# facebookresearch/dmc-net

Hardware: AMD Instinct MI355X
Metric: clips/sec (3-seg 224x224) DMC-gen+ResNet-18 train step (higher is better)
Workload: dtype f32

## Files before the change

dmc-net_amd/_lib.py:

```python
import ctypes
import os

PKG = os.path.dirname(os.path.abspath(__file__))
LIB_PATH = os.environ.get("DMC_HIP_LIB", os.path.join(PKG, "libdmcnet_hip.so"))

_P = ctypes.c_void_p
_I = ctypes.c_int
_F = ctypes.c_float
_Z = ctypes.c_size_t
_L = ctypes.c_long

SIGNATURES = {
    "dmc_version": (_I, []),
    "dmc_last_error": (ctypes.c_char_p, []),
    "dmc_profile_mark": (_I, [_P]),
    "dmc_set_option": (_I, [ctypes.c_char_p, _I]),
    "dmc_get_option": (_I, [ctypes.c_char_p]),
    "dmc_gen_tiny_workspace_bytes": (_Z, []),
    "dmc_gen_tiny_saved_bytes": (_Z, [_I, _I, _I]),
    "dmc_gen_tiny_gbuf_bytes": (_Z, [_I, _I, _I]),
    "dmc_gen_tiny_partials_bytes": (_Z, [_I, _I, _I]),
    "dmc_gen_tiny_fwd": (_I, [_P, _P, _P, _P, _P, _P, _P, _I, _I, _I, _I, _P]),
    "dmc_gen_tiny_mse_partials_bytes": (_Z, []),
    "dmc_gen_tiny_fwd_mse": (_I, [_P] * 10 + [_I, _I, _I, _I, _P]),
    "dmc_gen_tiny_bwd": (_I, [_P, _P, _P, _P, _P, _P, _P, _P, _P, _P, _I, _I, _I, _P]),
    "dmc_flow_mse_partials_bytes": (_Z, []),
    "dmc_flow_mse_fwd": (_I, [_P, _P, _P, _P, _Z, _P]),
    "dmc_flow_mse_bwd": (_I, [_P, _P, _P, _P, _Z, _P]),
    "dmc_consensus_ce_fwd_bwd": (_I, [_P, _P, _P, _P, _P, _I, _I, _I, _P]),
    "dmc_disc_tail_stats_bytes": (_Z, [_I]),
    "dmc_disc_tail_fwd": (_I, [_P, _P, _P, _P, _P, _P, _P, _P, _I, _I, _I, _I, _I, _I, _F, _F, _P]),
    "dmc_disc_tail_bwd": (_I, [_P, _P, _P, _P, _P, _P, _P, _P, _I, _I, _I, _I, _I, _P]),
    "dmc_prepare_inputs_workspace_bytes": (_Z, [_I, _I, _I, _I]),
    "dmc_prepare_inputs": (_I, [_P, _P, _P, _P, _P, _P, _I, _I, _I, _I, _P, _P]),
    "dmc_prepare_crop_workspace_bytes": (_Z, [_I, _I, _I, _I]),
    "dmc_prepare_inputs_crop": (_I, [_P, _P, _P, _P, _P, _P, _P, _I, _I, _I, _I, _I, _I, _P, _P]),
    "dmc_prepare_views_workspace_bytes": (_Z, [_I, _I, _I, _I, _I]),
    "dmc_prepare_inputs_views": (_I, [_P, _P, _P, _P, _P, _P, _P, _P, _I, _I, _I, _I, _I, _I, _I, _I, _P, _P]),
    "dmc_prepare_interp_taps": (_I, [_I, _I, _P, _P, _P]),
    "dmc_prepare_clip_workspace_bytes": (_Z, [_I, _I, _I, _I, _I]),
    "dmc_prepare_clip": (_I, [_P, _P, _P, _P] + [_I] * 8 + [_P, _P, _P]),
    "dmc_bn_act_supported": (_I, [_I, _I]),
    "dmc_bn_act_stats_bytes": (_Z, [_I]),
    "dmc_bn_act_scratch_bytes": (_Z, [_I]),
    "dmc_bn_act_fwd": (_I, [_P, _P, _P, _P, _P, _P, _P, _P, _P, _P, _I, _I, _I, _I, _F, _F, _P]),
    "dmc_bn_act_bwd": (_I, [_P, _P, _P, _P, _P, _P, _P, _P, _P, _P, _P, _P, _I, _I, _I, _P]),
    "dmc_bn_apply_nhwc": (_I, [_P, _P, _P, _P, _P, _I, _I, _P]),
    "dmc_bn_apply_act_nhwc": (_I, [_P, _P, _P, _P, _P, _P, _P, _I, _I, _I, _P]),
    "dmc_bn_bwd_act_nhwc": (_I, [_P] * 10 + [_I, _F, _I, _I, _P]),
    "dmc_channel_sum_nhwc": (_I, [_P, _P, _P, _I, _I, _P]),
    "dmc_bn_relu_pool_supported": (_I, [_I, _I, _I, _I]),
    "dmc_bn_relu_pool_fwd": (_I, [_P, _P, _P, _P, _P, _P, _P, _P, _I, _I, _I, _I, _I, _F, _F, _P]),
    "dmc_bn_relu_pool_codes_bytes": (_Z, [_I, _I, _I, _I]),
    "dmc_bn_relu_pool_bwd": (_I, [_P, _P, _P, _P, _P, _P, _P, _P, _P, _P, _I, _I, _I, _I, _P]),
    "dmc_conv_nhwc_supported": (_I, [_I] * 9),
    "dmc_conv_nhwc_stat_blocks": (_I, [_I] * 8),
    "dmc_conv_nhwc_fwd": (_I, [_P] * 7 + [_I] * 11 + [_P]),
    "dmc_conv_nhwc_stats_final": (_I, [_P, _I, _I, ctypes.c_long, _P, _P, _P, _F, _F, _P]),
    "dmc_conv_nhwc_wt_bytes": (_Z, [_I] * 4),
    "dmc_conv_nhwc_presplit_supported": (_I, [_I, _I]),
    "dmc_conv_nhwc_split": (_I, [_P, _P, _P, _I, _I, _I, _I, _P]),
    "dmc_conv_nhwc_dgrad": (_I, [_P] * 4 + [_I] * 9 + [_P]),
    "dmc_conv_nhwc_dgrad_add": (_I, [_P] * 5 + [_I] * 9 + [_P]),
    "dmc_conv_nhwc_wgrad_bytes": (_Z, [_I] * 9),
    "dmc_conv_nhwc_wgrad": (_I, [_P] * 4 + [_I] * 9 + [_P]),
    "dmc_x3s_slices_bytes": (_Z, [_L, _I]),
    "dmc_x3s_split": (_I, [_P, _P, _L, _I, _P]),
    "dmc_x3s_merge": (_I, [_P, _P, _L, _I, _P]),
    "dmc_x3s_wpack_bytes": (_Z, [_I, _I]),
    "dmc_x3s_pack_weights": (_I, [_P, _P, _P, _I, _I, _P]),
    "dmc_x3s_conv_supported": (_I, [_I] * 5),
    "dmc_x3s_conv_stat_blocks": (_I, [_I] * 4),
    "dmc_x3s_conv_fwd": (_I, [_P] * 4 + [_I] * 6 + [_P]),
    "dmc_x3s_conv_dgrad": (_I, [_P] * 4 + [_I] * 5 + [_P]),
    "dmc_x3s_conv_wgrad_supported": (_I, [_I] * 5),
    "dmc_x3s_conv_wgrad_bytes": (_Z, [_I] * 5),
    "dmc_x3s_conv_wgrad": (_I, [_P] * 4 + [_I] * 5 + [_P]),
    "dmc_x3s_conv_dgrad_s2_supported": (_I, [_I] * 5),
    "dmc_x3s_pack_weights_s2": (_I, [_P, _P, _I, _I, _P]),
    "dmc_x3s_conv_dgrad_s2": (_I, [_P] * 3 + [_I] * 5 + [_P]),
    "dmc_x3q_wpack_bytes": (_Z, [_I, _I]),
    "dmc_x3q_supported": (_I, [_I] * 5),
    "dmc_x3q_stat_blocks": (_I, [_I] * 4),
    "dmc_x3q_split": (_I, [_P, _P, _I, _I, _I, _I, _P]),
    "dmc_x3q_merge": (_I, [_P, _P, _I, _I, _I, _I, _P]),
    "dmc_x3q_pack_weights": (_I, [_P, _P, _P, _P, _I, _I, _P]),
    "dmc_x3q_conv_fwd": (_I, [_P] * 6 + [_I] * 6 + [_P]),
    "dmc_x3q_conv_dgrad": (_I, [_P] * 4 + [_I] * 5 + [_P]),
    "dmc_bn_apply_act_x3q": (_I, [_P] * 8 + [_I] * 5 + [_P]),
    "dmc_x3q_conv_wgrad_supported": (_I, [_I] * 5),
    "dmc_x3q_conv_wgrad_bytes": (_Z, [_I] * 5),
    "dmc_x3q_conv_wgrad": (_I, [_P] * 6 + [_I] * 5 + [_P]),
    "dmc_bn_apply_act_x3s": (_I, [_P] * 8 + [_I, _I, _I, _P]),
    "dmc_bn_act_bwd_x3s": (_I, [_P] * 13 + [_I, _I, _I, _P]),
    "dmc_x3s_conv_dgrad_bnb": (_I, [_P] * 9 + [_I] + [_P] + [_I] + [_P] * 2 + [_I] * 5 + [_P]),
    "dmc_bn_act_bwd_x3s_apply": (_I, [_P] * 12 + [_I, _I, _I, _P]),
    "dmc_bn_relu_pool_fwd_x3s": (_I, [_P] * 9 + [_I, _I, _I, _I, _I, _F, _F, _P]),
    "dmc_bn_relu_pool_fwd_arg": (_I, [_P] * 11 + [_I, _I, _I, _I, _I, _I, _F, _F, _P]),
    "dmc_bn_relu_pool_bwd_arg": (_I, [_P] * 11 + [_I, _I, _I, _I, _P]),
    "dmc_disc_first_supported": (_I, [_I]),
    "dmc_disc_first_fwd": (_I, [_P] * 5 + [_I] * 5 + [_P]),
    "dmc_disc_first_dgrad": (_I, [_P] * 3 + [_I] * 4 + [_P]),
    "dmc_disc_first_wgrad_bytes": (_Z, [_I]),
    "dmc_disc_first_wgrad": (_I, [_P] * 5 + [_I] * 4 + [_P]),
    "dmc_stem_wgrad_supported": (_I, [_I, _I]),
    "dmc_stem_wgrad_partials_bytes": (_Z, [_I, _I, _I]),
    "dmc_stem_wgrad": (_I, [_P, _P, _P, _P, _I, _I, _I, _P]),
    "dmc_stem_fwd": (_I, [_P, _P, _L, _L, _L, _L, _P, _I, _I, _I, _P]),
    "dmc_stem_fwd_x3_workspace_bytes": (_Z, [_I, _I, _I]),
    "dmc_stem_fwd_x3": (_I, [_P, _P, _L, _L, _L, _L, _P, _P, _I, _I, _I, _P]),
    "dmc_stem_fwd_x3_stat_blocks": (_I, [_I, _I, _I]),
    "dmc_stem_dgrad_workspace_bytes": (_Z, []),
    "dmc_stem_dgrad_supported": (_I, [_I, _I]),
    "dmc_stem_dgrad": (_I, [_P, _P, _L, _L, _L, _L, _P, _P, _I, _I, _I, _P]),
    "dmc_stem_fwd_x3_stats": (_I, [_P, _P, _L, _L, _L, _L, _P, _P, _P, _I, _I, _I, _P]),
    "dmc_conv3d_bf16_supported": (_I, [_I] * 9),
    "dmc_conv3d_bf16_wpack_bytes": (_Z, [_I] * 5),
    "dmc_conv3d_bf16_pack": (_I, [_P, _L, _L, _L, _P, _P] + [_I] * 5 + [_P]),
    "dmc_conv3d_bf16_stat_blocks": (_I, [_I] * 5),
    "dmc_conv3d_bf16_stat_blocks_k": (_I, [_I] * 9),
    "dmc_conv3d_bf16_fwd": (_I, [_P, _P, _L, _L, _L, _P, _P, _P] + [_I] * 9 + [_P]),
    "dmc_conv3d_bf16_dgrad": (_I, [_P, _P, _L, _L, _L, _P, _P] + [_I] * 9 + [_P]),
    "dmc_conv3d_bf16_wgrad_bytes": (_Z, [_I] * 9),
    "dmc_conv3d_bf16_wgrad": (_I, [_P] * 4 + [_I] * 9 + [_P]),
    "dmc_stem3d_bf16_workspace_bytes": (_Z, [_I] * 4),
    "dmc_stem3d_bf16_stat_blocks": (_I, [_I] * 4),
    "dmc_stem3d_bf16_fwd": (_I, [_P] * 5 + [_I] * 4 + [_P]),
    "dmc_stem3d_bf16_wgrad_workspace_bytes": (_Z, [_I] * 4),
    "dmc_stem3d_bf16_wgrad": (_I, [_P] * 4 + [_I] * 4 + [_P]),
    "dmc_stem3d_bf16_dgrad_workspace_bytes": (_Z, []),
    "dmc_stem3d_bf16_dgrad": (_I, [_P] * 4 + [_I] * 4 + [_P]),
    "dmc_bn3d_bf16_supported": (_I, [_L, _I]),
    "dmc_bn3d_bf16_scratch_bytes": (_Z, [_I]),
    "dmc_bn3d_bf16_fwd": (_I, [_P, _P, _I, _P, _P, _P, _P, _P, _P, _L, _I, _I, _F, _F, _P]),
    "dmc_add4_bf16": (_I, [_P] * 5 + [_L, _P]),
    "dmc_bn3d_bf16_fwd_ld": (_I, [_P, _P, _I, _P, _P, _P, _P, _P, _P, _L, _L, _I, _I, _F, _F, _P]),
    "dmc_bn3d_bf16_bwd": (_I, [_P, _L] + [_P] * 8 + [_L, _I, _I, _P]),
    "dmc_unit3d_bf16_fwd_workspace_bytes": (_Z, [_I] * 9),
    "dmc_unit3d_bf16_bwd_workspace_bytes": (_Z, [_I] * 9),
    "dmc_unit3d_bf16_fwd": (_I, [_P] * 9 + [_I] * 10 + [_F, _F, _P]),
    "dmc_unit3d_bf16_fwd_into": (_I, [_P] * 9 + [_L] + [_I] * 10 + [_F, _F, _P]),
    "dmc_unit3d_bf16_bwd": (_I, [_P, _L] + [_P] * 11 + [_I] * 10 + [_P]),
    "dmc_unit3d_bf16_eval_workspace_bytes": (_Z, [_I] * 9),
    "dmc_unit3d_bf16_fwd_eval": (_I, [_P] * 6 + [_F, _P, _P, _L] + [_I] * 10 + [_P]),
    "dmc_stem3d_bf16_eval_workspace_bytes": (_Z, [_I] * 4),
    "dmc_stem3d_bf16_fwd_eval": (_I, [_P] * 6 + [_F, _P, _P] + [_I] * 5 + [_P]),
    "dmc_maxpool3d_tf_out_shape": (_I, [_I] * 10 + [_P] * 3),
    "dmc_maxpool3d_tf_bf16_fwd": (_I, [_P] * 3 + [_I] * 11 + [_P]),
    "dmc_maxpool3d_tf_bf16_bwd": (_I, [_P] * 3 + [_I] * 11 + [_P]),
    "dmc_mv_owner_bytes": (_Z, [_I, _I, _I]),
    "dmc_mv_accu_init": (_I, [_P, _I, _I, _P]),
    "dmc_mv_rasterise": (_I, [_P, _I, _I, _P, _P, _P, _I, _I, _P]),
    "dmc_mv_accumulate": (_I, [_P, _I, _I, _P, _P, _P, _P, _I, _I, _P]),
    "dmc_mv_from_accu": (_I, [_P, _P, _I, _I, _P]),
    "dmc_residual": (_I, [_P, _P, _P, _P, _P, _I, _I, _P]),
    "dmc_mv_gop_batch": (_I, [_P, _I, _I, _P, _I, _P, _I, _P, _P, _P, _P, _P, _P, _P, _P, _I, _I, _P]),
}

_lib = None


class DmcHipError(RuntimeError):
    pass


def load():
    global _lib
    if _lib is None:
        if not os.path.exists(LIB_PATH):
            raise DmcHipError(
                "%s is missing: the DMC-Net hot path has no CPU fallback. Build it with "
                "`python -c 'import __graft_entry__ as g; g.build()'`." % LIB_PATH)
        lib = ctypes.CDLL(LIB_PATH)
        for name, (res, args) in SIGNATURES.items():
            fn = getattr(lib, name)
            fn.restype, fn.argtypes = res, args
        _lib = lib
    return _lib


def check(rc, what):
    if rc != 0:
        raise DmcHipError("%s failed (%d): %s" % (what, rc, load().dmc_last_error().decode()))


def ptr(t):
    return _P(t.data_ptr()) if t is not None else _P(0)


def ptr_array(tensors):
    return (_P * len(tensors))(*[t.data_ptr() for t in tensors])
```

dmc-net_amd/build.py:

```python
import os
import subprocess
import sys

PKG = os.path.dirname(os.path.abspath(__file__))
ROOT = os.path.dirname(PKG)
CSRC = os.path.join(PKG, "csrc")
LIB = os.path.join(PKG, "libdmcnet_hip.so")
MEASURE_ONLY = ["gen_fused_bwd.hip"]
SOURCES = ["gen_tiny.hip", "gen_x3.hip", "gen_fused.hip", "gen_wgrad.hip", "losses.hip", "disc_tail.hip", "bn_act.hip", "prepare.hip", "clip_prep.hip", "stem.hip", "conv_nhwc.hip", "conv_small.hip", "conv_x3s.hip", "conv_x3q.hip", "disc_first.hip", "conv3d_bf16.hip", "pool3d_bf16.hip", "bn3d_bf16.hip", "stem3d_bf16.hip", "unit3d.hip", "coviar_post.hip"]
HIPCC = os.environ.get("HIPCC", "/opt/rocm/bin/hipcc")
FLAGS = ["--offload-arch=gfx950", "-O3", "-std=c++17", "-fPIC", "-ffp-contract=off",
         "-Wall", "-Wno-unused-function"]


MANIFEST = os.path.join(PKG, "libdmcnet_hip.manifest.json")


def _sha(path):
    import hashlib
    with open(path, "rb") as f:
        return hashlib.sha256(f.read()).hexdigest()


def source_hashes():
    deps = sorted(os.path.join(CSRC, f) for f in os.listdir(CSRC) if not f.endswith((".o", ".hipfb")))
    deps += [os.path.join(ROOT, "include", "dmcnet_hip.h"), os.path.abspath(__file__)]
    return {os.path.relpath(d, ROOT): _sha(d) for d in deps}


def read_manifest():
    import json
    try:
        with open(MANIFEST) as f:
            return json.load(f)
    except (OSError, ValueError):
        return None


def _stale():
    if not os.path.exists(LIB):
        return True
    m = read_manifest()
    return m is None or m.get("library_sha256") != _sha(LIB) or m.get("sources") != source_hashes()


def _write_manifest(compiled):
    import json
    import time
    with open(MANIFEST, "w") as f:
        json.dump({"library": os.path.relpath(LIB, ROOT), "library_sha256": _sha(LIB), "built_at": time.strftime("%Y-%m-%dT%H:%M:%SZ", time.gmtime()),
                   "compiled_objects": compiled, "hipcc": HIPCC, "flags": FLAGS, "sources": source_hashes()}, f, indent=1, sort_keys=True)


LAST_BUILD = {"action": None}


MEASURE_LIB = os.path.join(PKG, "libdmcnet_hip_measure.so")


def build_library(force=False, verbose=False, measure=False):
    if measure:
        return _build_measure(verbose)
    if not force and not _stale():
        LAST_BUILD["action"] = "up to date (sources and library match the manifest's hashes)"
        return LIB
    objs, compiled = [], []
    for src in SOURCES:
        path = os.path.join(CSRC, src)
        if not os.path.exists(path):
            continue
        obj = os.path.join(CSRC, src.replace(".hip", ".o"))
        objs.append(obj)
        hdrs = [os.path.join(CSRC, "dmc_common.h"), os.path.join(CSRC, "x3s_common.h"), os.path.join(CSRC, "conv_small.h"), os.path.join(CSRC, "gen_x3.h"), os.path.join(CSRC, "gen_fused.h"), os.path.join(CSRC, "gen_fused_inl.h"), os.path.join(CSRC, "gen_wgrad.h"), os.path.join(ROOT, "include", "dmcnet_hip.h"),
                os.path.abspath(__file__)]
        if not force and os.path.exists(obj) and all(os.path.getmtime(d) <= os.path.getmtime(obj) for d in [path] + hdrs):
            continue
        cmd = [HIPCC] + FLAGS + ["-I", os.path.join(ROOT, "include"), "-I", CSRC, "-c", path, "-o", obj]
        if verbose:
            print(" ".join(cmd))
        subprocess.check_call(cmd)
        compiled.append(src)
    cmd = [HIPCC, "--offload-arch=gfx950", "-shared", "-fPIC", "-o", LIB] + objs
    if verbose:
        print(" ".join(cmd))
    subprocess.check_call(cmd)
    _write_manifest(compiled)
    LAST_BUILD["action"] = "compiled %d of %d sources and linked: %s" % (len(compiled), len(objs), ", ".join(compiled) or "(objects were current)")
    return LIB


def _build_measure(verbose):
    objs = []
    for src in SOURCES + MEASURE_ONLY:
        path = os.path.join(CSRC, src)
        obj = os.path.join(CSRC, "measure_" + src.replace(".hip", ".o"))
        objs.append(obj)
        deps = [path, os.path.abspath(__file__)] + [os.path.join(CSRC, f) for f in os.listdir(CSRC) if f.endswith(".h")]
        if os.path.exists(obj) and all(os.path.getmtime(d) <= os.path.getmtime(obj) for d in deps):
            continue
        cmd = [HIPCC] + FLAGS + ["-DDMC_MEASURE", "-I", os.path.join(ROOT, "include"), "-I", CSRC, "-c", path, "-o", obj]
        if verbose:
            print(" ".join(cmd))
        subprocess.check_call(cmd)
    subprocess.check_call([HIPCC, "--offload-arch=gfx950", "-shared", "-fPIC", "-o", MEASURE_LIB] + objs)
    return MEASURE_LIB


if __name__ == "__main__":
    print(build_library(force="--force" in sys.argv, verbose=True, measure="--measure" in sys.argv))
```

dmc-net_amd/csrc/bn_act.hip:

```cpp
#include "dmc_common.h"

using namespace dmc;

namespace {

constexpr int MAX_SPLIT = BN_MAX_SPLIT;

struct BnArgs {
    const float* x;
    const float* res;
    const float* gamma;
    const float* beta;
    const float* stats;
    const float* dy;
    float* y;
    float* dx;
    float* dres;
    int M, C, relu;
    unsigned char* mask;
    const float* keep;
    int hw;
    float slope;
};

template <int MODE>
__global__ __launch_bounds__(256) void bn_partial_kernel(BnArgs a, double* __restrict__ scratch) {
    __shared__ double sm[2][256][4];
    const int cq = a.C >> 2;
    const int tx = threadIdx.x % cq, ty = threadIdx.x / cq, rows = 256 / cq;
    const int per = (a.M + (int)gridDim.x - 1) / (int)gridDim.x;
    const int r0 = blockIdx.x * per, r1 = (r0 + per < a.M) ? r0 + per : a.M;
    float4 s0 = make_float4(0.f, 0.f, 0.f, 0.f), s1 = s0;
    float4 mean = s0, istd = s0, g = s0, b = s0;
    if (MODE == 1) {
        mean = reinterpret_cast<const float4*>(a.stats)[tx];
        istd = reinterpret_cast<const float4*>(a.stats + a.C)[tx];
        g = reinterpret_cast<const float4*>(a.gamma)[tx];
        b = reinterpret_cast<const float4*>(a.beta)[tx];
    }
#pragma unroll 4
    for (int r = r0 + ty; r < r1; r += rows) {
        const size_t o = (size_t)r * cq + tx;
        const float4 x = reinterpret_cast<const float4*>(a.x)[o];
        if (MODE == 0) {
            s0.x += x.x; s0.y += x.y; s0.z += x.z; s0.w += x.w;
            s1.x = fmaf(x.x, x.x, s1.x); s1.y = fmaf(x.y, x.y, s1.y);
            s1.z = fmaf(x.z, x.z, s1.z); s1.w = fmaf(x.w, x.w, s1.w);
        } else {
            float4 d = reinterpret_cast<const float4*>(a.dy)[o];
            const float4 xh = make_float4((x.x - mean.x) * istd.x, (x.y - mean.y) * istd.y,
                                          (x.z - mean.z) * istd.z, (x.w - mean.w) * istd.w);
            if (a.relu && a.mask) {
                const unsigned mb = a.mask[o];
                d.x = (mb & 1) ? d.x : 0.f; d.y = (mb & 2) ? d.y : 0.f;
                d.z = (mb & 4) ? d.z : 0.f; d.w = (mb & 8) ? d.w : 0.f;
            } else if (a.relu) {
                float4 v = make_float4(fmaf(xh.x, g.x, b.x), fmaf(xh.y, g.y, b.y),
                                       fmaf(xh.z, g.z, b.z), fmaf(xh.w, g.w, b.w));
                if (a.res) {
                    const float4 rr = reinterpret_cast<const float4*>(a.res)[o];
                    v.x += rr.x; v.y += rr.y; v.z += rr.z; v.w += rr.w;
                }
                d.x = v.x > 0.f ? d.x : 0.f; d.y = v.y > 0.f ? d.y : 0.f;
                d.z = v.z > 0.f ? d.z : 0.f; d.w = v.w > 0.f ? d.w : 0.f;
            }
            s0.x += d.x; s0.y += d.y; s0.z += d.z; s0.w += d.w;
            s1.x = fmaf(d.x, xh.x, s1.x); s1.y = fmaf(d.y, xh.y, s1.y);
            s1.z = fmaf(d.z, xh.z, s1.z); s1.w = fmaf(d.w, xh.w, s1.w);
        }
    }
    sm[0][threadIdx.x][0] = s0.x; sm[0][threadIdx.x][1] = s0.y;
    sm[0][threadIdx.x][2] = s0.z; sm[0][threadIdx.x][3] = s0.w;
    sm[1][threadIdx.x][0] = s1.x; sm[1][threadIdx.x][1] = s1.y;
    sm[1][threadIdx.x][2] = s1.z; sm[1][threadIdx.x][3] = s1.w;
    __syncthreads();
    for (int i = threadIdx.x; i < cq * 8; i += 256) {
        const int col = i >> 3, which = (i >> 2) & 1, e = i & 3;
        double acc = 0.0;
        for (int t = 0; t < rows; ++t) acc += sm[which][t * cq + col][e];
        scratch[((size_t)(col * 4 + e) * MAX_SPLIT + blockIdx.x) * 2 + which] = acc;
    }
}

__device__ __forceinline__ void reduce_partials(const double* __restrict__ scratch, int C, int c,
                                                int split, int sub, double& s, double& ss) {
    s = 0.0; ss = 0.0;
    if (c < C) {
        const double2* row = reinterpret_cast<const double2*>(scratch) + (size_t)c * MAX_SPLIT;
#pragma unroll 4
        for (int sp = sub; sp < split; sp += 32) {
            const double2 v = row[sp];
            s += v.x;
            ss += v.y;
        }
    }
#pragma unroll
    for (int o = 16; o > 0; o >>= 1) {
        s += __shfl_down(s, o, 32);
        ss += __shfl_down(ss, o, 32);
    }
}

__global__ __launch_bounds__(256) void bn_stats_final_kernel(
    const double* __restrict__ scratch, float* __restrict__ stats, float* __restrict__ running_mean,
    float* __restrict__ running_var, int C, long count, int training, float eps, float momentum,
    int split) {
    const int c = blockIdx.x * 8 + (threadIdx.x >> 5), sub = threadIdx.x & 31;
    if (!training) {
        if (c < C && sub == 0) {
            stats[c] = running_mean[c];
            stats[C + c] = rsqrtf(running_var[c] + eps);
        }
        return;
    }
    double s, ss;
    reduce_partials(scratch, C, c, split, sub, s, ss);
    if (c >= C || sub != 0) return;
    const double mean = s / (double)count;
    double var = ss / (double)count - mean * mean;
    if (var < 0.0) var = 0.0;
    stats[c] = (float)mean;
    stats[C + c] = (float)(1.0 / sqrt(var + (double)eps));
    const double unbiased = count > 1 ? var * (double)count / (double)(count - 1) : var;
    running_mean[c] = (1.f - momentum) * running_mean[c] + momentum * (float)mean;
    running_var[c] = (1.f - momentum) * running_var[c] + momentum * (float)unbiased;
}

__global__ __launch_bounds__(256) void bn_bwd_final_kernel(const double* __restrict__ scratch,
                                                           float* __restrict__ dgamma,
                                                           float* __restrict__ dbeta, int C,
                                                           int split) {
    __shared__ double red[2][4];
    const int c = blockIdx.x, lane = threadIdx.x & 63, wave = threadIdx.x >> 6;
    const double2* row = reinterpret_cast<const double2*>(scratch) + (size_t)c * MAX_SPLIT;
    double2 v[MAX_SPLIT / 256];
#pragma unroll
    for (int k = 0; k < MAX_SPLIT / 256; ++k) {
        const int sp = (int)threadIdx.x + 256 * k;
        v[k] = sp < split ? row[sp] : make_double2(0.0, 0.0);
    }
    double s = 0.0, ss = 0.0;
#pragma unroll
    for (int k = 0; k < MAX_SPLIT / 256; ++k) { s += v[k].x; ss += v[k].y; }
#pragma unroll
    for (int o = 32; o > 0; o >>= 1) { s += __shfl_down(s, o, 64); ss += __shfl_down(ss, o, 64); }
    if (lane == 0) { red[0][wave] = s; red[1][wave] = ss; }
    __syncthreads();
    if (threadIdx.x != 0) return;
    dbeta[c] = (float)(red[0][0] + red[0][1] + red[0][2] + red[0][3]);
    dgamma[c] = (float)(red[1][0] + red[1][1] + red[1][2] + red[1][3]);
}

__global__ __launch_bounds__(256) void bn_apply_fwd_kernel(BnArgs a) {
    const int cq = a.C >> 2;
    const size_t total = (size_t)a.M * cq;
    for (size_t o = (size_t)blockIdx.x * 256 + threadIdx.x; o < total; o += (size_t)gridDim.x * 256) {
        const int tx = (int)(o & (size_t)(cq - 1));
        const float4 mean = reinterpret_cast<const float4*>(a.stats)[tx];
        const float4 istd = reinterpret_cast<const float4*>(a.stats + a.C)[tx];
        const float4 g = reinterpret_cast<const float4*>(a.gamma)[tx];
        const float4 b = reinterpret_cast<const float4*>(a.beta)[tx];
        const float4 x = reinterpret_cast<const float4*>(a.x)[o];
        float4 v = make_float4(fmaf((x.x - mean.x) * istd.x, g.x, b.x), fmaf((x.y - mean.y) * istd.y, g.y, b.y),
                               fmaf((x.z - mean.z) * istd.z, g.z, b.z), fmaf((x.w - mean.w) * istd.w, g.w, b.w));
        if (a.res) {
            const float4 rr = reinterpret_cast<const float4*>(a.res)[o];
            v.x += rr.x; v.y += rr.y; v.z += rr.z; v.w += rr.w;
        }
        if (a.relu) {
            if (a.mask)
                a.mask[o] = (unsigned char)((v.x > 0.f ? 1 : 0) | (v.y > 0.f ? 2 : 0) | (v.z > 0.f ? 4 : 0) | (v.w > 0.f ? 8 : 0));
            v.x = fmaxf(v.x, 0.f); v.y = fmaxf(v.y, 0.f); v.z = fmaxf(v.z, 0.f); v.w = fmaxf(v.w, 0.f);
        }
        reinterpret_cast<float4*>(a.y)[o] = v;
    }
}

__global__ __launch_bounds__(256) void bn_apply_bwd_kernel(BnArgs a, const float* __restrict__ dgamma,
                                                           const float* __restrict__ dbeta,
                                                           float inv_count) {
    const int cq = a.C >> 2;
    const size_t total = (size_t)a.M * cq;
    for (size_t o = (size_t)blockIdx.x * 256 + threadIdx.x; o < total; o += (size_t)gridDim.x * 256) {
        const int tx = (int)(o & (size_t)(cq - 1));
        const float4 mean = reinterpret_cast<const float4*>(a.stats)[tx];
        const float4 istd = reinterpret_cast<const float4*>(a.stats + a.C)[tx];
        const float4 g = reinterpret_cast<const float4*>(a.gamma)[tx];
        const float4 b = reinterpret_cast<const float4*>(a.beta)[tx];
        const float4 dg = reinterpret_cast<const float4*>(dgamma)[tx];
        const float4 db = reinterpret_cast<const float4*>(dbeta)[tx];
        const float4 x = reinterpret_cast<const float4*>(a.x)[o];
        float4 d = reinterpret_cast<const float4*>(a.dy)[o];
        const float4 xh = make_float4((x.x - mean.x) * istd.x, (x.y - mean.y) * istd.y,
                                      (x.z - mean.z) * istd.z, (x.w - mean.w) * istd.w);
        if (a.relu && a.mask) {
            const unsigned mb = a.mask[o];
            d.x = (mb & 1) ? d.x : 0.f; d.y = (mb & 2) ? d.y : 0.f;
            d.z = (mb & 4) ? d.z : 0.f; d.w = (mb & 8) ? d.w : 0.f;
        } else if (a.relu) {
            float4 v = make_float4(fmaf(xh.x, g.x, b.x), fmaf(xh.y, g.y, b.y), fmaf(xh.z, g.z, b.z),
                                   fmaf(xh.w, g.w, b.w));
            if (a.res) {
                const float4 rr = reinterpret_cast<const float4*>(a.res)[o];
                v.x += rr.x; v.y += rr.y; v.z += rr.z; v.w += rr.w;
            }
            d.x = v.x > 0.f ? d.x : 0.f; d.y = v.y > 0.f ? d.y : 0.f;
            d.z = v.z > 0.f ? d.z : 0.f; d.w = v.w > 0.f ? d.w : 0.f;
        }
        if (a.dres) reinterpret_cast<float4*>(a.dres)[o] = d;
        float4 r;
        r.x = g.x * istd.x * (d.x - db.x * inv_count - xh.x * dg.x * inv_count);
        r.y = g.y * istd.y * (d.y - db.y * inv_count - xh.y * dg.y * inv_count);
        r.z = g.z * istd.z * (d.z - db.z * inv_count - xh.z * dg.z * inv_count);
        r.w = g.w * istd.w * (d.w - db.w * inv_count - xh.w * dg.w * inv_count);
        if (a.slope != 0.f) {
            float4 k = make_float4(1.f, 1.f, 1.f, 1.f);
            if (a.keep) k = reinterpret_cast<const float4*>(a.keep)[(size_t)((o / cq) / a.hw) * cq + tx];
            r.x *= k.x * (x.x > 0.f ? 1.f : a.slope); r.y *= k.y * (x.y > 0.f ? 1.f : a.slope);
            r.z *= k.z * (x.z > 0.f ? 1.f : a.slope); r.w *= k.w * (x.w > 0.f ? 1.f : a.slope);
        }
        reinterpret_cast<float4*>(a.dx)[o] = r;
    }
}

struct PoolArgs {
    const float* x;
    const float* gamma;
    const float* beta;
    const float* stats;
    const float* dpool;
    float* ypool;
    float* dx;
    int N, H, W, C, PH, PW;
};

__device__ __forceinline__ float4 bn_relu4(const float4 x, const float4 mean, const float4 istd,
                                           const float4 g, const float4 b) {
    return make_float4(fmaxf(fmaf((x.x - mean.x) * istd.x, g.x, b.x), 0.f), fmaxf(fmaf((x.y - mean.y) * istd.y, g.y, b.y), 0.f),
                       fmaxf(fmaf((x.z - mean.z) * istd.z, g.z, b.z), 0.f), fmaxf(fmaf((x.w - mean.w) * istd.w, g.w, b.w), 0.f));
}

__global__ __launch_bounds__(256) void pool_fwd_kernel(PoolArgs a) {
    const int cq = a.C >> 2;
    const size_t total = (size_t)a.N * a.PH * a.PW * cq;
    for (size_t o = (size_t)blockIdx.x * 256 + threadIdx.x; o < total; o += (size_t)gridDim.x * 256) {
        const int tx = (int)(o & (size_t)(cq - 1));
        size_t r = o / cq;
        const int px = (int)(r % a.PW); r /= a.PW;
        const int py = (int)(r % a.PH);
        const int n = (int)(r / a.PH);
        const float4 mean = reinterpret_cast<const float4*>(a.stats)[tx];
        const float4 istd = reinterpret_cast<const float4*>(a.stats + a.C)[tx];
        const float4 g = reinterpret_cast<const float4*>(a.gamma)[tx];
        const float4 b = reinterpret_cast<const float4*>(a.beta)[tx];
        float4 m = make_float4(0.f, 0.f, 0.f, 0.f);
        float4 xv[9];
#pragma unroll
        for (int k = 0; k < 9; ++k) {
            int iy = 2 * py + k / 3 - 1, ix = 2 * px + k % 3 - 1;
            iy = iy < 0 ? 0 : (iy >= a.H ? a.H - 1 : iy);
            ix = ix < 0 ? 0 : (ix >= a.W ? a.W - 1 : ix);
            xv[k] = reinterpret_cast<const float4*>(a.x)[((size_t)(n * a.H + iy) * a.W + ix) * cq + tx];
        }
#pragma unroll
        for (int k = 0; k < 9; ++k) {
            const float4 v = bn_relu4(xv[k], mean, istd, g, b);
            m.x = fmaxf(m.x, v.x); m.y = fmaxf(m.y, v.y); m.z = fmaxf(m.z, v.z); m.w = fmaxf(m.w, v.w);
        }
        reinterpret_cast<float4*>(a.ypool)[o] = m;
    }
}

constexpr int PT = 8;
template <int PASS>
__global__ __launch_bounds__(256) void pool_bwd_kernel(PoolArgs a, double* __restrict__ scratch,
                                                       const float* __restrict__ dgamma,
                                                       const float* __restrict__ dbeta, float inv_count,
                                                       unsigned* __restrict__ gcodes) {
    __shared__ unsigned codes[(PT + 1) * (PT + 1) * 64];
    __shared__ double sm[PASS == 1 ? 2 : 1][PASS == 1 ? 256 : 1][4];
    const int cq = a.C >> 2;
    const int tx = threadIdx.x % cq, ty = threadIdx.x / cq, rows = 256 / cq;
    const float4 mean = reinterpret_cast<const float4*>(a.stats)[tx];
    const float4 istd = reinterpret_cast<const float4*>(a.stats + a.C)[tx];
    const float4 g = reinterpret_cast<const float4*>(a.gamma)[tx];
    const float4 b = reinterpret_cast<const float4*>(a.beta)[tx];
    float4 dg = make_float4(0.f, 0.f, 0.f, 0.f), db = dg;
    if (PASS == 2) {
        dg = reinterpret_cast<const float4*>(dgamma)[tx];
        db = reinterpret_cast<const float4*>(dbeta)[tx];
    }
    float4 s0 = make_float4(0.f, 0.f, 0.f, 0.f), s1 = s0;
    const int tiles_x = (a.PW + PT - 1) / PT, tiles_y = (a.PH + PT - 1) / PT;
    const int ntiles = a.N * tiles_y * tiles_x;
    for (int tile = blockIdx.x; tile < ntiles; tile += gridDim.x) {
        const int n = tile / (tiles_y * tiles_x), tr = tile - n * tiles_y * tiles_x;
        const int wy0 = (tr / tiles_x) * PT, wx0 = (tr % tiles_x) * PT;
        __syncthreads();
        for (int wi = ty; wi < (PT + 1) * (PT + 1); wi += rows) {
            const int py = wy0 + wi / (PT + 1), px = wx0 + wi % (PT + 1);
            unsigned code = 0xffffffffu;
            if (PASS == 2 && gcodes) {
                if (py < a.PH && px < a.PW) code = gcodes[((size_t)(n * a.PH + py) * a.PW + px) * cq + tx];
            } else if (py < a.PH && px < a.PW) {
                float4 mv = make_float4(-INFINITY, -INFINITY, -INFINITY, -INFINITY);
                unsigned cx = 0, cy = 0, cz = 0, cw = 0;
                float4 xv[9];
#pragma unroll
                for (int k = 0; k < 9; ++k) {
                    int iy = 2 * py + k / 3 - 1, ix = 2 * px + k % 3 - 1;
                    iy = iy < 0 ? 0 : (iy >= a.H ? a.H - 1 : iy);
                    ix = ix < 0 ? 0 : (ix >= a.W ? a.W - 1 : ix);
                    xv[k] = reinterpret_cast<const float4*>(a.x)[((size_t)(n * a.H + iy) * a.W + ix) * cq + tx];
                }
#pragma unroll
                for (int k = 0; k < 9; ++k) {
                    const int iy = 2 * py + k / 3 - 1, ix = 2 * px + k % 3 - 1;
                    const bool in = iy >= 0 && iy < a.H && ix >= 0 && ix < a.W;
                    const float4 v = bn_relu4(xv[k], mean, istd, g, b);
                    if (in && v.x > mv.x) { mv.x = v.x; cx = k; }
                    if (in && v.y > mv.y) { mv.y = v.y; cy = k; }
                    if (in && v.z > mv.z) { mv.z = v.z; cz = k; }
                    if (in && v.w > mv.w) { mv.w = v.w; cw = k; }
                }
                code = cx | (cy << 8) | (cz << 16) | (cw << 24);
                if (PASS == 1 && gcodes && wi / (PT + 1) < PT && wi % (PT + 1) < PT)
                    gcodes[((size_t)(n * a.PH + py) * a.PW + px) * cq + tx] = code;
            }
            codes[wi * cq + tx] = code;
        }
        __syncthreads();
        for (int pi = ty; pi < 4 * PT * PT; pi += rows) {
            const int iy = 2 * wy0 + pi / (2 * PT), ix = 2 * wx0 + pi % (2 * PT);
            if (iy >= a.H || ix >= a.W) continue;
            const size_t o = ((size_t)(n * a.H + iy) * a.W + ix) * cq + tx;
            const float4 x = reinterpret_cast<const float4*>(a.x)[o];
            const float4 xh = make_float4((x.x - mean.x) * istd.x, (x.y - mean.y) * istd.y,
                                          (x.z - mean.z) * istd.z, (x.w - mean.w) * istd.w);
            const float4 v = make_float4(fmaf(xh.x, g.x, b.x), fmaf(xh.y, g.y, b.y), fmaf(xh.z, g.z, b.z), fmaf(xh.w, g.w, b.w));
            float4 d = make_float4(0.f, 0.f, 0.f, 0.f);
            const int py0 = iy >> 1, px0 = ix >> 1, npy = 1 + (iy & 1), npx = 1 + (ix & 1);
            float4 gp[4];
            unsigned cd[4];
            bool okc[4];
#pragma unroll
            for (int q = 0; q < 4; ++q) {
                const int jy = q >> 1, jx = q & 1;
                const int py = py0 + jy, px = px0 + jx;
                okc[q] = jy < npy && jx < npx && py < a.PH && px < a.PW;
                const int pyc = okc[q] ? py : py0, pxc = okc[q] ? px : px0;
                cd[q] = codes[((pyc - wy0) * (PT + 1) + (pxc - wx0)) * cq + tx];
                gp[q] = reinterpret_cast<const float4*>(a.dpool)[((size_t)(n * a.PH + pyc) * a.PW + pxc) * cq + tx];
            }
#pragma unroll
            for (int q = 0; q < 4; ++q) {
                const int py = py0 + (q >> 1), px = px0 + (q & 1);
                const unsigned k = (unsigned)((iy - 2 * py + 1) * 3 + (ix - 2 * px + 1));
                if (okc[q] && (cd[q] & 0xff) == k) d.x += gp[q].x;
                if (okc[q] && ((cd[q] >> 8) & 0xff) == k) d.y += gp[q].y;
                if (okc[q] && ((cd[q] >> 16) & 0xff) == k) d.z += gp[q].z;
                if (okc[q] && (cd[q] >> 24) == k) d.w += gp[q].w;
            }
            d.x = v.x > 0.f ? d.x : 0.f; d.y = v.y > 0.f ? d.y : 0.f;
            d.z = v.z > 0.f ? d.z : 0.f; d.w = v.w > 0.f ? d.w : 0.f;
            if (PASS == 1) {
                s0.x += d.x; s0.y += d.y; s0.z += d.z; s0.w += d.w;
                s1.x = fmaf(d.x, xh.x, s1.x); s1.y = fmaf(d.y, xh.y, s1.y);
                s1.z = fmaf(d.z, xh.z, s1.z); s1.w = fmaf(d.w, xh.w, s1.w);
            } else {
                float4 r;
                r.x = g.x * istd.x * (d.x - db.x * inv_count - xh.x * dg.x * inv_count);
                r.y = g.y * istd.y * (d.y - db.y * inv_count - xh.y * dg.y * inv_count);
                r.z = g.z * istd.z * (d.z - db.z * inv_count - xh.z * dg.z * inv_count);
                r.w = g.w * istd.w * (d.w - db.w * inv_count - xh.w * dg.w * inv_count);
                reinterpret_cast<float4*>(a.dx)[o] = r;
            }
        }
    }
    if (PASS == 1) {
        sm[0][threadIdx.x][0] = s0.x; sm[0][threadIdx.x][1] = s0.y;
        sm[0][threadIdx.x][2] = s0.z; sm[0][threadIdx.x][3] = s0.w;
        sm[1][threadIdx.x][0] = s1.x; sm[1][threadIdx.x][1] = s1.y;
        sm[1][threadIdx.x][2] = s1.z; sm[1][threadIdx.x][3] = s1.w;
        __syncthreads();
        for (int i = threadIdx.x; i < cq * 8; i += 256) {
            const int col = i >> 3, which = (i >> 2) & 1, e = i & 3;
            double acc = 0.0;
            for (int t = 0; t < rows; ++t) acc += sm[which][t * cq + col][e];
            scratch[((size_t)(col * 4 + e) * MAX_SPLIT + blockIdx.x) * 2 + which] = acc;
        }
    }
}

__global__ __launch_bounds__(256) void act_mask_bwd_kernel(const float* __restrict__ z, const float* __restrict__ keep,
                                                           const float* __restrict__ dz, float* __restrict__ dx,
                                                           int M, int C, int hw, float slope) {
    const int cq = C >> 2;
    const size_t total = (size_t)M * cq;
    for (size_t o = (size_t)blockIdx.x * 256 + threadIdx.x; o < total; o += (size_t)gridDim.x * 256) {
        const int tx = (int)(o % cq);
        const float4 x = reinterpret_cast<const float4*>(z)[o];
        float4 d = reinterpret_cast<const float4*>(dz)[o];
        float4 k = make_float4(1.f, 1.f, 1.f, 1.f);
        if (keep) k = reinterpret_cast<const float4*>(keep)[(size_t)((o / cq) / hw) * cq + tx];
        d.x *= k.x * (x.x > 0.f ? 1.f : slope); d.y *= k.y * (x.y > 0.f ? 1.f : slope);
        d.z *= k.z * (x.z > 0.f ? 1.f : slope); d.w *= k.w * (x.w > 0.f ? 1.f : slope);
        reinterpret_cast<float4*>(dx)[o] = d;
    }
}

__global__ __launch_bounds__(256) void channel_sum_final_kernel(const double* __restrict__ scratch,
                                                                float* __restrict__ out, int C, int split) {
    const int c = blockIdx.x * 8 + (threadIdx.x >> 5), sub = threadIdx.x & 31;
    double s, ss;
    reduce_partials(scratch, C, c, split, sub, s, ss);
    if (c < C && sub == 0) out[c] = (float)s;
}

bool shape_ok(int M, int C) {
    const int cq = C / 4;
    return M > 0 && C > 0 && C % 4 == 0 && cq <= 256 && 256 % cq == 0;
}

int split_of(int M, int C) {
    long sp = (long)M * C / 8192;
    return sp < 1 ? 1 : (sp > MAX_SPLIT ? MAX_SPLIT : (int)sp);
}

int stream_blocks(size_t total) {
    size_t b = (total + 255) / 256;
    return (int)(b < 1 ? 1 : (b > 8192 ? 8192 : b));
}


__device__ __forceinline__ void load8(const float* p, size_t i8, float (&v)[8]) {
    const float4 a = reinterpret_cast<const float4*>(p)[2 * i8], b = reinterpret_cast<const float4*>(p)[2 * i8 + 1];
    v[0] = a.x; v[1] = a.y; v[2] = a.z; v[3] = a.w; v[4] = b.x; v[5] = b.y; v[6] = b.z; v[7] = b.w;
}
__device__ __forceinline__ void store8(float* p, size_t i8, const float (&v)[8]) {
    reinterpret_cast<float4*>(p)[2 * i8] = make_float4(v[0], v[1], v[2], v[3]);
    reinterpret_cast<float4*>(p)[2 * i8 + 1] = make_float4(v[4], v[5], v[6], v[7]);
}

__global__ __launch_bounds__(256) void bn_apply_fwd_x3s_kernel(BnArgs a, unsigned short* __restrict__ ys, int s2d_h, int s2d_w) {
    const int c8 = a.C >> 3;
    const size_t total = (size_t)a.M * c8;
    for (size_t o = (size_t)blockIdx.x * 256 + threadIdx.x; o < total; o += (size_t)gridDim.x * 256) {
        const int tx = (int)(o & (size_t)(c8 - 1));
        const size_t m = o / c8;
        float mean[8], istd[8], g[8], b[8], x[8], v[8];
        load8(a.stats, tx, mean); load8(a.stats + a.C, tx, istd); load8(a.gamma, tx, g); load8(a.beta, tx, b);
        load8(a.x, o, x);
#pragma unroll
        for (int e = 0; e < 8; ++e) v[e] = fmaf((x[e] - mean[e]) * istd[e], g[e], b[e]);
        if (a.res) {
            float rr[8];
            load8(a.res, o, rr);
#pragma unroll
            for (int e = 0; e < 8; ++e) v[e] += rr[e];
        }
        if (a.relu) {
            if (a.mask) {
                unsigned mb = 0;
#pragma unroll
                for (int e = 0; e < 8; ++e) mb |= (v[e] > 0.f ? 1u : 0u) << e;
                reinterpret_cast<unsigned short*>(a.mask)[o] = (unsigned short)((mb & 15u) | ((mb >> 4) << 8));
            }
#pragma unroll
            for (int e = 0; e < 8; ++e) v[e] = fmaxf(v[e], 0.f);
        }
        if (a.y) store8(a.y, o, v);
        if (ys) {
            if (s2d_w) {
                const int xx = (int)(m % (size_t)s2d_w), yy = (int)((m / (size_t)s2d_w) % (size_t)s2d_h);
                const size_t n = m / ((size_t)s2d_w * s2d_h);
                const int cls = (yy & 1) * 2 + (xx & 1), nchunk = a.C >> 4;
                x3s_store8(ys, v, (size_t)a.M >> 2, 4 * nchunk, (n * (s2d_h >> 1) + (yy >> 1)) * (s2d_w >> 1) + (xx >> 1), tx + cls * 2 * nchunk);
            } else {
                x3s_store8(ys, v, (size_t)a.M, a.C >> 4, m, tx);
            }
        }
    }
}

__global__ __launch_bounds__(256) void bn_apply_bwd_x3s_kernel(BnArgs a, const float* __restrict__ dgamma,
                                                               const float* __restrict__ dbeta, float inv_count,
                                                               unsigned short* __restrict__ dxs) {
    const int c8 = a.C >> 3;
    const size_t total = (size_t)a.M * c8;
    for (size_t o = (size_t)blockIdx.x * 256 + threadIdx.x; o < total; o += (size_t)gridDim.x * 256) {
        const int tx = (int)(o & (size_t)(c8 - 1));
        const size_t m = o / c8;
        float mean[8], istd[8], g[8], b[8], dg[8], db[8], x[8], d[8], xh[8], r[8];
        load8(a.stats, tx, mean); load8(a.stats + a.C, tx, istd); load8(a.gamma, tx, g); load8(a.beta, tx, b);
        load8(dgamma, tx, dg); load8(dbeta, tx, db);
        load8(a.x, o, x); load8(a.dy, o, d);
#pragma unroll
        for (int e = 0; e < 8; ++e) xh[e] = (x[e] - mean[e]) * istd[e];
        if (a.relu && a.mask) {
            const unsigned mw = reinterpret_cast<const unsigned short*>(a.mask)[o];
            const unsigned mb = (mw & 15u) | ((mw >> 8) << 4);
#pragma unroll
            for (int e = 0; e < 8; ++e) d[e] = ((mb >> e) & 1u) ? d[e] : 0.f;
        } else if (a.relu) {
            float rr[8];
            if (a.res) load8(a.res, o, rr);
#pragma unroll
            for (int e = 0; e < 8; ++e) {
                float v = fmaf(xh[e], g[e], b[e]);
                if (a.res) v += rr[e];
                d[e] = v > 0.f ? d[e] : 0.f;
            }
        }
        if (a.dres) store8(a.dres, o, d);
#pragma unroll
        for (int e = 0; e < 8; ++e) r[e] = g[e] * istd[e] * (d[e] - db[e] * inv_count - xh[e] * dg[e] * inv_count);
        if (a.dx) store8(a.dx, o, r);
        if (dxs) x3s_store8(dxs, r, (size_t)a.M, a.C >> 4, m, tx);
    }
}

__global__ __launch_bounds__(256) void pool_fwd_x3s_kernel(PoolArgs a, unsigned short* __restrict__ ys, unsigned* __restrict__ codes,
                                                           float* __restrict__ xmax) {
    const int c8 = a.C >> 3;
    const size_t total = (size_t)a.N * a.PH * a.PW * c8;
    for (size_t o = (size_t)blockIdx.x * 256 + threadIdx.x; o < total; o += (size_t)gridDim.x * 256) {
        const int tx = (int)(o & (size_t)(c8 - 1));
        size_t r = o / c8;
        const size_t mp = r;
        const int px = (int)(r % a.PW); r /= a.PW;
        const int py = (int)(r % a.PH);
        const int n = (int)(r / a.PH);
        float mean[8], istd[8], g[8], b[8], mx[8];
        load8(a.stats, tx, mean); load8(a.stats + a.C, tx, istd); load8(a.gamma, tx, g); load8(a.beta, tx, b);
        float xv[9][8];
#pragma unroll
        for (int k = 0; k < 9; ++k) {
            int iy = 2 * py + k / 3 - 1, ix = 2 * px + k % 3 - 1;
            iy = iy < 0 ? 0 : (iy >= a.H ? a.H - 1 : iy);
            ix = ix < 0 ? 0 : (ix >= a.W ? a.W - 1 : ix);
            load8(a.x, ((size_t)(n * a.H + iy) * a.W + ix) * c8 + tx, xv[k]);
        }
        if (codes) {
            float bx[8];
            unsigned ck[8];
#pragma unroll
            for (int e = 0; e < 8; ++e) { mx[e] = -INFINITY; bx[e] = 0.f; ck[e] = 0; }
#pragma unroll
            for (int k = 0; k < 9; ++k) {
                const int iy = 2 * py + k / 3 - 1, ix = 2 * px + k % 3 - 1;
                const bool in = iy >= 0 && iy < a.H && ix >= 0 && ix < a.W;
#pragma unroll
                for (int e = 0; e < 8; ++e) {
                    const float v = fmaxf(fmaf((xv[k][e] - mean[e]) * istd[e], g[e], b[e]), 0.f);
                    const bool take = in && v > mx[e];
                    mx[e] = take ? v : mx[e];
                    bx[e] = take ? xv[k][e] : bx[e];
                    ck[e] = take ? (unsigned)k : ck[e];
                }
            }
            reinterpret_cast<uint2*>(codes)[o] = make_uint2(ck[0] | (ck[1] << 8) | (ck[2] << 16) | (ck[3] << 24),
                                                            ck[4] | (ck[5] << 8) | (ck[6] << 16) | (ck[7] << 24));
            store8(xmax, o, bx);
        } else {
#pragma unroll
            for (int e = 0; e < 8; ++e) mx[e] = 0.f;
#pragma unroll
            for (int k = 0; k < 9; ++k)
#pragma unroll
                for (int e = 0; e < 8; ++e) mx[e] = fmaxf(mx[e], fmaxf(fmaf((xv[k][e] - mean[e]) * istd[e], g[e], b[e]), 0.f));
        }
        if (a.ypool) store8(a.ypool, o, mx);
        if (ys) x3s_store8(ys, mx, (size_t)a.N * a.PH * a.PW, a.C >> 4, mp, tx);
    }
}

bool shape_ok8(int M, int C) { return shape_ok(M, C) && C % 16 == 0 && C >= 16; }

}

extern "C" {

int dmc_bn_act_supported(int M, int C) { return shape_ok(M, C) ? 1 : 0; }

size_t dmc_bn_act_stats_bytes(int C) { return (((size_t)2 * C * sizeof(float)) + 15) / 16 * 16; }
size_t dmc_bn_act_scratch_bytes(int C) { return (size_t)MAX_SPLIT * C * 2 * sizeof(double); }

int dmc_bn_act_fwd(const float* x, const float* residual, const float* gamma, const float* beta,
                   float* running_mean, float* running_var, float* y, float* stats, void* scratch_,
                   unsigned char* relu_mask, int M, int C, int relu, int training, float eps,
                   float momentum, dmc_stream_t stream) {
    if (!x || !gamma || !beta || !running_mean || !running_var || !y || !stats || (training && !scratch_))
        return fail(DMC_E_INVALID, "dmc_bn_act_fwd: null pointer");
    if (!shape_ok(M, C)) return fail(DMC_E_INVALID, "dmc_bn_act_fwd: unsupported shape M=%d C=%d", M, C);
    hipStream_t s = (hipStream_t)stream;
    BnArgs a = {x, residual, gamma, beta, stats, nullptr, y, nullptr, nullptr, M, C, relu, relu_mask};
    double* scratch = static_cast<double*>(scratch_);
    int rc;
    const int split = split_of(M, C);
    if (training) {
        bn_partial_kernel<0><<<split, 256, 0, s>>>(a, scratch);
        if ((rc = check_launch("bn_partial"))) return rc;
    }
    bn_stats_final_kernel<<<(C + 7) / 8, 256, 0, s>>>(scratch, stats, running_mean, running_var, C,
                                                       (long)M, training, eps, momentum, split);
    if ((rc = check_launch("bn_stats_final"))) return rc;
    bn_apply_fwd_kernel<<<stream_blocks((size_t)M * (C / 4)), 256, 0, s>>>(a);
    return check_launch("bn_apply_fwd");
}

int dmc_bn_act_bwd(const float* x, const float* residual, const float* gamma, const float* beta,
                   const float* stats, void* scratch_, const float* dy, float* dx, float* dresidual,
                   float* dgamma, float* dbeta, const unsigned char* relu_mask, int M, int C, int relu,
                   dmc_stream_t stream) {
    if (!x || !gamma || !beta || !stats || !scratch_ || !dy || !dx || !dgamma || !dbeta)
        return fail(DMC_E_INVALID, "dmc_bn_act_bwd: null pointer");
    if (!shape_ok(M, C)) return fail(DMC_E_INVALID, "dmc_bn_act_bwd: unsupported shape M=%d C=%d", M, C);
    hipStream_t s = (hipStream_t)stream;
    BnArgs a = {x, residual, gamma, beta, stats, dy, nullptr, dx, dresidual, M, C, relu,
                const_cast<unsigned char*>(relu_mask)};
    double* scratch = static_cast<double*>(scratch_);
    int rc;
    const int split = split_of(M, C);
    bn_partial_kernel<1><<<split, 256, 0, s>>>(a, scratch);
    if ((rc = check_launch("bn_bwd_partial"))) return rc;
    bn_bwd_final_kernel<<<C, 256, 0, s>>>(scratch, dgamma, dbeta, C, split);
    if ((rc = check_launch("bn_bwd_final"))) return rc;
    bn_apply_bwd_kernel<<<stream_blocks((size_t)M * (C / 4)), 256, 0, s>>>(a, dgamma, dbeta, 1.f / (float)M);
    return check_launch("bn_apply_bwd");
}

int dmc_bn_relu_pool_supported(int N, int H, int W, int C) {
    return N > 0 && H > 0 && W > 0 && shape_ok(1, C) && C / 4 <= 64 ? 1 : 0;
}

int dmc_bn_relu_pool_fwd(const float* x, const float* gamma, const float* beta, float* running_mean,
                         float* running_var, float* y_pool, float* stats, void* scratch_, int N, int H,
                         int W, int C, int training, float eps, float momentum, dmc_stream_t stream) {
    if (!x || !gamma || !beta || !running_mean || !running_var || !y_pool || !stats || (training && !scratch_))
        return fail(DMC_E_INVALID, "dmc_bn_relu_pool_fwd: null pointer");
    if (!dmc_bn_relu_pool_supported(N, H, W, C))
        return fail(DMC_E_INVALID, "dmc_bn_relu_pool_fwd: unsupported shape N=%d H=%d W=%d C=%d", N, H, W, C);
    hipStream_t s = (hipStream_t)stream;
    const int M = N * H * W;
    BnArgs a = {x, nullptr, gamma, beta, stats, nullptr, nullptr, nullptr, nullptr, M, C, 1, nullptr};
    double* scratch = static_cast<double*>(scratch_);
    int rc;
    const int split = split_of(M, C);
    if (training) {
        bn_partial_kernel<0><<<split, 256, 0, s>>>(a, scratch);
        if ((rc = check_launch("bn_partial"))) return rc;
    }
    bn_stats_final_kernel<<<(C + 7) / 8, 256, 0, s>>>(scratch, stats, running_mean, running_var, C,
                                                       (long)M, training, eps, momentum, split);
    if ((rc = check_launch("bn_stats_final"))) return rc;
    PoolArgs p = {x, gamma, beta, stats, nullptr, y_pool, nullptr, N, H, W, C, (H - 1) / 2 + 1, (W - 1) / 2 + 1};
    pool_fwd_kernel<<<stream_blocks((size_t)N * p.PH * p.PW * (C / 4)), 256, 0, s>>>(p);
    return check_launch("pool_fwd");
}

size_t dmc_bn_relu_pool_codes_bytes(int N, int H, int W, int C) {
    return (size_t)N * ((H - 1) / 2 + 1) * ((W - 1) / 2 + 1) * (C / 4) * sizeof(unsigned);
}

int dmc_bn_relu_pool_bwd(const float* x, const float* gamma, const float* beta, const float* stats,
                         void* scratch_, const float* d_pool, float* dx, float* dgamma, float* dbeta,
                         void* codes, int N, int H, int W, int C, dmc_stream_t stream) {
    if (!x || !gamma || !beta || !stats || !scratch_ || !d_pool || !dx || !dgamma || !dbeta)
        return fail(DMC_E_INVALID, "dmc_bn_relu_pool_bwd: null pointer");
    if (!dmc_bn_relu_pool_supported(N, H, W, C))
        return fail(DMC_E_INVALID, "dmc_bn_relu_pool_bwd: unsupported shape N=%d H=%d W=%d C=%d", N, H, W, C);
    hipStream_t s = (hipStream_t)stream;
    PoolArgs p = {x, gamma, beta, stats, d_pool, nullptr, dx, N, H, W, C, (H - 1) / 2 + 1, (W - 1) / 2 + 1};
    double* scratch = static_cast<double*>(scratch_);
    const long tiles = (long)N * ((p.PH + PT - 1) / PT) * ((p.PW + PT - 1) / PT);
    const int blocks = (int)(tiles < MAX_SPLIT ? tiles : MAX_SPLIT);
    int rc;
    pool_bwd_kernel<1><<<blocks, 256, 0, s>>>(p, scratch, nullptr, nullptr, 0.f, (unsigned*)codes);
    if ((rc = check_launch("pool_bwd_partial"))) return rc;
    bn_bwd_final_kernel<<<C, 256, 0, s>>>(scratch, dgamma, dbeta, C, blocks);
    if ((rc = check_launch("bn_bwd_final"))) return rc;
    pool_bwd_kernel<2><<<blocks * 4 > 8192 ? 8192 : blocks * 4, 256, 0, s>>>(p, nullptr, dgamma, dbeta,
                                                                             1.f / (float)((long)N * H * W), (unsigned*)codes);
    return check_launch("pool_bwd_apply");
}

int dmc_bn_apply_act_nhwc(const float* x, const float* residual, const float* gamma, const float* beta,
                          const float* stats, float* y, unsigned char* relu_mask, int M, int C, int relu,
                          dmc_stream_t stream) {
    if (!x || !gamma || !beta || !stats || !y) return fail(DMC_E_INVALID, "dmc_bn_apply_act_nhwc: null pointer");
    if (!shape_ok(M, C)) return fail(DMC_E_INVALID, "dmc_bn_apply_act_nhwc: unsupported shape M=%d C=%d", M, C);
    BnArgs a = {x, residual, gamma, beta, stats, nullptr, y, nullptr, nullptr, M, C, relu, relu_mask};
    bn_apply_fwd_kernel<<<stream_blocks((size_t)M * (C / 4)), 256, 0, (hipStream_t)stream>>>(a);
    return check_launch("bn_apply_act_nhwc");
}

int dmc_bn_apply_nhwc(const float* x, const float* gamma, const float* beta, const float* stats, float* y,
                      int M, int C, dmc_stream_t stream) {
    return dmc_bn_apply_act_nhwc(x, nullptr, gamma, beta, stats, y, nullptr, M, C, 0, stream);
}

int dmc_bn_bwd_act_nhwc(const float* z, const float* gamma, const float* beta, const float* stats, void* scratch_,
                        const float* dy, float* dpre, float* dgamma, float* dbeta, const float* keep, int hw,
                        float slope, int M, int C, dmc_stream_t stream) {
    if (!z || !dy || !dpre || hw <= 0) return fail(DMC_E_INVALID, "dmc_bn_bwd_act_nhwc: bad argument");
    if (!shape_ok(M, C)) return fail(DMC_E_INVALID, "dmc_bn_bwd_act_nhwc: unsupported shape M=%d C=%d", M, C);
    hipStream_t s = (hipStream_t)stream;
    if (!gamma) {
        act_mask_bwd_kernel<<<stream_blocks((size_t)M * (C / 4)), 256, 0, s>>>(z, keep, dy, dpre, M, C, hw, slope);
        return check_launch("act_mask_bwd");
    }
    if (!beta || !stats || !scratch_ || !dgamma || !dbeta)
        return fail(DMC_E_INVALID, "dmc_bn_bwd_act_nhwc: null BatchNorm pointer");
    BnArgs a = {z, nullptr, gamma, beta, stats, dy, nullptr, dpre, nullptr, M, C, 0, nullptr, keep, hw, slope};
    double* scratch = static_cast<double*>(scratch_);
    int rc;
    const int split = split_of(M, C);
    bn_partial_kernel<1><<<split, 256, 0, s>>>(a, scratch);
    if ((rc = check_launch("bn_bwd_partial"))) return rc;
    bn_bwd_final_kernel<<<C, 256, 0, s>>>(scratch, dgamma, dbeta, C, split);
    if ((rc = check_launch("bn_bwd_final"))) return rc;
    bn_apply_bwd_kernel<<<stream_blocks((size_t)M * (C / 4)), 256, 0, s>>>(a, dgamma, dbeta, 1.f / (float)M);
    return check_launch("bn_apply_bwd_act");
}

int dmc_channel_sum_nhwc(const float* g, void* scratch_, float* out, int M, int C, dmc_stream_t stream) {
    if (!g || !scratch_ || !out) return fail(DMC_E_INVALID, "dmc_channel_sum_nhwc: null pointer");
    if (!shape_ok(M, C)) return fail(DMC_E_INVALID, "dmc_channel_sum_nhwc: unsupported shape M=%d C=%d", M, C);
    hipStream_t s = (hipStream_t)stream;
    BnArgs a = {g, nullptr, nullptr, nullptr, nullptr, nullptr, nullptr, nullptr, nullptr, M, C, 0, nullptr};
    const int split = split_of(M, C);
    bn_partial_kernel<0><<<split, 256, 0, s>>>(a, static_cast<double*>(scratch_));
    int rc = check_launch("channel_sum_partial");
    if (rc) return rc;
    channel_sum_final_kernel<<<(C + 7) / 8, 256, 0, s>>>(static_cast<const double*>(scratch_), out, C, split);
    return check_launch("channel_sum_final");
}

int dmc_bn_apply_act_x3s(const float* x, const float* residual, const float* gamma, const float* beta, const float* stats,
                         float* y, void* ys, unsigned char* relu_mask, int M, int C, int relu, dmc_stream_t stream) {
    if (!x || !gamma || !beta || !stats || (!y && !ys)) return fail(DMC_E_INVALID, "dmc_bn_apply_act_x3s: null pointer");
    if (!shape_ok8(M, C)) return fail(DMC_E_INVALID, "dmc_bn_apply_act_x3s: unsupported shape M=%d C=%d", M, C);
    BnArgs a = {x, residual, gamma, beta, stats, nullptr, y, nullptr, nullptr, M, C, relu, relu_mask};
    bn_apply_fwd_x3s_kernel<<<stream_blocks((size_t)M * (C / 8)), 256, 0, (hipStream_t)stream>>>(a, static_cast<unsigned short*>(ys), 0, 0);
    return check_launch("bn_apply_act_x3s");
}

int dmc_bn_apply_act_x3q(const float* x, const float* residual, const float* gamma, const float* beta, const float* stats,
                         float* y, void* yq, unsigned char* relu_mask, int N, int H, int W, int C, int relu, dmc_stream_t stream) {
    if (!x || !gamma || !beta || !stats || !yq) return fail(DMC_E_INVALID, "dmc_bn_apply_act_x3q: null pointer");
    if (N <= 0 || H <= 0 || W <= 0 || (H & 1) || (W & 1) || (long)N * H * W >= (1L << 31)) return fail(DMC_E_INVALID, "dmc_bn_apply_act_x3q: bad geometry");
    const int M = N * H * W;
    if (!shape_ok8(M, C)) return fail(DMC_E_INVALID, "dmc_bn_apply_act_x3q: unsupported shape M=%d C=%d", M, C);
    BnArgs a = {x, residual, gamma, beta, stats, nullptr, y, nullptr, nullptr, M, C, relu, relu_mask};
    bn_apply_fwd_x3s_kernel<<<stream_blocks((size_t)M * (C / 8)), 256, 0, (hipStream_t)stream>>>(a, static_cast<unsigned short*>(yq), H, W);
    return check_launch("bn_apply_act_x3q");
}

int dmc_bn_act_bwd_x3s(const float* x, const float* residual, const float* gamma, const float* beta, const float* stats,
                       void* scratch_, const float* dy, float* dx, void* dxs, float* dresidual, float* dgamma, float* dbeta,
                       const unsigned char* relu_mask, int M, int C, int relu, dmc_stream_t stream) {
    if (!x || !gamma || !beta || !stats || !scratch_ || !dy || (!dx && !dxs) || !dgamma || !dbeta)
        return fail(DMC_E_INVALID, "dmc_bn_act_bwd_x3s: null pointer");
    if (!shape_ok8(M, C)) return fail(DMC_E_INVALID, "dmc_bn_act_bwd_x3s: unsupported shape M=%d C=%d", M, C);
    hipStream_t s = (hipStream_t)stream;
    BnArgs a = {x, residual, gamma, beta, stats, dy, nullptr, dx, dresidual, M, C, relu, const_cast<unsigned char*>(relu_mask)};
    double* scratch = static_cast<double*>(scratch_);
    int rc;
    const int split = split_of(M, C);
    bn_partial_kernel<1><<<split, 256, 0, s>>>(a, scratch);
    if ((rc = check_launch("bn_bwd_partial"))) return rc;
    bn_bwd_final_kernel<<<C, 256, 0, s>>>(scratch, dgamma, dbeta, C, split);
    if ((rc = check_launch("bn_bwd_final"))) return rc;
    bn_apply_bwd_x3s_kernel<<<stream_blocks((size_t)M * (C / 8)), 256, 0, s>>>(a, dgamma, dbeta, 1.f / (float)M, static_cast<unsigned short*>(dxs));
    return check_launch("bn_apply_bwd_x3s");
}

int dmc_bn_relu_pool_fwd_arg(const float* x, const float* gamma, const float* beta, float* running_mean, float* running_var,
                             float* y_pool, void* ys, void* codes, float* xmax, float* stats, void* scratch_, int stat_split,
                             int N, int H, int W, int C, int training, float eps, float momentum, dmc_stream_t stream) {
    if (!x || !gamma || !beta || !running_mean || !running_var || (!y_pool && !ys) || !stats || (training && !scratch_))
        return fail(DMC_E_INVALID, "dmc_bn_relu_pool_fwd_x3s: null pointer");
    if (stat_split < 0 || stat_split > MAX_SPLIT) return fail(DMC_E_INVALID, "dmc_bn_relu_pool_fwd_arg: bad stat_split %d", stat_split);
    if ((codes == nullptr) != (xmax == nullptr)) return fail(DMC_E_INVALID, "dmc_bn_relu_pool_fwd_arg: codes and xmax go together");
    if (!dmc_bn_relu_pool_supported(N, H, W, C) || C % 16 != 0)
        return fail(DMC_E_INVALID, "dmc_bn_relu_pool_fwd_x3s: unsupported shape N=%d H=%d W=%d C=%d", N, H, W, C);
    hipStream_t s = (hipStream_t)stream;
    const int M = N * H * W;
    BnArgs a = {x, nullptr, gamma, beta, stats, nullptr, nullptr, nullptr, nullptr, M, C, 1, nullptr};
    double* scratch = static_cast<double*>(scratch_);
    int rc;
    const int split = stat_split > 0 ? stat_split : split_of(M, C);
    if (training && stat_split == 0) {
        bn_partial_kernel<0><<<split, 256, 0, s>>>(a, scratch);
        if ((rc = check_launch("bn_partial"))) return rc;
    }
    bn_stats_final_kernel<<<(C + 7) / 8, 256, 0, s>>>(scratch, stats, running_mean, running_var, C, (long)M, training, eps, momentum, split);
    if ((rc = check_launch("bn_stats_final"))) return rc;
    PoolArgs p = {x, gamma, beta, stats, nullptr, y_pool, nullptr, N, H, W, C, (H - 1) / 2 + 1, (W - 1) / 2 + 1};
    pool_fwd_x3s_kernel<<<stream_blocks((size_t)N * p.PH * p.PW * (C / 8)), 256, 0, s>>>(p, static_cast<unsigned short*>(ys),
                                                                                         static_cast<unsigned*>(codes), xmax);
    return check_launch("pool_fwd_x3s");
}

int dmc_bn_relu_pool_fwd_x3s(const float* x, const float* gamma, const float* beta, float* running_mean, float* running_var,
                             float* y_pool, void* ys, float* stats, void* scratch_, int N, int H, int W, int C, int training,
                             float eps, float momentum, dmc_stream_t stream) {
    return dmc_bn_relu_pool_fwd_arg(x, gamma, beta, running_mean, running_var, y_pool, ys, nullptr, nullptr, stats, scratch_, 0, N, H, W, C,
                                    training, eps, momentum, stream);
}

int dmc_bn_relu_pool_bwd_arg(const float* x, const float* gamma, const float* beta, const float* stats, void* scratch_,
                             const float* d_pool, const void* codes, const float* xmax, float* dx, float* dgamma, float* dbeta,
                             int N, int H, int W, int C, dmc_stream_t stream) {
    if (!x || !gamma || !beta || !stats || !scratch_ || !d_pool || !codes || !xmax || !dx || !dgamma || !dbeta)
        return fail(DMC_E_INVALID, "dmc_bn_relu_pool_bwd_arg: null pointer");
    if (!dmc_bn_relu_pool_supported(N, H, W, C) || C % 16 != 0)
        return fail(DMC_E_INVALID, "dmc_bn_relu_pool_bwd_arg: unsupported shape N=%d H=%d W=%d C=%d", N, H, W, C);
    hipStream_t s = (hipStream_t)stream;
    PoolArgs p = {x, gamma, beta, stats, d_pool, nullptr, dx, N, H, W, C, (H - 1) / 2 + 1, (W - 1) / 2 + 1};
    double* scratch = static_cast<double*>(scratch_);
    const int MP = N * p.PH * p.PW;
    BnArgs a = {xmax, nullptr, gamma, beta, stats, d_pool, nullptr, nullptr, nullptr, MP, C, 1, nullptr};
    const int split = split_of(MP, C);
    int rc;
    bn_partial_kernel<1><<<split, 256, 0, s>>>(a, scratch);
    if ((rc = check_launch("pool_bwd_sums"))) return rc;
    bn_bwd_final_kernel<<<C, 256, 0, s>>>(scratch, dgamma, dbeta, C, split);
    if ((rc = check_launch("bn_bwd_final"))) return rc;
    const long tiles = (long)N * ((p.PH + PT - 1) / PT) * ((p.PW + PT - 1) / PT);
    const long blocks = tiles * 4 > 8192 ? 8192 : tiles * 4;
    pool_bwd_kernel<2><<<(int)blocks, 256, 0, s>>>(p, nullptr, dgamma, dbeta, 1.f / (float)((long)N * H * W),
                                                   const_cast<unsigned*>(static_cast<const unsigned*>(codes)));
    return check_launch("pool_bwd_apply");
}

int dmc_bn_act_bwd_x3s_apply(const float* x, const float* residual, const float* gamma, const float* beta, const float* stats,
                             const float* dy, float* dx, void* dxs, float* dresidual, const float* dgamma, const float* dbeta,
                             const unsigned char* relu_mask, int M, int C, int relu, dmc_stream_t stream) {
    if (!x || !gamma || !beta || !stats || !dy || (!dx && !dxs) || !dgamma || !dbeta)
        return fail(DMC_E_INVALID, "dmc_bn_act_bwd_x3s_apply: null pointer");
    if (!shape_ok8(M, C)) return fail(DMC_E_INVALID, "dmc_bn_act_bwd_x3s_apply: unsupported shape M=%d C=%d", M, C);
    BnArgs a = {x, residual, gamma, beta, stats, dy, nullptr, dx, dresidual, M, C, relu, const_cast<unsigned char*>(relu_mask)};
    bn_apply_bwd_x3s_kernel<<<stream_blocks((size_t)M * (C / 8)), 256, 0, (hipStream_t)stream>>>(a, dgamma, dbeta, 1.f / (float)M, static_cast<unsigned short*>(dxs));
    return check_launch("bn_apply_bwd_x3s");
}

}
```

dmc-net_amd/csrc/stem.hip:

```cpp
#include "dmc_common.h"

using namespace dmc;

namespace {

constexpr int S_CO = 64, S_CI = 2, S_K = 7, S_NCOL = S_CI * S_K * S_K;
constexpr int S_NT = (S_NCOL + 15) / 16;
constexpr int S_MT = S_CO / 16;
constexpr int S_TH = 7, S_TW = 16;
constexpr int S_XROWS = 2 * S_TH + 5, S_XPITCH = 40;
constexpr int S_XPLANE = S_XROWS * S_XPITCH;
constexpr int S_X = S_CI * S_XPLANE;
constexpr int S_G = S_TH * S_TW * S_CO;
constexpr int S_BUF = S_X + S_G;
constexpr int S_PART = S_MT * S_NT * 256;
constexpr int S_MAX_GROUPS = 256, S_RED = 16;
static_assert(S_PART <= 2 * S_BUF, "cross-wave reduction reuses the tile buffers");

struct StemArgs {
    const float* x;
    const float* dy;
    float* partials;
    int N, H, W, OH, OW, tiles_x, tiles_y;
};

__device__ __forceinline__ void stem_stage(const StemArgs& a, float* buf, int tile, int per_frame, int lane) {
    const int n = tile / per_frame, r0 = tile - n * per_frame;
    const int oy0 = (r0 / a.tiles_x) * S_TH, ox0 = (r0 % a.tiles_x) * S_TW;
    const unsigned buf_byte = lds_addr_of(buf);
    const bool g_interior = oy0 + S_TH <= a.OH && ox0 + S_TW <= a.OW;
#pragma unroll
    for (int row = 0; row < S_TH; ++row) {
        const unsigned long long rbase =
            (unsigned long long)(a.dy + (((size_t)n * a.OH + (oy0 + row)) * a.OW + ox0) * S_CO);
#pragma unroll
        for (int q = 0; q < 4; ++q) {
            const unsigned dst = buf_byte + (unsigned)(S_X + (row * S_TW + q * 4) * S_CO) * 4;
            if (g_interior) {
                lds_dma16(rbase + q * 1024, (unsigned)lane * 16, dst);
            } else {
                const bool ok = oy0 + row < a.OH && ox0 + q * 4 + (lane >> 4) < a.OW;
                if (ok) lds_dma16(rbase + q * 1024, (unsigned)lane * 16, dst);
                else reinterpret_cast<float4*>(buf + S_X + (row * S_TW + q * 4) * S_CO)[lane] = make_float4(0.f, 0.f, 0.f, 0.f);
            }
        }
    }
    const int iy0 = 2 * oy0 - 3, ix0 = 2 * ox0 - 4;
    const bool x_interior = iy0 >= 0 && iy0 + S_XROWS <= a.H && ix0 >= 0 && ix0 + S_XPITCH <= a.W;
    const size_t HW = (size_t)a.H * a.W;
#pragma unroll
    for (int ci = 0; ci < S_CI; ++ci) {
        const long org = ((long)iy0 * a.W + ix0) * 4;
        const unsigned long long pbase = (unsigned long long)(a.x + ((size_t)n * S_CI + ci) * HW) + (unsigned long long)org;
#pragma unroll
        for (int h = 0; h < 3; ++h) {
            const int L = 64 * h + lane;
            const int row = L / 10, ch = L - row * 10;
            const unsigned voff = (unsigned)(row * a.W + ch * 4) * 4;
            const unsigned dst = buf_byte + (unsigned)(ci * S_XPLANE + 256 * h) * 4;
            if (L < S_XROWS * 10) {
                const int iy = iy0 + row, ix = ix0 + ch * 4;
                const bool ok = x_interior || (iy >= 0 && iy < a.H && ix >= 0 && ix < a.W);
                if (ok) lds_dma16(pbase, voff, dst);
                else reinterpret_cast<float4*>(buf + ci * S_XPLANE)[L] = make_float4(0.f, 0.f, 0.f, 0.f);
            }
        }
    }
}

__global__ __launch_bounds__(512, 2) void stem_wgrad_kernel(StemArgs a) {
    __shared__ __attribute__((aligned(16))) float lds2[2 * S_BUF];
    const int lane = threadIdx.x & 63;
    const int wave = __builtin_amdgcn_readfirstlane((int)(threadIdx.x >> 6));
    const int j = lane & 15, kq = lane >> 4;
    const int per_frame = a.tiles_x * a.tiles_y;
    const int ntiles = a.N * per_frame;

    mfma_f32x4 acc[S_MT][S_NT];
#pragma unroll
    for (int m = 0; m < S_MT; ++m)
#pragma unroll
        for (int t = 0; t < S_NT; ++t) acc[m][t] = (mfma_f32x4){0.f, 0.f, 0.f, 0.f};

    if (wave == S_TH) {
        int it = 0;
        if ((int)blockIdx.x < ntiles) stem_stage(a, lds2, blockIdx.x, per_frame, lane);
        asm volatile("s_waitcnt vmcnt(0) lgkmcnt(0)\n\ts_barrier" ::: "memory");
        for (int tile = blockIdx.x; tile < ntiles; tile += gridDim.x, ++it) {
            const int next = tile + (int)gridDim.x;
            if (next < ntiles) stem_stage(a, lds2 + ((it + 1) & 1) * S_BUF, next, per_frame, lane);
            asm volatile("s_waitcnt vmcnt(0) lgkmcnt(0)\n\ts_barrier" ::: "memory");
        }
    } else {
        int offB[S_NT];
#pragma unroll
        for (int t = 0; t < S_NT; ++t) {
            int nn = 16 * t + j;
            nn = nn < S_NCOL ? nn : S_NCOL - 1;
            const int ci = nn / 49, rem = nn - ci * 49, ky = rem / 7, kx = rem - ky * 7;
            offB[t] = ci * S_XPLANE + (2 * wave + ky) * S_XPITCH + kx + 1 + 2 * kq;
        }
        const int offA = S_X + (wave * S_TW + kq) * S_CO + 4 * j;
        int it = 0;
        asm volatile("s_barrier" ::: "memory");
        for (int tile = blockIdx.x; tile < ntiles; tile += gridDim.x, ++it) {
            const float* lds = lds2 + (it & 1) * S_BUF;
#pragma unroll
            for (int g = 0; g < S_TW / 4; ++g) {
                const float4 av = *reinterpret_cast<const float4*>(lds + offA + g * 4 * S_CO);
                const float am[S_MT] = {av.x, av.y, av.z, av.w};
                float b[S_NT];
#pragma unroll
                for (int t = 0; t < S_NT; ++t) b[t] = lds[offB[t] + g * 8];
#pragma unroll
                for (int m = 0; m < S_MT; ++m)
#pragma unroll
                    for (int t = 0; t < S_NT; ++t)
                        acc[m][t] = __builtin_amdgcn_mfma_f32_16x16x4f32(am[m], b[t], acc[m][t], 0, 0, 0);
            }
            asm volatile("s_barrier" ::: "memory");
        }
    }
    float* lds = lds2;
    for (int w = 0; w < S_TH; ++w) {
        if (wave == w) {
#pragma unroll
            for (int m = 0; m < S_MT; ++m)
#pragma unroll
                for (int t = 0; t < S_NT; ++t)
#pragma unroll
                    for (int q = 0; q < 4; ++q) {
                        const int idx = (m * S_NT + t) * 256 + (kq * 4 + q) * 16 + j;
                        lds[idx] = (w == 0 ? 0.f : lds[idx]) + acc[m][t][q];
                    }
        }
        __syncthreads();
    }
    float* part = a.partials + (size_t)blockIdx.x * S_PART;
    for (int i = threadIdx.x; i < S_PART; i += 512) part[i] = lds[i];
}

__global__ __launch_bounds__(256) void stem_reduce1_kernel(float* __restrict__ partials, int groups) {
    const int i = blockIdx.x * 256 + threadIdx.x;
    const int per = (groups + S_RED - 1) / S_RED;
    const int g0 = blockIdx.y * per, g1 = (g0 + per < groups) ? g0 + per : groups;
    float s = 0.f;
    for (int g = g0; g < g1; ++g) s += partials[(size_t)g * S_PART + i];
    partials[(size_t)(groups + blockIdx.y) * S_PART + i] = s;
}

__global__ void stem_reduce2_kernel(const float* __restrict__ partials, int groups, float* __restrict__ dw) {
    const int i = blockIdx.x * blockDim.x + threadIdx.x;
    if (i >= S_CO * S_NCOL) return;
    const int co = i / S_NCOL, nn = i - co * S_NCOL;
    const int m = co & 3, row = co >> 2, t = nn >> 4, col = nn & 15;
    const size_t off = (size_t)(m * S_NT + t) * 256 + row * 16 + col;
    float s = 0.f;
    for (int c = 0; c < S_RED; ++c) s += partials[(size_t)(groups + c) * S_PART + off];
    dw[i] = s;
}


typedef float stem_f32x16 __attribute__((ext_vector_type(16)));

struct StemFwdArgs {
    const float* x;
    const float* w;
    float* y;
    int N, H, W, OH, OW, tiles_x;
    long ws_co, ws_ci, ws_ky, ws_kx;
};

__global__ __launch_bounds__(256, 2) void stem_fwd_kernel(StemFwdArgs a) {
    const int lane = threadIdx.x & 63;
    const int wave = __builtin_amdgcn_readfirstlane((int)(threadIdx.x >> 6));
    const int l31 = lane & 31, half = lane >> 5;
    const int HW = a.H * a.W;

    float wr[2][49];
#pragma unroll
    for (int kp = 0; kp < 49; ++kp) {
        const long o = half * a.ws_ci + (kp / 7) * a.ws_ky + (kp % 7) * a.ws_kx;
#pragma unroll
        for (int ct = 0; ct < 2; ++ct) wr[ct][kp] = a.w[(32 * ct + l31) * a.ws_co + o];
    }

    const long ntiles = (long)a.N * a.OH * a.tiles_x;
    const long stride = (long)gridDim.x * 4;
    auto load_tile = [&](long tile, float (&xv)[49]) {
        const int xt = (int)(tile % a.tiles_x);
        const long r = tile / a.tiles_x;
        const int oy = (int)(r % a.OH);
        const int n = (int)(r / a.OH);
        const int ox = 32 * xt + l31;
        const int iy0 = 2 * oy - 3, ix0 = 2 * ox - 3;
        const float* plane = a.x + ((long)n * 2 + half) * HW;
        const bool cols_inside = 64 * xt - 3 >= 0 && 64 * xt + 62 + 3 < a.W;
        unsigned cm = 0;
#pragma unroll
        for (int kx = 0; kx < 7; ++kx) cm |= (ix0 + kx >= 0 && ix0 + kx < a.W) ? 1u << kx : 0u;
#pragma unroll
        for (int ky = 0; ky < 7; ++ky) {
            const int iy = iy0 + ky;
            if (iy < 0 || iy >= a.H) {
#pragma unroll
                for (int kx = 0; kx < 7; ++kx) xv[ky * 7 + kx] = 0.f;
                continue;
            }
            const int rowoff = iy * a.W + ix0;
            if (cols_inside) {
#pragma unroll
                for (int kx = 0; kx < 7; ++kx) xv[ky * 7 + kx] = plane[rowoff + kx];
            } else {
#pragma unroll
                for (int kx = 0; kx < 7; ++kx) {
                    const bool ok = (cm >> kx) & 1;
                    const float v = plane[ok ? rowoff + kx : iy * a.W];
                    xv[ky * 7 + kx] = ok ? v : 0.f;
                }
            }
        }
    };

    long tile = (long)blockIdx.x * 4 + wave;
    float xc[49], xn[49];
    if (tile < ntiles) load_tile(tile, xc);
    for (; tile < ntiles; tile += stride) {
        const long next = tile + stride;
        if (next < ntiles) load_tile(next, xn);
        stem_f32x16 acc[2];
#pragma unroll
        for (int ct = 0; ct < 2; ++ct)
#pragma unroll
            for (int e = 0; e < 16; ++e) acc[ct][e] = 0.f;
#pragma unroll
        for (int kp = 0; kp < 49; ++kp)
#pragma unroll
            for (int ct = 0; ct < 2; ++ct) acc[ct] = __builtin_amdgcn_mfma_f32_32x32x2f32(wr[ct][kp], xc[kp], acc[ct], 0, 0, 0);
        const int xt = (int)(tile % a.tiles_x);
        const long r = tile / a.tiles_x;
        const int ox = 32 * xt + l31;
        if (ox < a.OW) {
            float* dst = a.y + (r * a.OW + ox) * S_CO;
#pragma unroll
            for (int ct = 0; ct < 2; ++ct)
#pragma unroll
                for (int g = 0; g < 4; ++g)
                    *reinterpret_cast<float4*>(dst + 32 * ct + 8 * g + 4 * half) =
                        make_float4(acc[ct][4 * g], acc[ct][4 * g + 1], acc[ct][4 * g + 2], acc[ct][4 * g + 3]);
        }
#pragma unroll
        for (int kp = 0; kp < 49; ++kp) xc[kp] = xn[kp];
    }
}

typedef __bf16 stem_bf16x8 __attribute__((ext_vector_type(8)));
typedef unsigned stem_u32x4 __attribute__((ext_vector_type(4)));
typedef unsigned stem_u32x2 __attribute__((ext_vector_type(2)));
constexpr int SX_WLDS = 3 * 7 * S_CO * 32;

__device__ __forceinline__ void stem_split3(float v, unsigned& s0, unsigned& s1, unsigned& s2) {
    const unsigned u0 = __float_as_uint(v);
    const float r1 = v - __uint_as_float(u0 & 0xffff0000u);
    const unsigned u1 = __float_as_uint(r1);
    const unsigned u2 = __float_as_uint(r1 - __uint_as_float(u1 & 0xffff0000u));
    s0 = u0 >> 16; s1 = u1 >> 16; s2 = u2 >> 16;
}

__global__ __launch_bounds__(256) void stem_prep_x3_kernel(const float* __restrict__ x, unsigned* __restrict__ xs, int N, int H, int W,
                                                           int Hp, int Wp) {
    const long vol = (long)N * Hp * Wp, plane = (long)H * W;
    for (long i = (long)blockIdx.x * 256 + threadIdx.x; i < vol; i += (long)gridDim.x * 256) {
        const int xx = (int)(i % Wp);
        const long r = i / Wp;
        const int yy = (int)(r % Hp);
        const int n = (int)(r / Hp);
        const int h = yy - 3, w = xx - 3;
        unsigned a0 = 0, a1 = 0, a2 = 0, b0 = 0, b1 = 0, b2 = 0;
        if (h >= 0 && h < H && w >= 0 && w < W) {
            const long o = (long)n * 2 * plane + (long)h * W + w;
            stem_split3(x[o], a0, a1, a2);
            stem_split3(x[o + plane], b0, b1, b2);
        }
        xs[i] = a0 | (b0 << 16); xs[vol + i] = a1 | (b1 << 16); xs[2 * vol + i] = a2 | (b2 << 16);
    }
}

__global__ __launch_bounds__(256) void stem_pack_w3_kernel(const float* __restrict__ w, unsigned short* __restrict__ wp, long s_co, long s_ci,
                                                           long s_ky, long s_kx) {
    const int i = blockIdx.x * 256 + threadIdx.x;
    if (i >= 7 * S_CO * 16) return;
    const int j = i & 15, co = (i >> 4) & 63, ky = i >> 10;
    unsigned s0 = 0, s1 = 0, s2 = 0;
    if (j < 14) stem_split3(w[co * s_co + (j & 1) * s_ci + ky * s_ky + (j >> 1) * s_kx], s0, s1, s2);
    wp[i] = (unsigned short)s0; wp[7 * S_CO * 16 + i] = (unsigned short)s1; wp[2 * 7 * S_CO * 16 + i] = (unsigned short)s2;
}

struct StemX3Args {
    const unsigned* xs;
    const unsigned short* wp;
    float* y;
    int N, OH, OW, Hp, Wp, tiles_x;
    long vol;
    double* stat_part;
};

constexpr int SX_THREADS = 1024, SX_WAVES = SX_THREADS / 64;
constexpr int SX_EP_PITCH = 36;
constexpr int SX_EP_BYTES = 32 * SX_EP_PITCH * 4;
constexpr int SX_LDS = SX_WLDS + SX_WAVES * SX_EP_BYTES;

__global__ __launch_bounds__(SX_THREADS) void stem_fwd_x3_kernel(StemX3Args a) {
    extern __shared__ __attribute__((aligned(16))) char wlds3[];
    const int tid = threadIdx.x, lane = tid & 63;
    const int wave = __builtin_amdgcn_readfirstlane(tid >> 6);
    const int l31 = lane & 31, half = lane >> 5;
    for (int i = tid; i < SX_WLDS / 16; i += SX_THREADS) reinterpret_cast<stem_u32x4*>(wlds3)[i] = reinterpret_cast<const stem_u32x4*>(a.wp)[i];
    __syncthreads();
    const long ntiles = (long)a.N * a.OH * a.tiles_x;
    const long stride = (long)gridDim.x * SX_WAVES;
    const int woff = l31 * 32 + half * 16;
    float* ep = reinterpret_cast<float*>(wlds3 + SX_WLDS + wave * SX_EP_BYTES);
    const int q8 = lane >> 3, c4 = (lane & 7) * 4;
    float ssum[2][4], ssq[2][4], piv[2][4];
    int cnt = 0;
#pragma unroll
    for (int ct = 0; ct < 2; ++ct)
#pragma unroll
        for (int j = 0; j < 4; ++j) ssum[ct][j] = ssq[ct][j] = piv[ct][j] = 0.f;
    bool first_tile = true;
    for (long tile = (long)blockIdx.x * SX_WAVES + wave; tile < ntiles; tile += stride) {
        const int xt = (int)(tile % a.tiles_x);
        const long r = tile / a.tiles_x;
        const int oy = (int)(r % a.OH);
        const int n = (int)(r / a.OH);
        const int ox = 32 * xt + l31;
        const int oxc = ox < a.OW ? ox : a.OW - 1;
        const unsigned* base = a.xs + ((long)n * a.Hp + 2 * oy) * a.Wp + 2 * oxc + 4 * half;
        stem_f32x16 acc[2];
#pragma unroll
        for (int ct = 0; ct < 2; ++ct)
#pragma unroll
            for (int e = 0; e < 16; ++e) acc[ct][e] = 0.f;
        stem_u32x4 xb[7][3];
#pragma unroll
        for (int ky = 0; ky < 7; ++ky)
#pragma unroll
            for (int sl = 0; sl < 3; ++sl) {
                const unsigned* p = base + sl * a.vol + (long)ky * a.Wp;
                const stem_u32x2 lo = *reinterpret_cast<const stem_u32x2*>(p), hi = *reinterpret_cast<const stem_u32x2*>(p + 2);
                xb[ky][sl] = stem_u32x4{lo[0], lo[1], hi[0], hi[1]};
            }
#pragma unroll
        for (int ky = 0; ky < 7; ++ky)
#pragma unroll
            for (int ct = 0; ct < 2; ++ct) {
                stem_u32x4 wf[3];
#pragma unroll
                for (int sl = 0; sl < 3; ++sl)
                    wf[sl] = *reinterpret_cast<const stem_u32x4*>(wlds3 + ((sl * 7 + ky) * S_CO + 32 * ct) * 32 + woff);
                auto mm = [&](int i, int j) {
                    acc[ct] = __builtin_amdgcn_mfma_f32_32x32x16_bf16(__builtin_bit_cast(stem_bf16x8, wf[i]), __builtin_bit_cast(stem_bf16x8, xb[ky][j]),
                                                                      acc[ct], 0, 0, 0);
                };
                mm(0, 2); mm(2, 0); mm(1, 1); mm(0, 1); mm(1, 0); mm(0, 0);
            }
        float* dst = a.y + (r * a.OW + 32 * xt) * S_CO + c4;
#pragma unroll
        for (int ct = 0; ct < 2; ++ct) {
#pragma unroll
            for (int g = 0; g < 4; ++g)
                *reinterpret_cast<float4*>(ep + l31 * SX_EP_PITCH + 8 * g + 4 * half) =
                    make_float4(acc[ct][4 * g], acc[ct][4 * g + 1], acc[ct][4 * g + 2], acc[ct][4 * g + 3]);
            __builtin_amdgcn_wave_barrier();
#pragma unroll
            for (int i = 0; i < 4; ++i) {
                const int px = 8 * i + q8;
                const float4 v = *reinterpret_cast<const float4*>(ep + px * SX_EP_PITCH + c4);
                if (first_tile && i == 0) {
                    piv[ct][0] = v.x; piv[ct][1] = v.y; piv[ct][2] = v.z; piv[ct][3] = v.w;
                }
                if (32 * xt + px < a.OW) {
                    *reinterpret_cast<float4*>(dst + (long)px * S_CO + 32 * ct) = v;
                    if (a.stat_part) {
                        const float d0 = v.x - piv[ct][0], d1 = v.y - piv[ct][1], d2 = v.z - piv[ct][2], d3 = v.w - piv[ct][3];
                        ssum[ct][0] += d0; ssum[ct][1] += d1; ssum[ct][2] += d2; ssum[ct][3] += d3;
                        ssq[ct][0] = fmaf(d0, d0, ssq[ct][0]); ssq[ct][1] = fmaf(d1, d1, ssq[ct][1]);
                        ssq[ct][2] = fmaf(d2, d2, ssq[ct][2]); ssq[ct][3] = fmaf(d3, d3, ssq[ct][3]);
                        if (ct == 0) ++cnt;
                    }
                }
            }
            __builtin_amdgcn_wave_barrier();
        }
        first_tile = false;
    }
    if (!a.stat_part) return;
    __syncthreads();
    double* red = reinterpret_cast<double*>(wlds3);
#pragma unroll
    for (int ct = 0; ct < 2; ++ct)
#pragma unroll
        for (int j = 0; j < 4; ++j) {
            const double k = (double)piv[ct][j], s1 = (double)ssum[ct][j], nn = (double)cnt;
            double t1 = s1 + nn * k, t2 = (double)ssq[ct][j] + 2.0 * k * s1 + nn * k * k;
#pragma unroll
            for (int m = 8; m < 64; m <<= 1) {
                t1 += __shfl_xor(t1, m, 64);
                t2 += __shfl_xor(t2, m, 64);
            }
            if (lane < 8) {
                red[(wave * 2 + 0) * S_CO + 32 * ct + c4 + j] = t1;
                red[(wave * 2 + 1) * S_CO + 32 * ct + c4 + j] = t2;
            }
        }
    __syncthreads();
    if (tid < 2 * S_CO) {
        const int c = tid & (S_CO - 1), which = tid >> 6;
        double t = 0.0;
#pragma unroll
        for (int w8 = 0; w8 < SX_WAVES; ++w8) t += red[(w8 * 2 + which) * S_CO + c];
        a.stat_part[((size_t)c * BN_MAX_SPLIT + blockIdx.x) * 2 + which] = t;
    }
}

typedef float stem_f32x4 __attribute__((ext_vector_type(4)));
constexpr int SD_WAVES = 4, SD_MT = 8;

__global__ __launch_bounds__(256) void stem_pack_wq3_kernel(const float* __restrict__ w, unsigned short* __restrict__ wq, long s_co, long s_ci,
                                                            long s_ky, long s_kx) {
    const int i = blockIdx.x * 256 + threadIdx.x;
    if (i >= 7 * 16 * S_CO) return;
    const int co = i & 63, j = (i >> 6) & 15, ky = i >> 10;
    unsigned s0 = 0, s1 = 0, s2 = 0;
    if (j < 14) stem_split3(w[co * s_co + (j & 1) * s_ci + ky * s_ky + (j >> 1) * s_kx], s0, s1, s2);
    wq[i] = (unsigned short)s0; wq[7 * 16 * S_CO + i] = (unsigned short)s1; wq[2 * 7 * 16 * S_CO + i] = (unsigned short)s2;
}

struct StemDgArgs {
    const float* dy;
    const unsigned short* wq;
    float* dx;
    int N, H, W, OH, OW;
};

__device__ __forceinline__ void stem_split8(const float4 lo, const float4 hi, stem_u32x4 (&sl)[3]) {
    const float v[8] = {lo.x, lo.y, lo.z, lo.w, hi.x, hi.y, hi.z, hi.w};
    unsigned u[3][8];
#pragma unroll
    for (int e = 0; e < 8; ++e) {
        u[0][e] = __float_as_uint(v[e]);
        const float r1 = v[e] - __uint_as_float(u[0][e] & 0xffff0000u);
        u[1][e] = __float_as_uint(r1);
        u[2][e] = __float_as_uint(r1 - __uint_as_float(u[1][e] & 0xffff0000u));
    }
#pragma unroll
    for (int k = 0; k < 3; ++k)
#pragma unroll
        for (int e = 0; e < 4; ++e) sl[k][e] = __builtin_amdgcn_perm(u[k][2 * e + 1], u[k][2 * e], 0x07060302u);
}

template <int MTC>
__global__ __launch_bounds__(SD_WAVES * 64) void stem_dgrad_x3_kernel(StemDgArgs a) {
    __shared__ float qlds[SD_WAVES][SD_MT * 16 * 16];
    const int lane = threadIdx.x & 63;
    const int wave = __builtin_amdgcn_readfirstlane((int)(threadIdx.x >> 6));
    const int l15 = lane & 15, kg = lane >> 4;
    float* Q = qlds[wave];
    const long nrows = (long)a.N * a.H;
    const int mtiles = MTC ? MTC : (a.OW + 15) / 16;
    const long plane = (long)a.H * a.W;
    for (long row = (long)blockIdx.x * SD_WAVES + wave; row < nrows; row += (long)gridDim.x * SD_WAVES) {
        const int h = (int)(row % a.H);
        const int n = (int)(row / a.H);
        stem_f32x4 acc[SD_MT];
#pragma unroll
        for (int m = 0; m < SD_MT; ++m) acc[m] = stem_f32x4{0.f, 0.f, 0.f, 0.f};
        for (int ky = (h + 1) & 1; ky < S_K; ky += 2) {
            const int oh2 = h + 3 - ky;
            if (oh2 < 0 || (oh2 >> 1) >= a.OH) continue;
            const float* drow = a.dy + ((long)n * a.OH + (oh2 >> 1)) * a.OW * S_CO;
#pragma unroll
            for (int kb = 0; kb < 2; ++kb) {
                stem_u32x4 bf[3];
#pragma unroll
                for (int sl = 0; sl < 3; ++sl)
                    bf[sl] = *reinterpret_cast<const stem_u32x4*>(a.wq + ((sl * 7 + ky) * 16 + l15) * S_CO + 32 * kb + 8 * kg);
                float4 lo[SD_MT], hi[SD_MT];
#pragma unroll
                for (int m = 0; m < SD_MT; ++m) {
                    if (MTC ? m >= MTC : m >= mtiles) continue;
                    int ow = 16 * m + l15;
                    ow = ow < a.OW ? ow : a.OW - 1;
                    const float4* p = reinterpret_cast<const float4*>(drow + (long)ow * S_CO + 32 * kb + 8 * kg);
                    lo[m] = p[0]; hi[m] = p[1];
                }
#pragma unroll
                for (int m = 0; m < SD_MT; ++m) {
                    if (MTC ? m >= MTC : m >= mtiles) continue;
                    stem_u32x4 af[3];
                    stem_split8(lo[m], hi[m], af);
                    auto mm = [&](int i, int j) {
                        acc[m] = __builtin_amdgcn_mfma_f32_16x16x32_bf16(__builtin_bit_cast(stem_bf16x8, af[i]), __builtin_bit_cast(stem_bf16x8, bf[j]),
                                                                         acc[m], 0, 0, 0);
                    };
                    mm(0, 2); mm(2, 0); mm(1, 1); mm(0, 1); mm(1, 0); mm(0, 0);
                }
            }
        }
#pragma unroll
        for (int m = 0; m < SD_MT; ++m) {
            if (m >= mtiles) continue;
#pragma unroll
            for (int q = 0; q < 4; ++q) Q[(16 * m + 4 * kg + q) * 16 + l15] = acc[m][q];
        }
        __builtin_amdgcn_wave_barrier();
        asm volatile("s_waitcnt lgkmcnt(0)" ::: "memory");
        float* dst = a.dx + (long)n * 2 * plane + (long)h * a.W;
        for (int i = lane; i < 2 * a.W; i += 64) {
            const int c = i / a.W, w = i - c * a.W;
            float sum = 0.f;
#pragma unroll
            for (int u = 0; u < 4; ++u) {
                const int kx = ((w + 1) & 1) + 2 * u;
                const int ow2 = w + 3 - kx;
                if (kx < S_K && ow2 >= 0 && (ow2 >> 1) < a.OW) sum += Q[(ow2 >> 1) * 16 + 2 * kx + c];
            }
            dst[c * plane + w] = sum;
        }
        __builtin_amdgcn_wave_barrier();
        asm volatile("s_waitcnt lgkmcnt(0)" ::: "memory");
    }
}

int stem_groups(int N, int H, int W) {
    const int OH = (H + 1) / 2, OW = (W + 1) / 2;
    const long tiles = (long)N * ((OH + S_TH - 1) / S_TH) * ((OW + S_TW - 1) / S_TW);
    return (int)(tiles < S_MAX_GROUPS ? tiles : S_MAX_GROUPS);
}

}

extern "C" {

int dmc_stem_wgrad_supported(int H, int W) { return H > 0 && W > 0 && W % 4 == 0 && ((long)H * W) % 4 == 0; }

size_t dmc_stem_wgrad_partials_bytes(int N, int H, int W) {
    return (size_t)(stem_groups(N, H, W) + S_RED) * S_PART * sizeof(float);
}

int dmc_stem_wgrad(const float* x, const float* dy, float* dw, float* partials, int N, int H, int W,
                   dmc_stream_t stream) {
    if (!x || !dy || !dw || !partials) return fail(DMC_E_INVALID, "dmc_stem_wgrad: null pointer");
    if (N <= 0 || !dmc_stem_wgrad_supported(H, W))
        return fail(DMC_E_INVALID, "dmc_stem_wgrad: unsupported shape N=%d H=%d W=%d (W %% 4 == 0 required)", N, H, W);
    hipStream_t s = (hipStream_t)stream;
    StemArgs a;
    a.x = x; a.dy = dy; a.partials = partials;
    a.N = N; a.H = H; a.W = W; a.OH = (H + 1) / 2; a.OW = (W + 1) / 2;
    a.tiles_x = (a.OW + S_TW - 1) / S_TW;
    a.tiles_y = (a.OH + S_TH - 1) / S_TH;
    const int groups = stem_groups(N, H, W);
    stem_wgrad_kernel<<<groups, 512, 0, s>>>(a);
    int rc = check_launch("stem_wgrad");
    if (rc) return rc;
    stem_reduce1_kernel<<<dim3(S_PART / 256, S_RED), 256, 0, s>>>(partials, groups);
    if ((rc = check_launch("stem_reduce1"))) return rc;
    stem_reduce2_kernel<<<(S_CO * S_NCOL + 255) / 256, 256, 0, s>>>(partials, groups, dw);
    return check_launch("stem_reduce2");
}

int dmc_stem_fwd(const float* x, const float* w, long ws_co, long ws_ci, long ws_ky, long ws_kx, float* y, int N, int H, int W,
                 dmc_stream_t stream) {
    if (!x || !w || !y) return fail(DMC_E_INVALID, "dmc_stem_fwd: null pointer");
    if (N <= 0 || H <= 0 || W <= 0) return fail(DMC_E_INVALID, "dmc_stem_fwd: bad shape");
    StemFwdArgs a;
    a.x = x; a.w = w; a.y = y; a.N = N; a.H = H; a.W = W; a.OH = (H + 1) / 2; a.OW = (W + 1) / 2;
    a.tiles_x = (a.OW + 31) / 32;
    a.ws_co = ws_co; a.ws_ci = ws_ci; a.ws_ky = ws_ky; a.ws_kx = ws_kx;
    const long tiles = (long)N * a.OH * a.tiles_x;
    long blocks = (tiles + 3) / 4;
    if (blocks > 512) blocks = 512;
    stem_fwd_kernel<<<(int)blocks, 256, 0, (hipStream_t)stream>>>(a);
    return check_launch("stem_fwd");
}

size_t dmc_stem_fwd_x3_workspace_bytes(int N, int H, int W) {
    const long Wp = (W + 8 + 3) / 4 * 4;
    return (size_t)3 * N * (H + 6) * Wp * 4 + (size_t)3 * 7 * S_CO * 16 * 2 + 64;
}
int dmc_stem_fwd_x3_stat_blocks(int N, int H, int W) {
    const long tiles = (long)N * ((H + 1) / 2) * (((W + 1) / 2 + 31) / 32);
    const long blocks = (tiles + SX_WAVES - 1) / SX_WAVES;
    return (int)(blocks > 256 ? 256 : blocks);
}
int dmc_stem_fwd_x3(const float* x, const float* w, long ws_co, long ws_ci, long ws_ky, long ws_kx, void* workspace, float* y, int N,
                    int H, int W, dmc_stream_t stream) {
    return dmc_stem_fwd_x3_stats(x, w, ws_co, ws_ci, ws_ky, ws_kx, workspace, y, nullptr, N, H, W, stream);
}
int dmc_stem_fwd_x3_stats(const float* x, const float* w, long ws_co, long ws_ci, long ws_ky, long ws_kx, void* workspace, float* y,
                          void* stat_scratch, int N, int H, int W, dmc_stream_t stream) {
    if (!x || !w || !workspace || !y) return fail(DMC_E_INVALID, "dmc_stem_fwd_x3: null pointer");
    if (N <= 0 || H <= 0 || W <= 0) return fail(DMC_E_INVALID, "dmc_stem_fwd_x3: bad shape");
    hipStream_t s = (hipStream_t)stream;
    const int Hp = H + 6, Wp = (W + 8 + 3) / 4 * 4;
    const long vol = (long)N * Hp * Wp;
    unsigned* xs = (unsigned*)workspace;
    unsigned short* wp = (unsigned short*)((char*)workspace + (size_t)3 * vol * 4);
    stem_prep_x3_kernel<<<(int)((vol + 255) / 256 > 8192 ? 8192 : (vol + 255) / 256), 256, 0, s>>>(x, xs, N, H, W, Hp, Wp);
    int rc = check_launch("stem_prep_x3");
    if (rc) return rc;
    stem_pack_w3_kernel<<<(7 * S_CO * 16 + 255) / 256, 256, 0, s>>>(w, wp, ws_co, ws_ci, ws_ky, ws_kx);
    if ((rc = check_launch("stem_pack_w3"))) return rc;
    StemX3Args a;
    a.xs = xs; a.wp = wp; a.y = y; a.N = N; a.OH = (H + 1) / 2; a.OW = (W + 1) / 2; a.Hp = Hp; a.Wp = Wp;
    a.tiles_x = (a.OW + 31) / 32; a.vol = vol;
    a.stat_part = static_cast<double*>(stat_scratch);
    const long blocks = dmc_stem_fwd_x3_stat_blocks(N, H, W);
    static LdsLimit lim_attr;
    const hipError_t attr = lim_attr.raise(reinterpret_cast<const void*>(&stem_fwd_x3_kernel), SX_LDS);
    if (attr != hipSuccess) return fail(DMC_E_LAUNCH, "dmc_stem_fwd_x3: cannot raise the dynamic LDS limit: %s", hipGetErrorString(attr));
    stem_fwd_x3_kernel<<<(int)blocks, SX_THREADS, SX_LDS, s>>>(a);
    return check_launch("stem_fwd_x3");
}

size_t dmc_stem_dgrad_workspace_bytes(void) { return (size_t)3 * 7 * 16 * S_CO * 2 + 64; }
int dmc_stem_dgrad_supported(int H, int W) { return H > 0 && W > 0 && (W + 1) / 2 <= 16 * SD_MT ? 1 : 0; }
int dmc_stem_dgrad(const float* dy, const float* w, long ws_co, long ws_ci, long ws_ky, long ws_kx, void* workspace, float* dx, int N,
                   int H, int W, dmc_stream_t stream) {
    if (!dy || !w || !workspace || !dx) return fail(DMC_E_INVALID, "dmc_stem_dgrad: null pointer");
    if (N <= 0 || !dmc_stem_dgrad_supported(H, W)) return fail(DMC_E_INVALID, "dmc_stem_dgrad: unsupported shape N=%d H=%d W=%d (W <= 256)", N, H, W);
    hipStream_t s = (hipStream_t)stream;
    unsigned short* wq = static_cast<unsigned short*>(workspace);
    stem_pack_wq3_kernel<<<(7 * 16 * S_CO + 255) / 256, 256, 0, s>>>(w, wq, ws_co, ws_ci, ws_ky, ws_kx);
    int rc = check_launch("stem_pack_wq3");
    if (rc) return rc;
    StemDgArgs a;
    a.dy = dy; a.wq = wq; a.dx = dx; a.N = N; a.H = H; a.W = W; a.OH = (H + 1) / 2; a.OW = (W + 1) / 2;
    const long rows = (long)N * H;
    long blocks = (rows + SD_WAVES - 1) / SD_WAVES;
    if (blocks > 4096) blocks = 4096;
    if (a.OW == 112) stem_dgrad_x3_kernel<7><<<(int)blocks, SD_WAVES * 64, 0, s>>>(a);
    else stem_dgrad_x3_kernel<0><<<(int)blocks, SD_WAVES * 64, 0, s>>>(a);
    return check_launch("stem_dgrad_x3");
}

}
```

dmc-net_amd/ops.py:

```python
import torch

from . import _lib

__all__ = ["gen_tiny", "flow_mse", "consensus_ce", "disc_tail", "bn_act", "bn_act_supported", "prepare_inputs",
           "u8_frames_buffer", "conv_nhwc", "conv_nhwc_supported", "disc_block", "disc_block_supported"]


class EventProbe(object):

    def __init__(self, only=None):
        self.pairs = {}
        self.only = None if only is None else frozenset(only)

    def span(self, name):
        return _Span(self, name)

    def summary(self):
        torch.cuda.synchronize()
        return {k: (sum(a.elapsed_time(b) for a, b in v) / len(v), len(v))
                for k, v in self.pairs.items() if v}


class _Span(object):
    def __init__(self, probe, name):
# ... 86 lines not shown
    @staticmethod
    def backward(ctx, grad_out):
        lib = _lib.load()
        mv, res, saved = ctx.saved_tensors[:3]
        ws = list(ctx.saved_tensors[3:])
        grad_out = grad_out.contiguous()
        n, _, h, w = mv.shape
        dws = [torch.empty_like(x) for x in ws]
        dbs = [torch.empty(s, dtype=d, device=mv.device) for s, d in ctx.bias_like]
        gbuf = _floats(lib.dmc_gen_tiny_gbuf_bytes(n, h, w), mv.device)
        partials = _floats(lib.dmc_gen_tiny_partials_bytes(n, h, w), mv.device)
        work = _floats(lib.dmc_gen_tiny_workspace_bytes(), mv.device)
        with _span("gen_tiny_bwd"):
            _lib.check(lib.dmc_gen_tiny_bwd(_lib.ptr(mv), _lib.ptr(res), _lib.ptr_array(ws),
                                            _lib.ptr(saved), _lib.ptr(grad_out), _lib.ptr_array(dws),
                                            _lib.ptr_array(dbs), _lib.ptr(gbuf), _lib.ptr(partials),
                                            _lib.ptr(work), n, h, w, _stream()),
                       "dmc_gen_tiny_bwd")
        return (None, None, None, None) + tuple(dws) + tuple(dbs)


class _GenTinyMSE(torch.autograd.Function):

    @staticmethod
    def forward(ctx, mv, res, flow, add_mv, *params):
        lib = _lib.load()
        _need_cuda(mv, res, flow, *params)
        if ctx.needs_input_grad[0] or ctx.needs_input_grad[1] or ctx.needs_input_grad[2]:
            raise NotImplementedError("no gradients w.r.t. the MV / residual / flow inputs")
        mv, res, flow = mv.contiguous(), res.contiguous(), flow.contiguous()
        ws, bs = [p.contiguous() for p in params[:6]], [p.contiguous() for p in params[6:]]
        n, _, h, w = mv.shape
        if tuple(flow.shape) != (n, 2, h, w):
            raise ValueError("flow target %s does not match the generator output %s" % (tuple(flow.shape), (n, 2, h, w)))
        out = torch.empty((n, 2, h, w), dtype=torch.float32, device=mv.device)
        loss = torch.empty((), dtype=torch.float32, device=mv.device)
        saved = _floats(lib.dmc_gen_tiny_saved_bytes(n, h, w), mv.device)
        work = _floats(lib.dmc_gen_tiny_workspace_bytes(), mv.device)
        part = _floats(lib.dmc_gen_tiny_mse_partials_bytes(), mv.device)
        with _span("gen_tiny_fwd"):
            _lib.check(lib.dmc_gen_tiny_fwd_mse(_lib.ptr(mv), _lib.ptr(res), _lib.ptr_array(ws), _lib.ptr_array(bs),
                                                _lib.ptr(flow), _lib.ptr(out), _lib.ptr(saved), _lib.ptr(work),
                                                _lib.ptr(loss), _lib.ptr(part), n, h, w, int(add_mv), _stream()),
                       "dmc_gen_tiny_fwd_mse")
        ctx.save_for_backward(mv, res, saved, out, flow, *ws)
        ctx.bias_like = [(b.shape, b.dtype) for b in bs]
        ctx.set_materialize_grads(False)
        return out, loss

    @staticmethod
    def backward(ctx, grad_out, grad_loss):
        lib = _lib.load()
        mv, res, saved, out, flow = ctx.saved_tensors[:5]
        ws = list(ctx.saved_tensors[5:])
        n, _, h, w = mv.shape
        g = None
        if grad_loss is not None:
            g = torch.empty_like(out)
            with _span("flow_mse_bwd"):
                _lib.check(lib.dmc_flow_mse_bwd(_lib.ptr(out), _lib.ptr(flow), _lib.ptr(grad_loss.contiguous().float()),
                                                _lib.ptr(g), out.numel(), _stream()), "dmc_flow_mse_bwd")
        if grad_out is not None:
            g = grad_out.contiguous() if g is None else g.add_(grad_out)
        if g is None:
            return (None,) * (4 + 12)
        dws = [torch.empty_like(x) for x in ws]
        dbs = [torch.empty(s, dtype=d, device=mv.device) for s, d in ctx.bias_like]
        gbuf = _floats(lib.dmc_gen_tiny_gbuf_bytes(n, h, w), mv.device)
        partials = _floats(lib.dmc_gen_tiny_partials_bytes(n, h, w), mv.device)
        work = _floats(lib.dmc_gen_tiny_workspace_bytes(), mv.device)
        with _span("gen_tiny_bwd"):
            _lib.check(lib.dmc_gen_tiny_bwd(_lib.ptr(mv), _lib.ptr(res), _lib.ptr_array(ws), _lib.ptr(saved),
                                            _lib.ptr(g), _lib.ptr_array(dws), _lib.ptr_array(dbs), _lib.ptr(gbuf),
                                            _lib.ptr(partials), _lib.ptr(work), n, h, w, _stream()),
                       "dmc_gen_tiny_bwd")
        return (None, None, None, None) + tuple(dws) + tuple(dbs)


def gen_tiny_mse(mv, res, flow, weights, biases, add_mv=False):
    return _GenTinyMSE.apply(mv, res, flow, bool(add_mv), *weights, *biases)


def gen_tiny(mv, res, weights, biases, add_mv=False):
    return _GenTiny.apply(mv, res, bool(add_mv), torch.is_grad_enabled(), *weights, *biases)


class _FlowMSE(torch.autograd.Function):

    @staticmethod
    def forward(ctx, gen_flow, flow):
        lib = _lib.load()
        _need_cuda(gen_flow, flow)
        if ctx.needs_input_grad[1]:
            raise NotImplementedError("no gradient w.r.t. the flow target")
        if gen_flow.shape != flow.shape:
            raise ValueError("shape mismatch %s vs %s" % (tuple(gen_flow.shape), tuple(flow.shape)))
        gen_flow, flow = gen_flow.contiguous(), flow.contiguous()
        loss = torch.empty((), dtype=torch.float32, device=gen_flow.device)
        partials = _floats(lib.dmc_flow_mse_partials_bytes(), gen_flow.device)
        with _span("flow_mse_fwd"):
            _lib.check(lib.dmc_flow_mse_fwd(_lib.ptr(gen_flow), _lib.ptr(flow), _lib.ptr(loss),
                                            _lib.ptr(partials), gen_flow.numel(), _stream()),
                       "dmc_flow_mse_fwd")
        ctx.save_for_backward(gen_flow, flow)
        return loss

    @staticmethod
    def backward(ctx, grad_loss):
        lib = _lib.load()
        gen_flow, flow = ctx.saved_tensors
        grad_loss = grad_loss.contiguous().float()
        grad = torch.empty_like(gen_flow)
        with _span("flow_mse_bwd"):
            _lib.check(lib.dmc_flow_mse_bwd(_lib.ptr(gen_flow), _lib.ptr(flow), _lib.ptr(grad_loss),
                                            _lib.ptr(grad), gen_flow.numel(), _stream()),
                       "dmc_flow_mse_bwd")
        return grad, None


def flow_mse(gen_flow, flow):
    return _FlowMSE.apply(gen_flow, flow)


class _ConsensusCE(torch.autograd.Function):

    @staticmethod
    def forward(ctx, logits, target, num_segments):
        lib = _lib.load()
        _need_cuda(logits, target)
        if logits.dtype != torch.float32 or target.dtype != torch.int64:
            raise _lib.DmcHipError("consensus_ce expects fp32 logits and int64 class labels, got %s / %s"
                                   % (logits.dtype, target.dtype))
        logits, target = logits.contiguous(), target.contiguous()
        n, c = logits.shape
        if n % num_segments != 0 or target.numel() * num_segments != n:
            raise ValueError("logits %s do not match %d targets x %d segments"
                             % (tuple(logits.shape), target.numel(), num_segments))
        b = n // num_segments
        consensus = torch.empty((b, c), dtype=torch.float32, device=logits.device)
        loss = torch.empty((), dtype=torch.float32, device=logits.device)
        grad = torch.empty_like(logits) if ctx.needs_input_grad[0] else None
        _lib.check(lib.dmc_consensus_ce_fwd_bwd(_lib.ptr(logits), _lib.ptr(target),
                                                _lib.ptr(consensus), _lib.ptr(loss), _lib.ptr(grad),
                                                b, num_segments, c, _stream()),
                   "dmc_consensus_ce_fwd_bwd")
        ctx.save_for_backward(grad)
        ctx.mark_non_differentiable(consensus)
        return loss, consensus

    @staticmethod
    def backward(ctx, grad_loss, _grad_consensus):
        (grad,) = ctx.saved_tensors
        return grad * grad_loss, None, None


def consensus_ce(logits, target, num_segments):
    return _ConsensusCE.apply(logits, target, num_segments)


class _DiscTail(torch.autograd.Function):

    @staticmethod
    def forward(ctx, x, keep, gamma, beta, running_mean, running_var, training, eps, momentum):
        lib = _lib.load()
        _need_cuda(x, keep, gamma, beta)
        x = x.contiguous()
        n, c, h, w = x.shape
        use_bn = gamma is not None
        keep = keep.contiguous() if keep is not None else None
        y = torch.empty_like(x)
        stats = _floats(lib.dmc_disc_tail_stats_bytes(c), x.device) if use_bn else None
        _lib.check(lib.dmc_disc_tail_fwd(_lib.ptr(x), _lib.ptr(keep), _lib.ptr(gamma), _lib.ptr(beta),
                                         _lib.ptr(running_mean), _lib.ptr(running_var), _lib.ptr(y),
                                         _lib.ptr(stats), n, c, h, w, int(use_bn), int(training),
                                         float(eps), float(momentum), _stream()),
                   "dmc_disc_tail_fwd")
        ctx.save_for_backward(x, keep, gamma, stats)
        ctx.use_bn = use_bn
        ctx.training = bool(training)
        return y

    @staticmethod
    def backward(ctx, dy):
        lib = _lib.load()
        x, keep, gamma, stats = ctx.saved_tensors
        if ctx.use_bn and not ctx.training:
            raise NotImplementedError("backward through eval-mode BatchNorm is not implemented")
        dy = dy.contiguous()
        n, c, h, w = x.shape
        dx = torch.empty_like(x)
        dgamma = torch.empty_like(gamma) if ctx.use_bn else None
        dbeta = torch.empty_like(gamma) if ctx.use_bn else None
        _lib.check(lib.dmc_disc_tail_bwd(_lib.ptr(x), _lib.ptr(keep), _lib.ptr(gamma), _lib.ptr(stats),
                                         _lib.ptr(dy), _lib.ptr(dx), _lib.ptr(dgamma), _lib.ptr(dbeta),
                                         n, c, h, w, int(ctx.use_bn), _stream()),
                   "dmc_disc_tail_bwd")
        return dx, None, dgamma, dbeta, None, None, None, None, None


def disc_tail(x, keep, bn, training):
    if bn is None:
        return _DiscTail.apply(x, keep, None, None, None, None, training, 0.0, 0.0)
    if training and bn.num_batches_tracked is not None:
        bn.num_batches_tracked.add_(1)
    return _DiscTail.apply(x, keep, bn.weight, bn.bias, bn.running_mean, bn.running_var, training,
                           bn.eps, bn.momentum)


class _BnAct(torch.autograd.Function):

    @staticmethod
    def forward(ctx, x, residual, gamma, beta, running_mean, running_var, relu, training, eps,
                momentum):
        lib = _lib.load()
        _need_cuda(x, residual, gamma, beta)
        n, c, h, w = x.shape
        m = n * h * w
        y = torch.empty_like(x)
        stats = _floats(lib.dmc_bn_act_stats_bytes(c), x.device)
        scratch = _floats(lib.dmc_bn_act_scratch_bytes(c), x.device) if training else None
        mask = None
        if relu and training and residual is not None:
            mask = torch.empty(m * (c // 4), dtype=torch.uint8, device=x.device)
        with _span("bn_act_fwd"):
            _lib.check(lib.dmc_bn_act_fwd(_lib.ptr(x), _lib.ptr(residual), _lib.ptr(gamma),
                                          _lib.ptr(beta), _lib.ptr(running_mean),
                                          _lib.ptr(running_var), _lib.ptr(y), _lib.ptr(stats),
                                          _lib.ptr(scratch), _lib.ptr(mask), m, c, int(relu), int(training), float(eps),
                                          float(momentum), _stream()), "dmc_bn_act_fwd")
        ctx.save_for_backward(x, residual if (relu and mask is None) else None, gamma, beta, stats, mask)
        ctx.relu, ctx.training, ctx.has_res = bool(relu), bool(training), residual is not None
        return y

    @staticmethod
    def backward(ctx, dy):
        lib = _lib.load()
        x, residual, gamma, beta, stats, mask = ctx.saved_tensors
        if not ctx.training:
            raise NotImplementedError("backward through eval-mode BatchNorm is not implemented")
        n, c, h, w = x.shape
        dy = dy.contiguous(memory_format=torch.channels_last)
        dx = torch.empty_like(x)
        want_dres = ctx.has_res and ctx.needs_input_grad[1]
        dres = torch.empty_like(x) if (want_dres and ctx.relu) else None
        dgamma, dbeta = torch.empty_like(gamma), torch.empty_like(gamma)
        scratch = _floats(lib.dmc_bn_act_scratch_bytes(c), x.device)
        with _span("bn_act_bwd"):
            _lib.check(lib.dmc_bn_act_bwd(_lib.ptr(x), _lib.ptr(residual), _lib.ptr(gamma),
                                          _lib.ptr(beta), _lib.ptr(stats), _lib.ptr(scratch), _lib.ptr(dy), _lib.ptr(dx),
                                          _lib.ptr(dres), _lib.ptr(dgamma), _lib.ptr(dbeta), _lib.ptr(mask),
                                          n * h * w, c, int(ctx.relu), _stream()), "dmc_bn_act_bwd")
        if want_dres and not ctx.relu:
            dres = dy
        return dx, dres, dgamma, dbeta, None, None, None, None, None, None


def bn_act_supported(x):
    if not (x.is_cuda and x.dtype == torch.float32 and x.dim() == 4):
        return False
    if not x.is_contiguous(memory_format=torch.channels_last):
        return False
    n, c, h, w = x.shape
    return bool(_lib.load().dmc_bn_act_supported(n * h * w, c))


_PENDING_COUNTERS = None


class batched_bn_counters:

    def __enter__(self):
        global _PENDING_COUNTERS
        self._outer = _PENDING_COUNTERS
        _PENDING_COUNTERS = []
        return self

    def __exit__(self, *exc):
        global _PENDING_COUNTERS
        pending, _PENDING_COUNTERS = _PENDING_COUNTERS, self._outer
        if pending and exc[0] is None:
            torch._foreach_add_(pending, 1)
        return False


def bn_act(x, bn, residual=None, relu=True):
    training = bn.training
    if training and bn.num_batches_tracked is not None:
        if _PENDING_COUNTERS is not None:
            _PENDING_COUNTERS.append(bn.num_batches_tracked)
        else:
            bn.num_batches_tracked.add_(1)
    if residual is not None:
        residual = residual.contiguous(memory_format=torch.channels_last)
    return _BnAct.apply(x, residual, bn.weight, bn.bias, bn.running_mean, bn.running_var, relu,
                        training, bn.eps, bn.momentum if bn.momentum is not None else 0.1)


POOL_ARGMAX = __import__("os").environ.get("DMC_POOL_ARGMAX", "1") != "0"


class _BnReluPool(torch.autograd.Function):

    @staticmethod
    def forward(ctx, x, gamma, beta, running_mean, running_var, training, eps, momentum, want_slices=False, stat_partials=None):
        lib = _lib.load()
        _need_cuda(x, gamma, beta)
        ctx.set_materialize_grads(False)
        n, c, h, w = x.shape
        ph, pw = (h - 1) // 2 + 1, (w - 1) // 2 + 1
        y = torch.empty((n, c, ph, pw), dtype=x.dtype, device=x.device,
                        memory_format=torch.channels_last)
        stats = _floats(lib.dmc_bn_act_stats_bytes(c), x.device)
        stat_split = 0
        if training and stat_partials is not None and want_slices and c % 16 == 0:
            scratch, stat_split = stat_partials
        else:
            scratch = _floats(lib.dmc_bn_act_scratch_bytes(c), x.device) if training else None
        ys = codes = xmax = None
        with _span("bn_relu_pool_fwd"):
            if want_slices and c % 16 == 0:
                ys = torch.empty(lib.dmc_x3s_slices_bytes(n * ph * pw, c), dtype=torch.uint8, device=x.device)
                if training and POOL_ARGMAX and any(ctx.needs_input_grad[:3]):
                    codes = _floats(lib.dmc_bn_relu_pool_codes_bytes(n, h, w, c), x.device)
                    xmax = torch.empty_like(y)
                _lib.check(lib.dmc_bn_relu_pool_fwd_arg(_lib.ptr(x), _lib.ptr(gamma), _lib.ptr(beta), _lib.ptr(running_mean),
                                                        _lib.ptr(running_var), _lib.ptr(y), _lib.ptr(ys), _lib.ptr(codes),
                                                        _lib.ptr(xmax), _lib.ptr(stats), _lib.ptr(scratch), int(stat_split), n, h, w, c,
                                                        int(training), float(eps), float(momentum), _stream()),
                           "dmc_bn_relu_pool_fwd_arg")
            else:
                _lib.check(lib.dmc_bn_relu_pool_fwd(_lib.ptr(x), _lib.ptr(gamma), _lib.ptr(beta),
                                                    _lib.ptr(running_mean), _lib.ptr(running_var),
                                                    _lib.ptr(y), _lib.ptr(stats), _lib.ptr(scratch), n, h, w, c, int(training),
                                                    float(eps), float(momentum), _stream()),
                           "dmc_bn_relu_pool_fwd")
        if codes is not None:
            ctx.save_for_backward(x, gamma, beta, stats, codes, xmax)
        else:
            ctx.save_for_backward(x, gamma, beta, stats)
        ctx.training = bool(training)
        if ys is None:
            ys = torch.empty(0, dtype=torch.uint8, device=x.device)
        ctx.mark_non_differentiable(ys)
        return y, ys

    @staticmethod
    def backward(ctx, dy, _dys):
        lib = _lib.load()
        x, gamma, beta, stats = ctx.saved_tensors[:4]
        if dy is None:
            return (None,) * 10
        if not ctx.training:
            raise NotImplementedError("backward through eval-mode BatchNorm is not implemented")
        n, c, h, w = x.shape
        dy = dy.contiguous(memory_format=torch.channels_last)
        dx = torch.empty_like(x)
        dgamma, dbeta = torch.empty_like(gamma), torch.empty_like(gamma)
        scratch = _floats(lib.dmc_bn_act_scratch_bytes(c), x.device)
        with _span("bn_relu_pool_bwd"):
            if len(ctx.saved_tensors) == 6:
                codes, xmax = ctx.saved_tensors[4:]
                _lib.check(lib.dmc_bn_relu_pool_bwd_arg(_lib.ptr(x), _lib.ptr(gamma), _lib.ptr(beta), _lib.ptr(stats),
                                                        _lib.ptr(scratch), _lib.ptr(dy), _lib.ptr(codes), _lib.ptr(xmax),
                                                        _lib.ptr(dx), _lib.ptr(dgamma), _lib.ptr(dbeta), n, h, w, c, _stream()),
                           "dmc_bn_relu_pool_bwd_arg")
            else:
                codes = _floats(lib.dmc_bn_relu_pool_codes_bytes(n, h, w, c), x.device)
                _lib.check(lib.dmc_bn_relu_pool_bwd(_lib.ptr(x), _lib.ptr(gamma), _lib.ptr(beta),
                                                    _lib.ptr(stats), _lib.ptr(scratch), _lib.ptr(dy), _lib.ptr(dx),
                                                    _lib.ptr(dgamma), _lib.ptr(dbeta), _lib.ptr(codes),
                                                    n, h, w, c, _stream()), "dmc_bn_relu_pool_bwd")
        return dx, dgamma, dbeta, None, None, None, None, None, None, None


def bn_relu_pool_supported(x):
    if not (x.is_cuda and x.dtype == torch.float32 and x.dim() == 4):
        return False
    if not x.is_contiguous(memory_format=torch.channels_last):
        return False
    n, c, h, w = x.shape
    return bool(_lib.load().dmc_bn_relu_pool_supported(n, h, w, c))


def bn_relu_pool(x, bn, want_slices=False):
    training = bn.training
    if training and bn.num_batches_tracked is not None:
        if _PENDING_COUNTERS is not None:
            _PENDING_COUNTERS.append(bn.num_batches_tracked)
        else:
            bn.num_batches_tracked.add_(1)
    y, ys = _BnReluPool.apply(x, bn.weight, bn.bias, bn.running_mean, bn.running_var, training, bn.eps,
                              bn.momentum if bn.momentum is not None else 0.1, bool(want_slices),
                              getattr(x, "_dmc_stat_partials", None))
    if ys.numel():
        y._dmc_x3s = ys
        y._dmc_f32 = True
    return y


STEM_FWD_HIP = __import__("os").environ.get("DMC_STEM_FWD", "1") != "0"


STEM_DGRAD_HIP = __import__("os").environ.get("DMC_STEM_DGRAD", "1") != "0"


class _StemConv(torch.autograd.Function):

    @staticmethod
    def forward(ctx, x, weight, want_stats=False):
        xc = x.detach().contiguous()
        stat = None
        if STEM_FWD_HIP:
            n, _, h, w = xc.shape
            y = torch.empty((n, 64, (h + 1) // 2, (w + 1) // 2), dtype=torch.float32, device=x.device,
                            memory_format=torch.channels_last)
            so, si, sy, sx = weight.stride()
            lib = _lib.load()
            with _span("stem_fwd"):
                if lib.dmc_get_option(b"conv_arith") == 1:
                    work = _floats(lib.dmc_stem_fwd_x3_workspace_bytes(n, h, w), x.device)
                    if want_stats:
                        stat = _floats(lib.dmc_bn_act_scratch_bytes(64), x.device)
                    _lib.check(lib.dmc_stem_fwd_x3_stats(_lib.ptr(xc), _lib.ptr(weight), so, si, sy, sx, _lib.ptr(work), _lib.ptr(y),
                                                         _lib.ptr(stat), n, h, w, _stream()), "dmc_stem_fwd_x3_stats")
                else:
                    _lib.check(lib.dmc_stem_fwd(_lib.ptr(xc), _lib.ptr(weight), so, si, sy, sx, _lib.ptr(y), n, h, w,
                                                _stream()), "dmc_stem_fwd")
        else:
            y = torch.nn.functional.conv2d(x, weight, None, 2, 3)
        ctx.save_for_backward(xc, weight)
        if stat is None:
            stat = torch.empty(0, dtype=torch.float32, device=x.device)
        ctx.mark_non_differentiable(stat)
        return y, stat

    @staticmethod
    def backward(ctx, dy, _dstat=None):
        lib = _lib.load()
        x, weight = ctx.saved_tensors
        n, _, h, w = x.shape
        dy = dy.contiguous(memory_format=torch.channels_last)
        dw = dx = None
        if ctx.needs_input_grad[1]:
            def launch():
                dw = torch.empty((64, 2, 7, 7), dtype=torch.float32, device=x.device)
                partials = _floats(lib.dmc_stem_wgrad_partials_bytes(n, h, w), x.device)
                _lib.check(lib.dmc_stem_wgrad(_lib.ptr(x), _lib.ptr(dy), _lib.ptr(dw), _lib.ptr(partials),
                                              n, h, w, _stream()), "dmc_stem_wgrad")
                if weight.is_contiguous(memory_format=torch.channels_last) and not weight.is_contiguous():
                    dw = dw.contiguous(memory_format=torch.channels_last)
                return dw
            with _span("stem_wgrad"):
                dw = _on_wgrad_stream(weight, (x, dy), launch)
        if ctx.needs_input_grad[0]:
            if STEM_DGRAD_HIP and dy.dtype == torch.float32 and lib.dmc_stem_dgrad_supported(h, w):
                dx = torch.empty((n, 2, h, w), dtype=torch.float32, device=x.device)
                work = _floats(lib.dmc_stem_dgrad_workspace_bytes(), x.device)
                so, si, sy, sx = weight.stride()
                with _span("stem_dgrad"):
                    _lib.check(lib.dmc_stem_dgrad(_lib.ptr(dy), _lib.ptr(weight), so, si, sy, sx, _lib.ptr(work), _lib.ptr(dx),
                                                  n, h, w, _stream()), "dmc_stem_dgrad")
            else:
                oh, ow = dy.shape[2], dy.shape[3]
                g = dy.permute(0, 2, 3, 1).reshape(n, oh * ow, 64)
                cols = torch.matmul(weight.reshape(64, 98).t(), g.transpose(1, 2))
                dx = torch.nn.functional.fold(cols, (h, w), kernel_size=7, padding=3, stride=2)
        return dx, dw, None


def stem_conv_supported(x, weight):
    return (x.is_cuda and x.dim() == 4 and x.dtype == torch.float32
            and tuple(weight.shape) == (64, 2, 7, 7) and weight.dtype == torch.float32
            and x.shape[1] == 2
            and bool(_lib.load().dmc_stem_wgrad_supported(int(x.shape[2]), int(x.shape[3]))))


STEM_STATS = __import__("os").environ.get("DMC_STEM_STATS", "1") != "0"


def stem_conv(x, weight, want_stats=False):
    _need_cuda(x, weight)
    y, stat = _StemConv.apply(x, weight, bool(want_stats) and STEM_STATS)
    if stat.numel():
        lib = _lib.load()
        y._dmc_stat_partials = (stat, lib.dmc_stem_fwd_x3_stat_blocks(int(x.shape[0]), int(x.shape[2]), int(x.shape[3])))
    return y


_CL = torch.channels_last


def _is_cl(t):
    return t.dim() == 4 and t.is_contiguous(memory_format=_CL)


def conv_nhwc_supported(x, weight, stride, padding):
    if not (x.is_cuda and x.dtype == torch.float32 and x.dim() == 4 and weight.dtype == torch.float32):
        return False
    n, cin, h, w = x.shape
    cout, cin2, kh, kw = weight.shape
    if cin2 != cin:
        return False
    return bool(_lib.load().dmc_conv_nhwc_supported(n, h, w, cin, cout, kh, kw, int(stride), int(padding)))


def _conv_geom(x, weight, stride, padding):
    n, cin, h, w = x.shape
    cout, _, kh, kw = weight.shape
    oh, ow = (h + 2 * padding - kh) // stride + 1, (w + 2 * padding - kw) // stride + 1
    return n, h, w, cin, cout, kh, kw, oh, ow


def _conv_fwd(x, weight, bias, keep, stride, padding, act, want_stats, presplit=None):
    lib = _lib.load()
    n, h, w, cin, cout, kh, kw, oh, ow = _conv_geom(x, weight, stride, padding)
    y = torch.empty((n, cout, oh, ow), dtype=torch.float32, device=x.device, memory_format=_CL)
    part, nblk = None, 0
    if want_stats:
        nblk = lib.dmc_conv_nhwc_stat_blocks(n, h, w, cin, cout, kh, stride, padding)
        part = torch.empty((nblk, cout, 2), dtype=torch.float64, device=x.device)
    wpack = presplit if presplit is not None else _floats(lib.dmc_conv_nhwc_wt_bytes(cin, cout, kh, kw), x.device)
    wptr = None if presplit is not None else _lib.ptr(weight)
    _lib.check(lib.dmc_conv_nhwc_fwd(_lib.ptr(x), wptr, _lib.ptr(wpack), _lib.ptr(bias), _lib.ptr(keep), _lib.ptr(y),
                                     _lib.ptr(part), nblk, n, h, w, cin, cout, kh, kw, stride, padding, int(act),
                                     _stream()), "dmc_conv_nhwc_fwd")
    return y, part, nblk


def _conv_dgrad(dy, weight, x_shape, stride, padding, presplit=None, addend=None):
    lib = _lib.load()
    n, cin, h, w = x_shape
    cout, _, kh, kw = weight.shape
    dx = torch.empty((n, cin, h, w), dtype=torch.float32, device=dy.device, memory_format=_CL)
    wt = presplit if presplit is not None else _floats(lib.dmc_conv_nhwc_wt_bytes(cin, cout, kh, kw), dy.device)
    wptr = None if presplit is not None else _lib.ptr(weight)
    if addend is not None:
        addend = _as_cl(addend)
        _lib.check(lib.dmc_conv_nhwc_dgrad_add(_lib.ptr(dy), wptr, _lib.ptr(wt), _lib.ptr(addend), _lib.ptr(dx), n, h, w,
                                               cin, cout, kh, kw, stride, padding, _stream()), "dmc_conv_nhwc_dgrad_add")
        return dx
    _lib.check(lib.dmc_conv_nhwc_dgrad(_lib.ptr(dy), wptr, _lib.ptr(wt), _lib.ptr(dx), n, h, w, cin,
                                       cout, kh, kw, stride, padding, _stream()), "dmc_conv_nhwc_dgrad")
    return dx


def _conv_wgrad(x, dy, weight, stride, padding):
    lib = _lib.load()
    n, cin, h, w = x.shape
    cout, _, kh, kw = weight.shape
    dw = torch.empty((cout, cin, kh, kw), dtype=torch.float32, device=x.device, memory_format=_CL)
    work = _floats(lib.dmc_conv_nhwc_wgrad_bytes(n, h, w, cin, cout, kh, kw, stride, padding), x.device)
    _lib.check(lib.dmc_conv_nhwc_wgrad(_lib.ptr(x), _lib.ptr(dy), _lib.ptr(dw), _lib.ptr(work), n, h, w, cin, cout,
                                       kh, kw, stride, padding, _stream()), "dmc_conv_nhwc_wgrad")
    return dw


def _as_cl(t):
    return t if _is_cl(t) else t.contiguous(memory_format=_CL)


def _grad_like(dw, weight):
    return dw if _is_cl(weight) and weight.stride() == dw.stride() else dw.contiguous().view_as(weight).contiguous()


class _ConvNHWC(torch.autograd.Function):

    @staticmethod
    def forward(ctx, x, weight, stride, padding):
        _need_cuda(x, weight)
        x, wcl = _as_cl(x), _as_cl(weight)
        with _span("conv_nhwc_fwd"):
            y, _, _ = _conv_fwd(x, wcl, None, None, stride, padding, 0, False)
        ctx.save_for_backward(x, weight)
        ctx.geom = (stride, padding)
        return y

    @staticmethod
    def backward(ctx, dy):
        x, weight = ctx.saved_tensors
        stride, padding = ctx.geom
        dy, wcl = _as_cl(dy), _as_cl(weight)
        dx = dw = None
        if ctx.needs_input_grad[0]:
            with _span("conv_nhwc_dgrad"):
                dx = _conv_dgrad(dy, wcl, x.shape, stride, padding)
        if ctx.needs_input_grad[1]:
            with _span("conv_nhwc_wgrad"):
                dw = _grad_like(_conv_wgrad(x, dy, wcl, stride, padding), weight)
        return dx, dw, None, None


def conv_nhwc(x, weight, stride=1, padding=1):
    return _ConvNHWC.apply(x, weight, int(stride), int(padding))



X3S = __import__("os").environ.get("DMC_X3S", "1") != "0"
BN_BWD_LINK = __import__("os").environ.get("DMC_BN_BWD_LINK", "0") == "1"


def x3s_of(t):
    return getattr(t, "_dmc_x3s", None)


def f32_valid(t):
    return getattr(t, "_dmc_f32", True)


def _attach_x3s(t, xs, has_f32=True):
    t._dmc_x3s = xs
    t._dmc_f32 = has_f32
    return t


def _x3s_buffer(m, c, device):
    return torch.empty(_lib.load().dmc_x3s_slices_bytes(m, c), dtype=torch.uint8, device=device)


def x3s_split(x):
    n, c, h, w = x.shape
    xs = _x3s_buffer(n * h * w, c, x.device)
    _lib.check(_lib.load().dmc_x3s_split(_lib.ptr(x), _lib.ptr(xs), n * h * w, c, _stream()), "dmc_x3s_split")
    return xs


def x3s_merge(xs, shape):
    n, c, h, w = shape
    x = torch.empty(shape, dtype=torch.float32, device=xs.device, memory_format=torch.channels_last)
    _lib.check(_lib.load().dmc_x3s_merge(_lib.ptr(xs), _lib.ptr(x), n * h * w, c, _stream()), "dmc_x3s_merge")
    return x


def x3s_pack_weights(weight, forward=True, transposed=True):
    lib = _lib.load()
    cout, cin = weight.shape[0], weight.shape[1]
    nb = lib.dmc_x3s_wpack_bytes(cin, cout)
    wf = torch.empty(nb, dtype=torch.uint8, device=weight.device) if forward else None
    wt = torch.empty(nb, dtype=torch.uint8, device=weight.device) if transposed else None
    _lib.check(lib.dmc_x3s_pack_weights(_lib.ptr(_as_cl(weight)), _lib.ptr(wf), _lib.ptr(wt), cin, cout, _stream()),
               "dmc_x3s_pack_weights")
    return wf, wt


def x3s_conv_fwd(xs, wpack_f, n, h, w, cin, cout, want_stats=False):
    lib = _lib.load()
    y = torch.empty((n, cout, h, w), dtype=torch.float32, device=xs.device, memory_format=torch.channels_last)
    part, nblk = None, 0
    if want_stats:
        nblk = lib.dmc_x3s_conv_stat_blocks(n, h, w, cout)
        part = torch.empty((nblk, cout, 2), dtype=torch.float64, device=xs.device)
    _lib.check(lib.dmc_x3s_conv_fwd(_lib.ptr(xs), _lib.ptr(wpack_f), _lib.ptr(y), _lib.ptr(part), nblk, n, h, w, cin, cout, _stream()),
               "dmc_x3s_conv_fwd")
    return y, part


def x3s_conv_dgrad(dys, wpack_t, n, h, w, cin, cout, addend=None):
    dx = torch.empty((n, cin, h, w), dtype=torch.float32, device=dys.device, memory_format=torch.channels_last)
    _lib.check(_lib.load().dmc_x3s_conv_dgrad(_lib.ptr(dys), _lib.ptr(wpack_t), _lib.ptr(addend), _lib.ptr(dx), n, h, w, cin, cout,
                                              _stream()), "dmc_x3s_conv_dgrad")
    return dx


def x3s_conv_wgrad(xs, dys, n, h, w, cin, cout):
    lib = _lib.load()
    dw = torch.empty((cout, cin, 3, 3), dtype=torch.float32, device=xs.device, memory_format=torch.channels_last)
    work = _floats(lib.dmc_x3s_conv_wgrad_bytes(n, h, w, cin, cout), xs.device)
    _lib.check(lib.dmc_x3s_conv_wgrad(_lib.ptr(xs), _lib.ptr(dys), _lib.ptr(dw), _lib.ptr(work), n, h, w, cin, cout, _stream()),
               "dmc_x3s_conv_wgrad")
    return dw


def x3s_usable(n, h, w, conv):
    if not X3S or conv.kernel_size != (3, 3) or conv.stride != (1, 1) or conv.padding != (1, 1) or conv.bias is not None:
        return False
    if conv.dilation != (1, 1) or conv.groups != 1:
        return False
    lib = _lib.load()
    if lib.dmc_get_option(b"conv_arith") != 1 or lib.dmc_get_option(b"conv_path") != 1:
        return False
    cin, cout = conv.in_channels, conv.out_channels
    return bool(lib.dmc_x3s_conv_supported(n, h, w, cin, cout)) and bool(lib.dmc_x3s_conv_wgrad_supported(n, h, w, cin, cout))


def x3q_split(x):
    n, c, h, w = x.shape
    xq = _x3s_buffer(n * h * w, c, x.device)
    _lib.check(_lib.load().dmc_x3q_split(_lib.ptr(x), _lib.ptr(xq), n, h, w, c, _stream()), "dmc_x3q_split")
    return xq


def x3q_merge(xq, shape):
    n, c, h, w = shape
    x = torch.empty(shape, dtype=torch.float32, device=xq.device, memory_format=torch.channels_last)
    _lib.check(_lib.load().dmc_x3q_merge(_lib.ptr(xq), _lib.ptr(x), n, h, w, c, _stream()), "dmc_x3q_merge")
    return x


def x3q_pack_weights(w3, w1, forward=True, transposed=True):
    lib = _lib.load()
    cout, cin = w3.shape[0], w3.shape[1]
    nb = lib.dmc_x3q_wpack_bytes(cin, cout)
    wf = torch.empty(nb, dtype=torch.uint8, device=w3.device) if forward else None
    wt = torch.empty(nb, dtype=torch.uint8, device=w3.device) if transposed else None
    _lib.check(lib.dmc_x3q_pack_weights(_lib.ptr(_as_cl(w3)), _lib.ptr(_as_cl(w1)), _lib.ptr(wf), _lib.ptr(wt), cin, cout, _stream()),
               "dmc_x3q_pack_weights")
    return wf, wt


def x3q_conv_fwd(xq, wpack_f, n, oh, ow, cin, cout, want_stats=False):
    lib = _lib.load()
    y3 = torch.empty((n, cout, oh, ow), dtype=torch.float32, device=xq.device, memory_format=torch.channels_last)
    y1 = torch.empty_like(y3)
    p3 = p1 = None
    nblk = 0
    if want_stats:
        nblk = lib.dmc_x3q_stat_blocks(n, oh, ow, cout)
        p3 = torch.empty((nblk, cout, 2), dtype=torch.float64, device=xq.device)
        p1 = torch.empty_like(p3)
    _lib.check(lib.dmc_x3q_conv_fwd(_lib.ptr(xq), _lib.ptr(wpack_f), _lib.ptr(y3), _lib.ptr(y1), _lib.ptr(p3), _lib.ptr(p1), nblk,
                                    n, oh, ow, cin, cout, _stream()), "dmc_x3q_conv_fwd")
    return y3, y1, p3, p1


def x3q_conv_dgrad(dys3, dys1, wpack_t, n, oh, ow, cin, cout):
    dx = torch.empty((n, cin, 2 * oh, 2 * ow), dtype=torch.float32, device=dys3.device, memory_format=torch.channels_last)
    _lib.check(_lib.load().dmc_x3q_conv_dgrad(_lib.ptr(dys3), _lib.ptr(dys1), _lib.ptr(wpack_t), _lib.ptr(dx), n, oh, ow, cin, cout,
                                              _stream()), "dmc_x3q_conv_dgrad")
    return dx


def x3q_conv_wgrad(xq, dys3, dys1, n, oh, ow, cin, cout):
    lib = _lib.load()
    dw3 = torch.empty((cout, cin, 3, 3), dtype=torch.float32, device=xq.device, memory_format=torch.channels_last)
    dw1 = torch.empty((cout, cin, 1, 1), dtype=torch.float32, device=xq.device, memory_format=torch.channels_last)
    work = _floats(lib.dmc_x3q_conv_wgrad_bytes(n, oh, ow, cin, cout), xq.device)
    _lib.check(lib.dmc_x3q_conv_wgrad(_lib.ptr(xq), _lib.ptr(dys3), _lib.ptr(dys1), _lib.ptr(dw3), _lib.ptr(dw1), _lib.ptr(work),
                                      n, oh, ow, cin, cout, _stream()), "dmc_x3q_conv_wgrad")
    return dw3, dw1


class ResidualGradLink:
    __slots__ = ("armed", "grad")

    def __init__(self):
        self.armed = False
        self.grad = None


WGRAD_STREAM = __import__("os").environ.get("DMC_WGRAD_STREAM", "1") != "0"
_WGRAD_STREAMS = {}
_WGRAD_PENDING = [False]
_WGRAD_SCOPE = [0]
_WGRAD_COUNT = [0]
_WGRAD_SEEN = set()
_WGRAD_MAIN = set()


class wgrad_side_stream(object):

    def __enter__(self):
        _WGRAD_SCOPE[0] += 1
        _WGRAD_SEEN.clear()
        _WGRAD_MAIN.clear()
        return self

    def __exit__(self, *exc):
        _WGRAD_SCOPE[0] -= 1
        join_wgrad_stream()
        _WGRAD_SEEN.clear()
        _WGRAD_MAIN.clear()
        return False


def _wgrad_stream(device):
    key = torch.device(device).index
    if key not in _WGRAD_STREAMS:
        _WGRAD_STREAMS[key] = torch.cuda.Stream(device=device)
    return _WGRAD_STREAMS[key]


def join_wgrad_stream():
    if _WGRAD_PENDING[0]:
        cur = torch.cuda.current_stream()
        for st in _WGRAD_STREAMS.values():
            cur.wait_stream(st)
# ... 1185 lines not shown
```

dmc-net_amd/resnet.py:

```python
import torch
from torch import nn

from . import ops


def _bn_act(bn, x, residual=None, relu=True):
    if x.is_cuda and bn.track_running_stats and (bn.training or not torch.is_grad_enabled()) \
            and ops.bn_act_supported(x):
        return ops.bn_act(x, bn, residual, relu)
    y = bn(x)
    if residual is not None:
        y = y + residual
    return torch.relu(y) if relu else y

import os as _os
OWN_CONV = _os.environ.get("DMC_OWN_CONV", "1") != "0"
KEEP_F32_OUTPUTS = _os.environ.get("DMC_KEEP_F32_OUTPUTS", "0") == "1"
RESIDUAL_GRAD_LINK = _os.environ.get("DMC_RESIDUAL_GRAD_LINK", "1") != "0"


def _same_bn_mode(bn, other):
    return (other is not None and other.training == bn.training and other.track_running_stats and other.affine
            and other.momentum is not None)


def _conv_bn_act(conv, bn, x, residual=None, relu=True, link=None, next_conv=None, only_consumer=False, bn_link=None,
                 next_bn=None, next_unit=None):
    train_op = OWN_CONV and x.is_cuda and ops.conv_bn_act_supported(x, conv, bn)
    eval_op = OWN_CONV and x.is_cuda and not train_op and ops.conv_bn_eval_supported(x, conv, bn)
    if train_op and next_unit is not None:
        n, _, h, w = x.shape
        k, s_, p = conv.kernel_size[0], conv.stride[0], conv.padding[0]
        oshape = (n, conv.out_channels, (h + 2 * p - k) // s_ + 1, (w + 2 * p - k) // s_ + 1)
        if ops.s2_pair_usable(oshape, next_unit):
            return ops.conv_bn_act(x, conv, bn, residual, relu, link, want_f32=False, want_slices=True, s2d=True)
    if train_op or eval_op:
        slices = False
        if next_conv is not None:
            n, _, h, w = x.shape
            k, s_, p = conv.kernel_size[0], conv.stride[0], conv.padding[0]
            slices = ops.x3s_usable(n, (h + 2 * p - k) // s_ + 1, (w + 2 * p - k) // s_ + 1, next_conv)
            only_consumer = only_consumer and _same_bn_mode(bn, next_bn)
        if eval_op:
            return ops.conv_bn_act_eval(x, conv, bn, residual, relu, want_f32=not (slices and only_consumer), want_slices=slices)
        return ops.conv_bn_act(x, conv, bn, residual, relu, link, want_f32=not (slices and only_consumer), want_slices=slices,
                               bn_link=bn_link if slices else None)
    if not ops.f32_valid(x):
        raise RuntimeError("the activation's fp32 memory was not written (slices only) but the stock path needs it")
    return _bn_act(bn, conv(x), residual, relu)


_CFG = {
    "resnet18": ("basic", (2, 2, 2, 2)),
    "resnet34": ("basic", (3, 4, 6, 3)),
    "resnet50": ("bottleneck", (3, 4, 6, 3)),
    "resnet101": ("bottleneck", (3, 4, 23, 3)),
    "resnet152": ("bottleneck", (3, 8, 36, 3)),
}


def _conv(cin, cout, k, stride=1):
    return nn.Conv2d(cin, cout, k, stride=stride, padding=k // 2, bias=False)


class ResidualUnit(nn.Module):

    def __init__(self, kind, cin, planes, stride):
        super().__init__()
        self.kind = kind
        cout = planes * (4 if kind == "bottleneck" else 1)
        if kind == "basic":
            self.conv1, self.bn1 = _conv(cin, planes, 3, stride), nn.BatchNorm2d(planes)
            self.conv2, self.bn2 = _conv(planes, planes, 3), nn.BatchNorm2d(planes)
        else:
            self.conv1, self.bn1 = _conv(cin, planes, 1), nn.BatchNorm2d(planes)
            self.conv2, self.bn2 = _conv(planes, planes, 3, stride), nn.BatchNorm2d(planes)
            self.conv3, self.bn3 = _conv(planes, cout, 1), nn.BatchNorm2d(cout)
        self.relu = nn.ReLU(inplace=True)
        self.downsample = None
        if stride != 1 or cin != cout:
            self.downsample = nn.Sequential(_conv(cin, cout, 1, stride), nn.BatchNorm2d(cout))
        self.out_channels = cout
        self.next_conv = [None]
        self.next_identity = [False]
        self.next_unit = [None]

    def _next_unit(self):
        return None if (KEEP_F32_OUTPUTS or self._forward_hooks) else self.next_unit[0]

    def forward(self, x):
        link = None
        if self.downsample is None:
            shortcut = x
            link = ops.ResidualGradLink() if RESIDUAL_GRAD_LINK and x.requires_grad else None
        elif OWN_CONV and x.is_cuda and ops.s2_pair_usable(tuple(x.shape), self) and (ops.x3q_of(x) is not None or ops.f32_valid(x)):
            n, _, h, w = x.shape
            y, shortcut = ops.conv_bn_s2_pair(x, self, want_slices=ops.x3s_usable(n, h // 2, w // 2, self.conv2) and
                                              _same_bn_mode(self.bn1, self.bn2))
            return _conv_bn_act(self.conv2, self.bn2, y, residual=shortcut, next_conv=self.next_conv[0],
                                bn_link="block" if (self.next_identity[0] and RESIDUAL_GRAD_LINK) else None,
                                next_unit=self._next_unit())
        else:
            shortcut = _conv_bn_act(self.downsample[0], self.downsample[1], x, relu=False)
        y = _conv_bn_act(self.conv1, self.bn1, x, link=link, next_conv=self.conv2, only_consumer=True, bn_link="inner",
                         next_bn=self.bn2)
        if self.kind == "basic":
            return _conv_bn_act(self.conv2, self.bn2, y, residual=shortcut, link=link, next_conv=self.next_conv[0],
                                bn_link="block" if (self.next_identity[0] and RESIDUAL_GRAD_LINK) else None,
                                next_unit=self._next_unit())
        y = _conv_bn_act(self.conv2, self.bn2, y, next_conv=self.conv3, only_consumer=True, next_bn=self.bn3)
        return _conv_bn_act(self.conv3, self.bn3, y, residual=shortcut, link=link, next_conv=self.next_conv[0])


class ResNet(nn.Module):
    def __init__(self, kind, depths, num_classes=1000):
        super().__init__()
        self.conv1 = nn.Conv2d(3, 64, 7, stride=2, padding=3, bias=False)
        self.bn1 = nn.BatchNorm2d(64)
        self.relu = nn.ReLU(inplace=True)
        self.maxpool = nn.MaxPool2d(kernel_size=3, stride=2, padding=1)
        width = 64
        for stage, (planes, count) in enumerate(zip((64, 128, 256, 512), depths)):
            units = []
            for j in range(count):
                unit = ResidualUnit(kind, width, planes, 2 if (stage > 0 and j == 0) else 1)
                width = unit.out_channels
                units.append(unit)
            setattr(self, "layer%d" % (stage + 1), nn.Sequential(*units))
        chain = [u for st in (self.layer1, self.layer2, self.layer3, self.layer4) for u in st]
        for u, nxt in zip(chain, chain[1:]):
            u.next_conv[0] = nxt.conv1
            u.next_identity[0] = nxt.downsample is None
            u.next_unit[0] = nxt if (nxt.downsample is not None and kind == "basic") else None
        self.avgpool = nn.AvgPool2d(7, stride=1)
        self.fc = nn.Linear(width, num_classes)

    def _stem(self, x):
        c = self.conv1
        if (c.in_channels == 2 and c.bias is None and c.stride == (2, 2) and c.padding == (3, 3)
                and c.dilation == (1, 1) and c.groups == 1
                and (not torch.is_grad_enabled() or c.weight.requires_grad or x.requires_grad)
                and ops.stem_conv_supported(x, c.weight)):
            return ops.stem_conv(x, c.weight, want_stats=self.bn1.training and self.bn1.track_running_stats)
        return c(x)

    def _stem_tail(self, x):
        bn, mp = self.bn1, self.maxpool
        if (x.is_cuda and bn.track_running_stats and (bn.training or not torch.is_grad_enabled())
                and mp.kernel_size == 3 and mp.stride == 2 and mp.padding == 1 and mp.dilation == 1
                and not mp.ceil_mode and not mp.return_indices and ops.bn_relu_pool_supported(x)):
            n, _, h, w = x.shape
            first = self.layer1[0].conv1
            return ops.bn_relu_pool(x, bn, want_slices=OWN_CONV and (bn.training or not torch.is_grad_enabled()) and
                                    ops.x3s_usable(n, (h - 1) // 2 + 1, (w - 1) // 2 + 1, first))
        return mp(_bn_act(bn, x))

    def forward(self, x):
        with ops.batched_bn_counters():
            x = self._stem_tail(self._stem(x))
            for stage in (self.layer1, self.layer2, self.layer3, self.layer4):
                x = stage(x)
            return self.fc(torch.flatten(self.avgpool(x), 1))


def _torchvision_init(net):
    for m in net.modules():
        if isinstance(m, nn.Conv2d):
            nn.init.kaiming_normal_(m.weight, mode="fan_out", nonlinearity="relu")
        elif isinstance(m, nn.BatchNorm2d):
            nn.init.constant_(m.weight, 1.0)
            nn.init.constant_(m.bias, 0.0)


def build(name, pretrained=False, weights=None):
    import os
    import warnings
    if name not in _CFG:
        raise ValueError("Unknown base model: {}".format(name))
    kind, depths = _CFG[name]
    net = ResNet(kind, depths)
    _torchvision_init(net)
    if weights is None:
        weights = os.environ.get("DMC_RESNET_WEIGHTS")
    if weights is not None:
        sd = torch.load(weights, map_location="cpu") if isinstance(weights, (str, bytes, os.PathLike)) else weights
        net.load_state_dict(sd, strict=True)
    elif pretrained:
        warnings.warn("%s: pretrained=True was requested (as the reference does) but no ImageNet weights "
                      "are available offline; the classifier starts from torchvision's random "
                      "initialisation. Pass weights=<torchvision state dict>, set DMC_RESNET_WEIGHTS, or "
                      "load a checkpoint with train.load_reference_weights." % name, stacklevel=2)
    return net
```

include/dmcnet_hip.h:

```cpp
#ifndef DMCNET_HIP_H
#define DMCNET_HIP_H

#include <stddef.h>
#include <stdint.h>

#ifdef __cplusplus
extern "C" {
#endif

#define DMC_OK 0
#define DMC_E_INVALID (-1)
#define DMC_E_LAUNCH (-2)

typedef void* dmc_stream_t;

int dmc_version(void);
const char* dmc_last_error(void);
int dmc_set_option(const char* name, int value);
int dmc_get_option(const char* name);
int dmc_profile_mark(dmc_stream_t stream);


size_t dmc_gen_tiny_workspace_bytes(void);
size_t dmc_gen_tiny_saved_bytes(int N, int H, int W);

int dmc_gen_tiny_fwd(const float* mv, const float* res, const float* const* w,
                     const float* const* b, float* out, float* saved, float* workspace, int N,
                     int H, int W, int add_mv_delta, dmc_stream_t stream);

size_t dmc_gen_tiny_mse_partials_bytes(void);
int dmc_gen_tiny_fwd_mse(const float* mv, const float* res, const float* const* w, const float* const* b,
                         const float* flow, float* out, float* saved, float* workspace, float* loss_out,
                         void* mse_partials, int N, int H, int W, int add_mv_delta, dmc_stream_t stream);

size_t dmc_gen_tiny_gbuf_bytes(int N, int H, int W);
size_t dmc_gen_tiny_partials_bytes(int N, int H, int W);

int dmc_gen_tiny_bwd(const float* mv, const float* res, const float* const* w,
                     const float* saved, const float* grad_out, float* const* dw,
                     float* const* db, float* gbuf, float* partials, float* workspace, int N,
                     int H, int W, dmc_stream_t stream);

size_t dmc_flow_mse_partials_bytes(void);
int dmc_flow_mse_fwd(const float* gen_flow, const float* flow, float* loss_out, float* partials,
                     size_t numel, dmc_stream_t stream);
int dmc_flow_mse_bwd(const float* gen_flow, const float* flow, const float* grad_loss,
                     float* grad_gen, size_t numel, dmc_stream_t stream);

int dmc_consensus_ce_fwd_bwd(const float* logits, const int64_t* target, float* consensus,
                             float* loss_out, float* grad_logits, int B, int S, int C,
                             dmc_stream_t stream);

size_t dmc_disc_tail_stats_bytes(int C);
int dmc_disc_tail_fwd(const float* x, const float* keep, const float* gamma, const float* beta,
                      float* running_mean, float* running_var, float* y, float* stats, int N,
                      int C, int H, int W, int use_bn, int training, float eps, float momentum,
                      dmc_stream_t stream);
int dmc_disc_tail_bwd(const float* x, const float* keep, const float* gamma, float* stats,
                      const float* dy, float* dx, float* dgamma, float* dbeta, int N, int C, int H,
                      int W, int use_bn, dmc_stream_t stream);

int dmc_bn_act_supported(int M, int C);
size_t dmc_bn_act_stats_bytes(int C);
size_t dmc_bn_act_scratch_bytes(int C);
int dmc_bn_act_fwd(const float* x, const float* residual, const float* gamma, const float* beta,
                   float* running_mean, float* running_var, float* y, float* stats, void* scratch,
                   unsigned char* relu_mask, int M, int C, int relu, int training, float eps,
                   float momentum, dmc_stream_t stream);
int dmc_bn_act_bwd(const float* x, const float* residual, const float* gamma, const float* beta,
                   const float* stats, void* scratch, const float* dy, float* dx, float* dresidual,
                   float* dgamma, float* dbeta, const unsigned char* relu_mask, int M, int C, int relu,
                   dmc_stream_t stream);

int dmc_bn_apply_nhwc(const float* x, const float* gamma, const float* beta, const float* stats, float* y,
                      int M, int C, dmc_stream_t stream);
int dmc_bn_apply_act_nhwc(const float* x, const float* residual, const float* gamma, const float* beta,
                          const float* stats, float* y, unsigned char* relu_mask, int M, int C, int relu,
                          dmc_stream_t stream);
int dmc_bn_bwd_act_nhwc(const float* z, const float* gamma, const float* beta, const float* stats, void* scratch,
                        const float* dy, float* dpre, float* dgamma, float* dbeta, const float* keep, int hw,
                        float slope, int M, int C, dmc_stream_t stream);
int dmc_channel_sum_nhwc(const float* g, void* scratch, float* out, int M, int C, dmc_stream_t stream);

size_t dmc_prepare_inputs_workspace_bytes(int N, int H, int W, int flow_ds_factor);
int dmc_prepare_inputs(const unsigned char* frames_u8, const unsigned char* flip, float* out_flow,
                       float* out_mv, float* out_res, float* workspace, int N, int H, int W,
                       int flow_ds_factor, const float* std4_host, dmc_stream_t stream);

size_t dmc_prepare_crop_workspace_bytes(int N, int OH, int OW, int flow_ds_factor);
int dmc_prepare_inputs_crop(const unsigned char* frames_u8, const int* boxes, const unsigned char* flip,
                            float* out_flow, float* out_mv, float* out_res, float* workspace, int N,
                            int H0, int W0, int OH, int OW, int flow_ds_factor, const float* std4_host,
                            dmc_stream_t stream);

size_t dmc_prepare_views_workspace_bytes(int N_out, int OH, int OW, int flow_ds_factor, int upsample_interp);
int dmc_prepare_inputs_views(const unsigned char* frames_u8, const int* src_index, const int* boxes,
                             const unsigned char* flip, float* out_flow, float* out_mv, float* out_res,
                             void* workspace, int N_src, int N_out, int H0, int W0, int OH, int OW,
                             int flow_ds_factor, int upsample_interp, const float* std4_host, dmc_stream_t stream);
int dmc_prepare_interp_taps(int n_blocks, int factor, int* lo, double* dx, double* t);

size_t dmc_prepare_clip_workspace_bytes(int B, int T, int OH, int OW, int flow_ds_factor);
int dmc_prepare_clip(const unsigned char* clips_u8, const int* plans, float* out, void* workspace,
                     int B, int T, int H0, int W0, int OH, int OW, int flow_ds_factor,
                     int n_norm, const float* mean_host, const float* std_host, dmc_stream_t stream);

int dmc_bn_relu_pool_supported(int N, int H, int W, int C);
int dmc_bn_relu_pool_fwd(const float* x, const float* gamma, const float* beta, float* running_mean,
                         float* running_var, float* y_pool, float* stats, void* scratch, int N, int H,
                         int W, int C, int training, float eps, float momentum, dmc_stream_t stream);
size_t dmc_bn_relu_pool_codes_bytes(int N, int H, int W, int C);
int dmc_bn_relu_pool_bwd(const float* x, const float* gamma, const float* beta, const float* stats,
                         void* scratch, const float* d_pool, float* dx, float* dgamma, float* dbeta,
                         void* codes, int N, int H, int W, int C, dmc_stream_t stream);

int dmc_conv_nhwc_supported(int N, int H, int W, int Cin, int Cout, int KH, int KW, int stride, int pad);
int dmc_conv_nhwc_stat_blocks(int N, int H, int W, int Cin, int Cout, int KH, int stride, int pad);
int dmc_conv_nhwc_fwd(const float* x, const float* w, void* wpack, const float* bias, const float* keep, float* y,
                      double* stat_partials, int stat_blocks, int N, int H, int W, int Cin, int Cout, int KH, int KW, int stride,
                      int pad, int act, dmc_stream_t stream);
int dmc_conv_nhwc_stats_final(const double* partials, int nblk, int C, long count, float* stats,
                              float* running_mean, float* running_var, float eps, float momentum,
                              dmc_stream_t stream);
size_t dmc_conv_nhwc_wt_bytes(int Cin, int Cout, int KH, int KW);
int dmc_conv_nhwc_presplit_supported(int Cin, int Cout);
int dmc_conv_nhwc_split(const float* w, void* wpack_f, void* wpack_t, int Cin, int Cout, int KH, int KW, dmc_stream_t stream);
int dmc_conv_nhwc_dgrad(const float* dy, const float* w, float* wt, float* dx, int N, int H, int W, int Cin,
                        int Cout, int KH, int KW, int stride, int pad, dmc_stream_t stream);
int dmc_conv_nhwc_dgrad_add(const float* dy, const float* w, float* wt, const float* addend, float* dx, int N, int H, int W,
                            int Cin, int Cout, int KH, int KW, int stride, int pad, dmc_stream_t stream);
size_t dmc_conv_nhwc_wgrad_bytes(int N, int H, int W, int Cin, int Cout, int KH, int KW, int stride, int pad);
int dmc_conv_nhwc_wgrad(const float* x, const float* dy, float* dw, float* workspace, int N, int H, int W,
                        int Cin, int Cout, int KH, int KW, int stride, int pad, dmc_stream_t stream);

size_t dmc_x3s_slices_bytes(long M, int C);
int dmc_x3s_split(const float* x, void* xs, long M, int C, dmc_stream_t stream);
int dmc_x3s_merge(const void* xs, float* x, long M, int C, dmc_stream_t stream);
size_t dmc_x3s_wpack_bytes(int Cin, int Cout);
int dmc_x3s_pack_weights(const float* w, void* wpack_f, void* wpack_t, int Cin, int Cout, dmc_stream_t stream);
int dmc_x3s_conv_supported(int N, int H, int W, int Cin, int Cout);
int dmc_x3s_conv_stat_blocks(int N, int H, int W, int Cout);
int dmc_x3s_conv_fwd(const void* xs, const void* wpack_f, float* y, double* stat_partials, int stat_blocks, int N, int H, int W,
                     int Cin, int Cout, dmc_stream_t stream);
int dmc_x3s_conv_dgrad(const void* dys, const void* wpack_t, const float* addend, float* dx, int N, int H, int W, int Cin,
                       int Cout, dmc_stream_t stream);
int dmc_x3s_conv_wgrad_supported(int N, int H, int W, int Cin, int Cout);
size_t dmc_x3s_conv_wgrad_bytes(int N, int H, int W, int Cin, int Cout);
int dmc_x3s_conv_wgrad(const void* xs, const void* dys, float* dw, float* workspace, int N, int H, int W, int Cin, int Cout,
                       dmc_stream_t stream);
int dmc_x3s_conv_dgrad_s2_supported(int N, int OH, int OW, int Cin, int Cout);
int dmc_x3s_pack_weights_s2(const float* w, void* wpack_t2, int Cin, int Cout, dmc_stream_t stream);
int dmc_x3s_conv_dgrad_s2(const void* dys, const void* wpack_t2, float* dx, int N, int OH, int OW, int Cin, int Cout,
                          dmc_stream_t stream);


int dmc_bn_apply_act_x3s(const float* x, const float* residual, const float* gamma, const float* beta, const float* stats,
                         float* y, void* ys, unsigned char* relu_mask, int M, int C, int relu, dmc_stream_t stream);
int dmc_bn_act_bwd_x3s(const float* x, const float* residual, const float* gamma, const float* beta, const float* stats,
                       void* scratch, const float* dy, float* dx, void* dxs, float* dresidual, float* dgamma, float* dbeta,
                       const unsigned char* relu_mask, int M, int C, int relu, dmc_stream_t stream);
int dmc_bn_relu_pool_fwd_x3s(const float* x, const float* gamma, const float* beta, float* running_mean, float* running_var,
                             float* y_pool, void* ys, float* stats, void* scratch, int N, int H, int W, int C, int training,
                             float eps, float momentum, dmc_stream_t stream);
int dmc_bn_relu_pool_fwd_arg(const float* x, const float* gamma, const float* beta, float* running_mean, float* running_var,
                             float* y_pool, void* ys, void* codes, float* xmax, float* stats, void* scratch, int stat_split,
                             int N, int H, int W, int C, int training, float eps, float momentum, dmc_stream_t stream);
int dmc_bn_relu_pool_bwd_arg(const float* x, const float* gamma, const float* beta, const float* stats, void* scratch,
                             const float* d_pool, const void* codes, const float* xmax, float* dx, float* dgamma, float* dbeta,
                             int N, int H, int W, int C, dmc_stream_t stream);
size_t dmc_x3q_wpack_bytes(int Cin, int Cout);
int dmc_x3q_supported(int N, int OH, int OW, int Cin, int Cout);
int dmc_x3q_stat_blocks(int N, int OH, int OW, int Cout);
int dmc_x3q_split(const float* x, void* xq, int N, int H, int W, int C, dmc_stream_t stream);
int dmc_x3q_merge(const void* xq, float* x, int N, int H, int W, int C, dmc_stream_t stream);
int dmc_x3q_pack_weights(const float* w3, const float* w1, void* wpack_f, void* wpack_t, int Cin, int Cout, dmc_stream_t stream);
int dmc_x3q_conv_fwd(const void* xq, const void* wpack_f, float* y3, float* y1, double* stat_partials3, double* stat_partials1,
                     int stat_blocks, int N, int OH, int OW, int Cin, int Cout, dmc_stream_t stream);
int dmc_x3q_conv_dgrad(const void* dys3, const void* dys1, const void* wpack_t, float* dx, int N, int OH, int OW, int Cin, int Cout,
                       dmc_stream_t stream);
int dmc_bn_apply_act_x3q(const float* x, const float* residual, const float* gamma, const float* beta, const float* stats,
                         float* y, void* yq, unsigned char* relu_mask, int N, int H, int W, int C, int relu, dmc_stream_t stream);
int dmc_x3q_conv_wgrad_supported(int N, int OH, int OW, int Cin, int Cout);
size_t dmc_x3q_conv_wgrad_bytes(int N, int OH, int OW, int Cin, int Cout);
int dmc_x3q_conv_wgrad(const void* xq, const void* dys3, const void* dys1, float* dw3, float* dw1, float* workspace, int N, int OH,
                       int OW, int Cin, int Cout, dmc_stream_t stream);

int dmc_x3s_conv_dgrad_bnb(const void* dys, const void* wpack_t, const float* addend, float* dx, const float* bn_y,
                           const float* bn_stats, const float* bn_gamma, const float* bn_beta, const unsigned char* bn_relu_mask,
                           int bn_relu, double* partials, int stat_blocks, float* dgamma, float* dbeta, int N, int H, int W, int Cin,
                           int Cout, dmc_stream_t stream);
int dmc_bn_act_bwd_x3s_apply(const float* x, const float* residual, const float* gamma, const float* beta, const float* stats,
                             const float* dy, float* dx, void* dxs, float* dresidual, const float* dgamma, const float* dbeta,
                             const unsigned char* relu_mask, int M, int C, int relu, dmc_stream_t stream);




int dmc_disc_first_supported(int Cout);
int dmc_disc_first_fwd(const float* x, const float* w, const float* bias, const float* keep, float* z, int M,
                       int H, int W, int Cout, int act, dmc_stream_t stream);
int dmc_disc_first_dgrad(const float* g, const float* w, float* dx, int M, int H, int W, int Cout,
                         dmc_stream_t stream);
size_t dmc_disc_first_wgrad_bytes(int Cout);
int dmc_disc_first_wgrad(const float* x, const float* g, float* dw, float* db, void* workspace, int M, int H,
                         int W, int Cout, dmc_stream_t stream);

int dmc_stem_wgrad_supported(int H, int W);
size_t dmc_stem_wgrad_partials_bytes(int N, int H, int W);
int dmc_stem_wgrad(const float* x, const float* dy, float* dw, float* partials, int N, int H, int W,
                   dmc_stream_t stream);
int dmc_stem_fwd(const float* x, const float* w, long ws_co, long ws_ci, long ws_ky, long ws_kx, float* y, int N, int H, int W,
                 dmc_stream_t stream);
size_t dmc_stem_fwd_x3_workspace_bytes(int N, int H, int W);
int dmc_stem_fwd_x3(const float* x, const float* w, long ws_co, long ws_ci, long ws_ky, long ws_kx, void* workspace, float* y, int N,
                    int H, int W, dmc_stream_t stream);
int dmc_stem_fwd_x3_stat_blocks(int N, int H, int W);
int dmc_stem_fwd_x3_stats(const float* x, const float* w, long ws_co, long ws_ci, long ws_ky, long ws_kx, void* workspace, float* y,
                          void* stat_scratch, int N, int H, int W, dmc_stream_t stream);
size_t dmc_stem_dgrad_workspace_bytes(void);
int dmc_stem_dgrad_supported(int H, int W);
int dmc_stem_dgrad(const float* dy, const float* w, long ws_co, long ws_ci, long ws_ky, long ws_kx, void* workspace, float* dx, int N,
                   int H, int W, dmc_stream_t stream);

int dmc_conv3d_bf16_supported(int N, int D, int H, int W, int Cin, int Cout, int KD, int KH, int KW);
size_t dmc_conv3d_bf16_wpack_bytes(int Cin, int Cout, int KD, int KH, int KW);
int dmc_conv3d_bf16_pack(const float* w, long w_s_co, long w_s_ci, long w_s_tap, void* wpack_f, void* wpack_b, int Cin, int Cout,
                         int KD, int KH, int KW, dmc_stream_t stream);
int dmc_conv3d_bf16_stat_blocks(int N, int D, int H, int W, int Cout);
int dmc_conv3d_bf16_stat_blocks_k(int N, int D, int H, int W, int Cin, int Cout, int KD, int KH, int KW);
int dmc_conv3d_bf16_fwd(const void* x, const float* w, long w_s_co, long w_s_ci, long w_s_tap, void* wpack, void* y,
                        float* stat_partials, int N, int D, int H, int W, int Cin, int Cout, int KD, int KH, int KW,
                        dmc_stream_t stream);
int dmc_conv3d_bf16_dgrad(const void* dy, const float* w, long w_s_co, long w_s_ci, long w_s_tap, void* wpack, void* dx,
                          int N, int D, int H, int W, int Cin, int Cout, int KD, int KH, int KW, dmc_stream_t stream);
size_t dmc_conv3d_bf16_wgrad_bytes(int N, int D, int H, int W, int Cin, int Cout, int KD, int KH, int KW);
int dmc_conv3d_bf16_wgrad(const void* x, const void* dy, float* dw, float* workspace, int N, int D, int H, int W, int Cin,
                          int Cout, int KD, int KH, int KW, dmc_stream_t stream);

int dmc_maxpool3d_tf_out_shape(int D, int H, int W, int C, int kd, int kh, int kw, int sd, int sh, int sw, int* od, int* oh,
                               int* ow);
int dmc_maxpool3d_tf_bf16_fwd(const void* x, void* y, void* code, int N, int D, int H, int W, int C, int kd, int kh, int kw,
                              int sd, int sh, int sw, dmc_stream_t stream);
int dmc_maxpool3d_tf_bf16_bwd(const void* dy, const void* code, void* dx, int N, int D, int H, int W, int C, int kd, int kh,
                              int kw, int sd, int sh, int sw, dmc_stream_t stream);

int dmc_bn3d_bf16_supported(long M, int C);
size_t dmc_bn3d_bf16_scratch_bytes(int C);
int dmc_bn3d_bf16_fwd(const void* y, const float* partials, int nblk, const float* gamma, const float* beta, float* stats,
                      float* running_mean, float* running_var, void* out, long M, int C, int relu, float eps, float momentum,
                      dmc_stream_t stream);
int dmc_bn3d_bf16_fwd_ld(const void* y, const float* partials, int nblk, const float* gamma, const float* beta, float* stats,
                         float* running_mean, float* running_var, void* out, long out_ld, long M, int C, int relu, float eps,
                         float momentum, dmc_stream_t stream);
int dmc_add4_bf16(const void* a, const void* b, const void* c, const void* d, void* out, long n, dmc_stream_t stream);
int dmc_bn3d_bf16_bwd(const void* dout, long dout_ld, const void* y, const float* stats, const float* gamma, const float* beta,
                      float* scratch, void* dy, float* dgamma, float* dbeta, long M, int C, int relu, dmc_stream_t stream);

size_t dmc_unit3d_bf16_fwd_workspace_bytes(int N, int D, int H, int W, int Cin, int Cout, int KD, int KH, int KW);
size_t dmc_unit3d_bf16_bwd_workspace_bytes(int N, int D, int H, int W, int Cin, int Cout, int KD, int KH, int KW);
int dmc_unit3d_bf16_fwd(const void* x, const float* w, const float* gamma, const float* beta, float* running_mean,
                        float* running_var, void* workspace, void* y, void* out, int N, int D, int H, int W, int Cin, int Cout,
                        int KD, int KH, int KW, int relu, float eps, float momentum, dmc_stream_t stream);
int dmc_unit3d_bf16_fwd_into(const void* x, const float* w, const float* gamma, const float* beta, float* running_mean,
                             float* running_var, void* workspace, void* y, void* out, long out_ld, int N, int D, int H, int W, int Cin,
                             int Cout, int KD, int KH, int KW, int relu, float eps, float momentum, dmc_stream_t stream);
int dmc_unit3d_bf16_bwd(const void* dout, long dout_ld, const void* x, const void* y, const void* fwd_workspace, const float* gamma,
                        const float* beta, void* bwd_workspace, void* dy, void* dx, float* dw, float* dgamma, float* dbeta, int N,
                        int D, int H, int W, int Cin, int Cout, int KD, int KH, int KW, int relu, dmc_stream_t stream);
size_t dmc_unit3d_bf16_eval_workspace_bytes(int N, int D, int H, int W, int Cin, int Cout, int KD, int KH, int KW);
int dmc_unit3d_bf16_fwd_eval(const void* x, const float* w, const float* gamma, const float* beta, const float* running_mean,
                             const float* running_var, float eps, void* workspace, void* out, long out_ld, int N, int D, int H, int W,
                             int Cin, int Cout, int KD, int KH, int KW, int relu, dmc_stream_t stream);

size_t dmc_stem3d_bf16_workspace_bytes(int N, int T, int H, int W);
int dmc_stem3d_bf16_stat_blocks(int N, int T, int H, int W);
int dmc_stem3d_bf16_fwd(const float* x, const float* w, void* workspace, void* y, float* stat_partials, int N, int T, int H, int W,
                        dmc_stream_t stream);
size_t dmc_stem3d_bf16_eval_workspace_bytes(int N, int T, int H, int W);
int dmc_stem3d_bf16_fwd_eval(const float* x, const float* w, const float* gamma, const float* beta, const float* running_mean,
                             const float* running_var, float eps, void* workspace, void* y, int N, int T, int H, int W, int relu,
                             dmc_stream_t stream);
size_t dmc_stem3d_bf16_wgrad_workspace_bytes(int N, int T, int H, int W);
int dmc_stem3d_bf16_wgrad(const float* x, const void* dy, float* dw, void* workspace, int N, int T, int H, int W, dmc_stream_t stream);
size_t dmc_stem3d_bf16_dgrad_workspace_bytes(void);
int dmc_stem3d_bf16_dgrad(const void* dy, const float* w, float* dx, void* workspace, int N, int T, int H, int W, dmc_stream_t stream);

size_t dmc_mv_owner_bytes(int n_frames, int H, int W);
int dmc_mv_accu_init(int32_t* accu, int H, int W, dmc_stream_t stream);
int dmc_mv_rasterise(const void* mvs, int mv_stride, int n_mv, int32_t* owner_ws, int32_t* mv_out, int32_t* bad_source, int H,
                     int W, dmc_stream_t stream);
int dmc_mv_accumulate(const void* mvs, int mv_stride, int n_mv, int32_t* owner_ws, const int32_t* accu_old, int32_t* accu_new,
                      int32_t* bad_source, int H, int W, dmc_stream_t stream);
int dmc_mv_from_accu(const int32_t* accu, int32_t* mv_out, int H, int W, dmc_stream_t stream);
int dmc_residual(const uint8_t* bgr_ref, const uint8_t* bgr_cur, const int32_t* accu, const int32_t* mv, int32_t* res, int H, int W,
                 dmc_stream_t stream);
int dmc_mv_gop_batch(const void* mvs, int mv_stride, int n_mv, const int32_t* frame_off, int n_frames, const int32_t* chain_off,
                     int n_chains, const int32_t* emit, int32_t* owner_ws, const uint8_t* bgr_ref, const uint8_t* bgr_cur,
                     int32_t* accu_out, int32_t* mv_out, int32_t* res_out, int32_t* bad_source, int H, int W, dmc_stream_t stream);

#ifdef __cplusplus
}
#endif
#endif
```

Baseline: 3613.

## Fuse BN-ReLU-maxpool backward dx recompute into stem conv wgrad kernel

The stem BN+ReLU+maxpool backward now only computes dgamma/dbeta sums and hands its operands to the stem conv backward through a link object. The stem wgrad kernel gains a fused variant that stages pooled gradients and argmax codes into LDS and recomputes the BN input gradient on the fly, so the full-resolution dx tensor is never written and read back. This adds LDS per block, cross-autograd coupling through a side channel, and only applies when the input does not require grad.

```diff
diff --git a/dmc-net_amd/_lib.py b/dmc-net_amd/_lib.py
--- a/dmc-net_amd/_lib.py
+++ b/dmc-net_amd/_lib.py
@@ -98,6 +98,7 @@
     "dmc_bn_relu_pool_fwd_x3s": (_I, [_P] * 9 + [_I, _I, _I, _I, _I, _F, _F, _P]),
     "dmc_bn_relu_pool_fwd_arg": (_I, [_P] * 11 + [_I, _I, _I, _I, _I, _I, _F, _F, _P]),
     "dmc_bn_relu_pool_bwd_arg": (_I, [_P] * 11 + [_I, _I, _I, _I, _P]),
+    "dmc_bn_relu_pool_bwd_sums": (_I, [_P] * 8 + [_I, _I, _I, _I, _P]),
     "dmc_disc_first_supported": (_I, [_I]),
     "dmc_disc_first_fwd": (_I, [_P] * 5 + [_I] * 5 + [_P]),
     "dmc_disc_first_dgrad": (_I, [_P] * 3 + [_I] * 4 + [_P]),
@@ -106,6 +107,9 @@
     "dmc_stem_wgrad_supported": (_I, [_I, _I]),
     "dmc_stem_wgrad_partials_bytes": (_Z, [_I, _I, _I]),
     "dmc_stem_wgrad": (_I, [_P, _P, _P, _P, _I, _I, _I, _P]),
+    "dmc_stem_wgrad_bnpool_supported": (_I, [_I, _I]),
+    "dmc_stem_wgrad_bnpool_workspace_bytes": (_Z, [_I, _I, _I]),
+    "dmc_stem_wgrad_bnpool": (_I, [_P] * 11 + [_I, _I, _I, _P]),
     "dmc_stem_fwd": (_I, [_P, _P, _L, _L, _L, _L, _P, _I, _I, _I, _P]),
     "dmc_stem_fwd_x3_workspace_bytes": (_Z, [_I, _I, _I]),
     "dmc_stem_fwd_x3": (_I, [_P, _P, _L, _L, _L, _L, _P, _P, _I, _I, _I, _P]),
diff --git a/dmc-net_amd/build.py b/dmc-net_amd/build.py
--- a/dmc-net_amd/build.py
+++ b/dmc-net_amd/build.py
@@ -71,7 +71,7 @@
             continue
         obj = os.path.join(CSRC, src.replace(".hip", ".o"))
         objs.append(obj)
-        hdrs = [os.path.join(CSRC, "dmc_common.h"), os.path.join(CSRC, "x3s_common.h"), os.path.join(CSRC, "conv_small.h"), os.path.join(CSRC, "gen_x3.h"), os.path.join(CSRC, "gen_fused.h"), os.path.join(CSRC, "gen_fused_inl.h"), os.path.join(CSRC, "gen_wgrad.h"), os.path.join(ROOT, "include", "dmcnet_hip.h"),
+        hdrs = [os.path.join(CSRC, "dmc_common.h"), os.path.join(CSRC, "x3s_common.h"), os.path.join(CSRC, "pool_bwd.h"), os.path.join(CSRC, "conv_small.h"), os.path.join(CSRC, "gen_x3.h"), os.path.join(CSRC, "gen_fused.h"), os.path.join(CSRC, "gen_fused_inl.h"), os.path.join(CSRC, "gen_wgrad.h"), os.path.join(ROOT, "include", "dmcnet_hip.h"),
                 os.path.abspath(__file__)]
         if not force and os.path.exists(obj) and all(os.path.getmtime(d) <= os.path.getmtime(obj) for d in [path] + hdrs):
             continue
diff --git a/dmc-net_amd/csrc/bn_act.hip b/dmc-net_amd/csrc/bn_act.hip
--- a/dmc-net_amd/csrc/bn_act.hip
+++ b/dmc-net_amd/csrc/bn_act.hip
@@ -1,4 +1,5 @@
 #include "dmc_common.h"
+#include "pool_bwd.h"
 
 using namespace dmc;
 
@@ -335,45 +336,24 @@
             if (iy >= a.H || ix >= a.W) continue;
             const size_t o = ((size_t)(n * a.H + iy) * a.W + ix) * cq + tx;
             const float4 x = reinterpret_cast<const float4*>(a.x)[o];
-            const float4 xh = make_float4((x.x - mean.x) * istd.x, (x.y - mean.y) * istd.y,
-                                          (x.z - mean.z) * istd.z, (x.w - mean.w) * istd.w);
-            const float4 v = make_float4(fmaf(xh.x, g.x, b.x), fmaf(xh.y, g.y, b.y), fmaf(xh.z, g.z, b.z), fmaf(xh.w, g.w, b.w));
-            float4 d = make_float4(0.f, 0.f, 0.f, 0.f);
-            const int py0 = iy >> 1, px0 = ix >> 1, npy = 1 + (iy & 1), npx = 1 + (ix & 1);
+            const float4 xh = bn_xhat4(x, mean, istd);
             float4 gp[4];
             unsigned cd[4];
             bool okc[4];
+            int pyc[4], pxc[4];
+            pool_bwd_windows(iy, ix, a.PH, a.PW, pyc, pxc, okc);
 #pragma unroll
             for (int q = 0; q < 4; ++q) {
-                const int jy = q >> 1, jx = q & 1;
-                const int py = py0 + jy, px = px0 + jx;
-                okc[q] = jy < npy && jx < npx && py < a.PH && px < a.PW;
-                const int pyc = okc[q] ? py : py0, pxc = okc[q] ? px : px0;
-                cd[q] = codes[((pyc - wy0) * (PT + 1) + (pxc - wx0)) * cq + tx];
-                gp[q] = reinterpret_cast<const float4*>(a.dpool)[((size_t)(n * a.PH + pyc) * a.PW + pxc) * cq + tx];
+                cd[q] = codes[((pyc[q] - wy0) * (PT + 1) + (pxc[q] - wx0)) * cq + tx];
+                gp[q] = reinterpret_cast<const float4*>(a.dpool)[((size_t)(n * a.PH + pyc[q]) * a.PW + pxc[q]) * cq + tx];
             }
-#pragma unroll
-            for (int q = 0; q < 4; ++q) {
-                const int py = py0 + (q >> 1), px = px0 + (q & 1);
-                const unsigned k = (unsigned)((iy - 2 * py + 1) * 3 + (ix - 2 * px + 1));
-                if (okc[q] && (cd[q] & 0xff) == k) d.x += gp[q].x;
-                if (okc[q] && ((cd[q] >> 8) & 0xff) == k) d.y += gp[q].y;
-                if (okc[q] && ((cd[q] >> 16) & 0xff) == k) d.z += gp[q].z;
-                if (okc[q] && (cd[q] >> 24) == k) d.w += gp[q].w;
-            }
-            d.x = v.x > 0.f ? d.x : 0.f; d.y = v.y > 0.f ? d.y : 0.f;
-            d.z = v.z > 0.f ? d.z : 0.f; d.w = v.w > 0.f ? d.w : 0.f;
+            const float4 d = pool_bwd_relu(pool_bwd_route(iy, ix, gp, cd, okc), xh, g, b);
             if (PASS == 1) {
                 s0.x += d.x; s0.y += d.y; s0.z += d.z; s0.w += d.w;
                 s1.x = fmaf(d.x, xh.x, s1.x); s1.y = fmaf(d.y, xh.y, s1.y);
                 s1.z = fmaf(d.z, xh.z, s1.z); s1.w = fmaf(d.w, xh.w, s1.w);
             } else {
-                float4 r;
-                r.x = g.x * istd.x * (d.x - db.x * inv_count - xh.x * dg.x * inv_count);
-                r.y = g.y * istd.y * (d.y - db.y * inv_count - xh.y * dg.y * inv_count);
-                r.z = g.z * istd.z * (d.z - db.z * inv_count - xh.z * dg.z * inv_count);
-                r.w = g.w * istd.w * (d.w - db.w * inv_count - xh.w * dg.w * inv_count);
-                reinterpret_cast<float4*>(a.dx)[o] = r;
+                reinterpret_cast<float4*>(a.dx)[o] = bn_bwd_dx4(d, xh, g, istd, dg, db, inv_count);
             }
         }
     }
@@ -810,6 +790,24 @@
                                     training, eps, momentum, stream);
 }
 
+int dmc_bn_relu_pool_bwd_sums(const float* gamma, const float* beta, const float* stats, void* scratch_, const float* d_pool,
+                              const float* xmax, float* dgamma, float* dbeta, int N, int H, int W, int C, dmc_stream_t stream) {
+    if (!gamma || !beta || !stats || !scratch_ || !d_pool || !xmax || !dgamma || !dbeta)
+        return fail(DMC_E_INVALID, "dmc_bn_relu_pool_bwd_sums: null pointer");
+    if (!dmc_bn_relu_pool_supported(N, H, W, C) || C % 16 != 0)
+        return fail(DMC_E_INVALID, "dmc_bn_relu_pool_bwd_sums: unsupported shape N=%d H=%d W=%d C=%d", N, H, W, C);
+    hipStream_t s = (hipStream_t)stream;
+    double* scratch = static_cast<double*>(scratch_);
+    const int MP = N * ((H - 1) / 2 + 1) * ((W - 1) / 2 + 1);
+    BnArgs a = {xmax, nullptr, gamma, beta, stats, d_pool, nullptr, nullptr, nullptr, MP, C, 1, nullptr};
+    const int split = split_of(MP, C);
+    bn_partial_kernel<1><<<split, 256, 0, s>>>(a, scratch);
+    int rc = check_launch("pool_bwd_sums");
+    if (rc) return rc;
+    bn_bwd_final_kernel<<<C, 256, 0, s>>>(scratch, dgamma, dbeta, C, split);
+    return check_launch("bn_bwd_final");
+}
+
 int dmc_bn_relu_pool_bwd_arg(const float* x, const float* gamma, const float* beta, const float* stats, void* scratch_,
                              const float* d_pool, const void* codes, const float* xmax, float* dx, float* dgamma, float* dbeta,
                              int N, int H, int W, int C, dmc_stream_t stream) {
@@ -819,15 +817,8 @@
         return fail(DMC_E_INVALID, "dmc_bn_relu_pool_bwd_arg: unsupported shape N=%d H=%d W=%d C=%d", N, H, W, C);
     hipStream_t s = (hipStream_t)stream;
     PoolArgs p = {x, gamma, beta, stats, d_pool, nullptr, dx, N, H, W, C, (H - 1) / 2 + 1, (W - 1) / 2 + 1};
-    double* scratch = static_cast<double*>(scratch_);
-    const int MP = N * p.PH * p.PW;
-    BnArgs a = {xmax, nullptr, gamma, beta, stats, d_pool, nullptr, nullptr, nullptr, MP, C, 1, nullptr};
-    const int split = split_of(MP, C);
-    int rc;
-    bn_partial_kernel<1><<<split, 256, 0, s>>>(a, scratch);
-    if ((rc = check_launch("pool_bwd_sums"))) return rc;
-    bn_bwd_final_kernel<<<C, 256, 0, s>>>(scratch, dgamma, dbeta, C, split);
-    if ((rc = check_launch("bn_bwd_final"))) return rc;
+    const int rc = dmc_bn_relu_pool_bwd_sums(gamma, beta, stats, scratch_, d_pool, xmax, dgamma, dbeta, N, H, W, C, stream);
+    if (rc) return rc;
     const long tiles = (long)N * ((p.PH + PT - 1) / PT) * ((p.PW + PT - 1) / PT);
     const long blocks = tiles * 4 > 8192 ? 8192 : tiles * 4;
     pool_bwd_kernel<2><<<(int)blocks, 256, 0, s>>>(p, nullptr, dgamma, dbeta, 1.f / (float)((long)N * H * W),
diff --git a/dmc-net_amd/csrc/pool_bwd.h b/dmc-net_amd/csrc/pool_bwd.h
--- /dev/null
+++ b/dmc-net_amd/csrc/pool_bwd.h
@@ -0,0 +1,52 @@
+#pragma once
+#include <hip/hip_runtime.h>
+
+namespace dmc {
+
+__device__ __forceinline__ void pool_bwd_windows(int iy, int ix, int PH, int PW, int (&pyc)[4], int (&pxc)[4], bool (&ok)[4]) {
+    const int py0 = iy >> 1, px0 = ix >> 1, npy = 1 + (iy & 1), npx = 1 + (ix & 1);
+#pragma unroll
+    for (int q = 0; q < 4; ++q) {
+        const int jy = q >> 1, jx = q & 1;
+        const int py = py0 + jy, px = px0 + jx;
+        ok[q] = jy < npy && jx < npx && py < PH && px < PW;
+        pyc[q] = ok[q] ? py : py0;
+        pxc[q] = ok[q] ? px : px0;
+    }
+}
+
+__device__ __forceinline__ float4 pool_bwd_route(int iy, int ix, const float4 (&gp)[4], const unsigned (&cd)[4], const bool (&ok)[4]) {
+    const int py0 = iy >> 1, px0 = ix >> 1;
+    float4 d = make_float4(0.f, 0.f, 0.f, 0.f);
+#pragma unroll
+    for (int q = 0; q < 4; ++q) {
+        const int py = py0 + (q >> 1), px = px0 + (q & 1);
+        const unsigned k = (unsigned)((iy - 2 * py + 1) * 3 + (ix - 2 * px + 1));
+        if (ok[q] && (cd[q] & 0xff) == k) d.x += gp[q].x;
+        if (ok[q] && ((cd[q] >> 8) & 0xff) == k) d.y += gp[q].y;
+        if (ok[q] && ((cd[q] >> 16) & 0xff) == k) d.z += gp[q].z;
+        if (ok[q] && (cd[q] >> 24) == k) d.w += gp[q].w;
+    }
+    return d;
+}
+
+__device__ __forceinline__ float4 bn_xhat4(const float4 x, const float4 mean, const float4 istd) {
+    return make_float4((x.x - mean.x) * istd.x, (x.y - mean.y) * istd.y, (x.z - mean.z) * istd.z, (x.w - mean.w) * istd.w);
+}
+
+__device__ __forceinline__ float4 pool_bwd_relu(const float4 d, const float4 xh, const float4 g, const float4 b) {
+    const float4 v = make_float4(fmaf(xh.x, g.x, b.x), fmaf(xh.y, g.y, b.y), fmaf(xh.z, g.z, b.z), fmaf(xh.w, g.w, b.w));
+    return make_float4(v.x > 0.f ? d.x : 0.f, v.y > 0.f ? d.y : 0.f, v.z > 0.f ? d.z : 0.f, v.w > 0.f ? d.w : 0.f);
+}
+
+__device__ __forceinline__ float4 bn_bwd_dx4(const float4 d, const float4 xh, const float4 g, const float4 istd, const float4 dg,
+                                             const float4 db, float inv_count) {
+    float4 r;
+    r.x = g.x * istd.x * (d.x - db.x * inv_count - xh.x * dg.x * inv_count);
+    r.y = g.y * istd.y * (d.y - db.y * inv_count - xh.y * dg.y * inv_count);
+    r.z = g.z * istd.z * (d.z - db.z * inv_count - xh.z * dg.z * inv_count);
+    r.w = g.w * istd.w * (d.w - db.w * inv_count - xh.w * dg.w * inv_count);
+    return r;
+}
+
+}
diff --git a/dmc-net_amd/csrc/stem.hip b/dmc-net_amd/csrc/stem.hip
--- a/dmc-net_amd/csrc/stem.hip
+++ b/dmc-net_amd/csrc/stem.hip
@@ -1,4 +1,7 @@
+#include <type_traits>
+
 #include "dmc_common.h"
+#include "pool_bwd.h"
 
 using namespace dmc;
 
@@ -16,12 +19,29 @@
 constexpr int S_PART = S_MT * S_NT * 256;
 constexpr int S_MAX_GROUPS = 256, S_RED = 16;
 static_assert(S_PART <= 2 * S_BUF, "cross-wave reduction reuses the tile buffers");
+constexpr int S_PR = 5, S_PC = S_TW / 2 + 1;
+constexpr int S_DP = S_PR * S_PC * S_CO;
+constexpr int S_CD = S_PR * S_PC * (S_CO / 4);
+constexpr int S_BUF_F = S_BUF + S_DP + S_CD;
+static_assert((S_BUF * 4) % 16 == 0 && (S_DP * 4) % 16 == 0 && (S_BUF_F * 4) % 16 == 0, "16-byte LDS-DMA destinations");
 
 struct StemArgs {
     const float* x;
     const float* dy;
     float* partials;
     int N, H, W, OH, OW, tiles_x, tiles_y;
+};
+
+struct StemFusedArgs : StemArgs {
+    const float* gamma;
+    const float* beta;
+    const float* stats;
+    const float* dgamma;
+    const float* dbeta;
+    const float* dpool;
+    const unsigned* codes;
+    int PH, PW;
+    float inv_count;
 };
 
 __device__ __forceinline__ void stem_stage(const StemArgs& a, float* buf, int tile, int per_frame, int lane) {
@@ -68,8 +88,45 @@
     }
 }
 
-__global__ __launch_bounds__(512, 2) void stem_wgrad_kernel(StemArgs a) {
-    __shared__ __attribute__((aligned(16))) float lds2[2 * S_BUF];
+__device__ __forceinline__ void stem_stage_pool(const StemFusedArgs& a, float* buf, int tile, int per_frame, int lane) {
+    const int n = tile / per_frame, r0 = tile - n * per_frame;
+    const int pyb = ((r0 / a.tiles_x) * S_TH) >> 1, pxb = ((r0 % a.tiles_x) * S_TW) >> 1;
+    const unsigned buf_byte = lds_addr_of(buf);
+    const size_t win0 = ((size_t)n * a.PH + pyb) * a.PW + pxb;
+    {
+        constexpr int ROWC = S_PC * S_CO / 4;
+        const unsigned long long pbase = (unsigned long long)(a.dpool + win0 * S_CO);
+#pragma unroll
+        for (int h = 0; h < (S_PR * ROWC + 63) / 64; ++h) {
+            const int L = 64 * h + lane;
+            const int row = L / ROWC, ch = L - row * ROWC;
+            if (L < S_PR * ROWC) {
+                const bool ok = pyb + row < a.PH && pxb + ch / (S_CO / 4) < a.PW;
+                if (ok) lds_dma16(pbase, (unsigned)(row * a.PW * S_CO + ch * 4) * 4, buf_byte + (unsigned)(S_BUF + 256 * h) * 4);
+                else reinterpret_cast<float4*>(buf + S_BUF)[L] = make_float4(0.f, 0.f, 0.f, 0.f);
+            }
+        }
+    }
+    {
+        constexpr int ROWC = S_PC * (S_CO / 4) / 4;
+        const unsigned long long cbase = (unsigned long long)(a.codes + win0 * (S_CO / 4));
+#pragma unroll
+        for (int h = 0; h < (S_PR * ROWC + 63) / 64; ++h) {
+            const int L = 64 * h + lane;
+            const int row = L / ROWC, ch = L - row * ROWC;
+            if (L < S_PR * ROWC) {
+                const bool ok = pyb + row < a.PH && pxb + ch / 4 < a.PW;
+                if (ok) lds_dma16(cbase, (unsigned)(row * a.PW * (S_CO / 4) + ch * 4) * 4, buf_byte + (unsigned)(S_BUF + S_DP + 256 * h) * 4);
+                else reinterpret_cast<float4*>(buf + S_BUF + S_DP)[L] = make_float4(0.f, 0.f, 0.f, 0.f);
+            }
+        }
+    }
+}
+
+template <bool FUSED>
+__global__ __launch_bounds__(512, 2) void stem_wgrad_kernel(std::conditional_t<FUSED, StemFusedArgs, StemArgs> a) {
+    constexpr int BUF = FUSED ? S_BUF_F : S_BUF;
+    __shared__ __attribute__((aligned(16))) float lds2[2 * BUF];
     const int lane = threadIdx.x & 63;
     const int wave = __builtin_amdgcn_readfirstlane((int)(threadIdx.x >> 6));
     const int j = lane & 15, kq = lane >> 4;
@@ -84,11 +141,17 @@
 
     if (wave == S_TH) {
         int it = 0;
-        if ((int)blockIdx.x < ntiles) stem_stage(a, lds2, blockIdx.x, per_frame, lane);
+        if ((int)blockIdx.x < ntiles) {
+            stem_stage(a, lds2, blockIdx.x, per_frame, lane);
+            if constexpr (FUSED) stem_stage_pool(a, lds2, blockIdx.x, per_frame, lane);
+        }
         asm volatile("s_waitcnt vmcnt(0) lgkmcnt(0)\n\ts_barrier" ::: "memory");
         for (int tile = blockIdx.x; tile < ntiles; tile += gridDim.x, ++it) {
             const int next = tile + (int)gridDim.x;
-            if (next < ntiles) stem_stage(a, lds2 + ((it + 1) & 1) * S_BUF, next, per_frame, lane);
+            if (next < ntiles) {
+                stem_stage(a, lds2 + ((it + 1) & 1) * BUF, next, per_frame, lane);
+                if constexpr (FUSED) stem_stage_pool(a, lds2 + ((it + 1) & 1) * BUF, next, per_frame, lane);
+            }
             asm volatile("s_waitcnt vmcnt(0) lgkmcnt(0)\n\ts_barrier" ::: "memory");
         }
     } else {
@@ -101,13 +164,46 @@
             offB[t] = ci * S_XPLANE + (2 * wave + ky) * S_XPITCH + kx + 1 + 2 * kq;
         }
         const int offA = S_X + (wave * S_TW + kq) * S_CO + 4 * j;
+        float4 mean, istd, gam, bet, dgam, dbet;
+        if constexpr (FUSED) {
+            mean = reinterpret_cast<const float4*>(a.stats)[j];
+            istd = reinterpret_cast<const float4*>(a.stats + S_CO)[j];
+            gam = reinterpret_cast<const float4*>(a.gamma)[j];
+            bet = reinterpret_cast<const float4*>(a.beta)[j];
+            dgam = reinterpret_cast<const float4*>(a.dgamma)[j];
+            dbet = reinterpret_cast<const float4*>(a.dbeta)[j];
+        }
         int it = 0;
         asm volatile("s_barrier" ::: "memory");
         for (int tile = blockIdx.x; tile < ntiles; tile += gridDim.x, ++it) {
-            const float* lds = lds2 + (it & 1) * S_BUF;
+            const float* lds = lds2 + (it & 1) * BUF;
+            int iy = 0, ix0 = 0, pyb = 0, pxb = 0;
+            if constexpr (FUSED) {
+                const int n = tile / per_frame, r0 = tile - n * per_frame;
+                const int oy0 = (r0 / a.tiles_x) * S_TH, ox0 = (r0 % a.tiles_x) * S_TW;
+                iy = oy0 + wave; ix0 = ox0 + kq; pyb = oy0 >> 1; pxb = ox0 >> 1;
+            }
 #pragma unroll
             for (int g = 0; g < S_TW / 4; ++g) {
-                const float4 av = *reinterpret_cast<const float4*>(lds + offA + g * 4 * S_CO);
+                float4 av = *reinterpret_cast<const float4*>(lds + offA + g * 4 * S_CO);
+                if constexpr (FUSED) {
+                    const int ix = ix0 + 4 * g;
+                    int pyc[4], pxc[4];
+                    bool okc[4];
+                    float4 gp[4];
+                    unsigned cd[4];
+                    pool_bwd_windows(iy, ix, a.PH, a.PW, pyc, pxc, okc);
+#pragma unroll
+                    for (int q = 0; q < 4; ++q) {
+                        const int wi = (pyc[q] - pyb) * S_PC + (pxc[q] - pxb);
+                        cd[q] = reinterpret_cast<const unsigned*>(lds + S_BUF + S_DP)[wi * (S_CO / 4) + j];
+                        gp[q] = *reinterpret_cast<const float4*>(lds + S_BUF + wi * S_CO + 4 * j);
+                    }
+                    const float4 xh = bn_xhat4(av, mean, istd);
+                    const float4 d = pool_bwd_relu(pool_bwd_route(iy, ix, gp, cd, okc), xh, gam, bet);
+                    const float4 r = bn_bwd_dx4(d, xh, gam, istd, dgam, dbet, a.inv_count);
+                    av = (iy < a.OH && ix < a.OW) ? r : make_float4(0.f, 0.f, 0.f, 0.f);
+                }
                 const float am[S_MT] = {av.x, av.y, av.z, av.w};
                 float b[S_NT];
 #pragma unroll
@@ -117,6 +213,7 @@
 #pragma unroll
                     for (int t = 0; t < S_NT; ++t)
                         acc[m][t] = __builtin_amdgcn_mfma_f32_16x16x4f32(am[m], b[t], acc[m][t], 0, 0, 0);
+                if constexpr (FUSED) __builtin_amdgcn_sched_barrier(0);
             }
             asm volatile("s_barrier" ::: "memory");
         }
@@ -561,8 +658,40 @@
     a.tiles_x = (a.OW + S_TW - 1) / S_TW;
     a.tiles_y = (a.OH + S_TH - 1) / S_TH;
     const int groups = stem_groups(N, H, W);
-    stem_wgrad_kernel<<<groups, 512, 0, s>>>(a);
+    stem_wgrad_kernel<false><<<groups, 512, 0, s>>>(a);
     int rc = check_launch("stem_wgrad");
+    if (rc) return rc;
+    stem_reduce1_kernel<<<dim3(S_PART / 256, S_RED), 256, 0, s>>>(partials, groups);
+    if ((rc = check_launch("stem_reduce1"))) return rc;
+    stem_reduce2_kernel<<<(S_CO * S_NCOL + 255) / 256, 256, 0, s>>>(partials, groups, dw);
+    return check_launch("stem_reduce2");
+}
+
+int dmc_stem_wgrad_bnpool_supported(int H, int W) { return dmc_stem_wgrad_supported(H, W); }
+
+size_t dmc_stem_wgrad_bnpool_workspace_bytes(int N, int H, int W) { return dmc_stem_wgrad_partials_bytes(N, H, W); }
+
+int dmc_stem_wgrad_bnpool(const float* x, const float* y1, const float* gamma, const float* beta, const float* stats,
+                          const float* dgamma, const float* dbeta, const float* dpool, const void* codes, float* dw,
+                          void* workspace, int N, int H, int W, dmc_stream_t stream) {
+    if (!x || !y1 || !gamma || !beta || !stats || !dgamma || !dbeta || !dpool || !codes || !dw || !workspace)
+        return fail(DMC_E_INVALID, "dmc_stem_wgrad_bnpool: null pointer");
+    if (N <= 0 || !dmc_stem_wgrad_bnpool_supported(H, W))
+        return fail(DMC_E_INVALID, "dmc_stem_wgrad_bnpool: unsupported shape N=%d H=%d W=%d (W %% 4 == 0 required)", N, H, W);
+    hipStream_t s = (hipStream_t)stream;
+    float* partials = static_cast<float*>(workspace);
+    StemFusedArgs a;
+    a.x = x; a.dy = y1; a.partials = partials;
+    a.N = N; a.H = H; a.W = W; a.OH = (H + 1) / 2; a.OW = (W + 1) / 2;
+    a.tiles_x = (a.OW + S_TW - 1) / S_TW;
+    a.tiles_y = (a.OH + S_TH - 1) / S_TH;
+    a.gamma = gamma; a.beta = beta; a.stats = stats; a.dgamma = dgamma; a.dbeta = dbeta; a.dpool = dpool;
+    a.codes = static_cast<const unsigned*>(codes);
+    a.PH = (a.OH - 1) / 2 + 1; a.PW = (a.OW - 1) / 2 + 1;
+    a.inv_count = 1.f / (float)((long)N * a.OH * a.OW);
+    const int groups = stem_groups(N, H, W);
+    stem_wgrad_kernel<true><<<groups, 512, 0, s>>>(a);
+    int rc = check_launch("stem_wgrad_bnpool");
     if (rc) return rc;
     stem_reduce1_kernel<<<dim3(S_PART / 256, S_RED), 256, 0, s>>>(partials, groups);
     if ((rc = check_launch("stem_reduce1"))) return rc;
diff --git a/dmc-net_amd/ops.py b/dmc-net_amd/ops.py
--- a/dmc-net_amd/ops.py
+++ b/dmc-net_amd/ops.py
@@ -412,10 +412,12 @@
 class _BnReluPool(torch.autograd.Function):
 
     @staticmethod
-    def forward(ctx, x, gamma, beta, running_mean, running_var, training, eps, momentum, want_slices=False, stat_partials=None):
+    def forward(ctx, x, gamma, beta, running_mean, running_var, training, eps, momentum, want_slices=False, stat_partials=None,
+                stem_link=None):
         lib = _lib.load()
         _need_cuda(x, gamma, beta)
         ctx.set_materialize_grads(False)
+        ctx.stem_link = None
         n, c, h, w = x.shape
         ph, pw = (h - 1) // 2 + 1, (w - 1) // 2 + 1
         y = torch.empty((n, c, ph, pw), dtype=x.dtype, device=x.device,
@@ -446,6 +448,9 @@
                            "dmc_bn_relu_pool_fwd")
         if codes is not None:
             ctx.save_for_backward(x, gamma, beta, stats, codes, xmax)
+            if stem_link is not None:
+                ctx.stem_link = stem_link
+                stem_link.armed = True
         else:
             ctx.save_for_backward(x, gamma, beta, stats)
         ctx.training = bool(training)
@@ -459,14 +464,23 @@
         lib = _lib.load()
         x, gamma, beta, stats = ctx.saved_tensors[:4]
         if dy is None:
-            return (None,) * 10
+            return (None,) * 11
         if not ctx.training:
             raise NotImplementedError("backward through eval-mode BatchNorm is not implemented")
         n, c, h, w = x.shape
         dy = dy.contiguous(memory_format=torch.channels_last)
-        dx = torch.empty_like(x)
         dgamma, dbeta = torch.empty_like(gamma), torch.empty_like(gamma)
         scratch = _floats(lib.dmc_bn_act_scratch_bytes(c), x.device)
+        link = ctx.stem_link
+        if link is not None and dy.dtype == torch.float32:
+            codes, xmax = ctx.saved_tensors[4:]
+            with _span("bn_relu_pool_bwd"):
+                _lib.check(lib.dmc_bn_relu_pool_bwd_sums(_lib.ptr(gamma), _lib.ptr(beta), _lib.ptr(stats), _lib.ptr(scratch),
+                                                         _lib.ptr(dy), _lib.ptr(xmax), _lib.ptr(dgamma), _lib.ptr(dbeta), n, h, w, c,
+                                                         _stream()), "dmc_bn_relu_pool_bwd_sums")
+            link.operands = (x, gamma, beta, stats, dgamma, dbeta, dy, codes)
+            return (None, dgamma, dbeta) + (None,) * 8
+        dx = torch.empty_like(x)
         with _span("bn_relu_pool_bwd"):
             if len(ctx.saved_tensors) == 6:
                 codes, xmax = ctx.saved_tensors[4:]
@@ -480,7 +494,7 @@
                                                     _lib.ptr(stats), _lib.ptr(scratch), _lib.ptr(dy), _lib.ptr(dx),
                                                     _lib.ptr(dgamma), _lib.ptr(dbeta), _lib.ptr(codes),
                                                     n, h, w, c, _stream()), "dmc_bn_relu_pool_bwd")
-        return dx, dgamma, dbeta, None, None, None, None, None, None, None
+        return dx, dgamma, dbeta, None, None, None, None, None, None, None, None
 
 
 def bn_relu_pool_supported(x):
@@ -501,7 +515,7 @@
             bn.num_batches_tracked.add_(1)
     y, ys = _BnReluPool.apply(x, bn.weight, bn.bias, bn.running_mean, bn.running_var, training, bn.eps,
                               bn.momentum if bn.momentum is not None else 0.1, bool(want_slices),
-                              getattr(x, "_dmc_stat_partials", None))
+                              getattr(x, "_dmc_stat_partials", None), getattr(x, "_dmc_stem_link", None))
     if ys.numel():
         y._dmc_x3s = ys
         y._dmc_f32 = True
@@ -514,12 +528,25 @@
 STEM_DGRAD_HIP = __import__("os").environ.get("DMC_STEM_DGRAD", "1") != "0"
 
 
+STEM_WGRAD_FUSED = __import__("os").environ.get("DMC_STEM_WGRAD_FUSED", "1") != "0"
+
+
+class StemTailLink:
+    __slots__ = ("armed", "operands")
+
+    def __init__(self):
+        self.armed, self.operands = False, None
+
+
 class _StemConv(torch.autograd.Function):
 
     @staticmethod
-    def forward(ctx, x, weight, want_stats=False):
+    def forward(ctx, x, weight, want_stats=False, link=None):
         xc = x.detach().contiguous()
         stat = None
+        ctx.link = link
+        if link is not None:
+            ctx.set_materialize_grads(False)
         if STEM_FWD_HIP:
             n, _, h, w = xc.shape
             y = torch.empty((n, 64, (h + 1) // 2, (w + 1) // 2), dtype=torch.float32, device=x.device,
@@ -549,6 +576,25 @@
         lib = _lib.load()
         x, weight = ctx.saved_tensors
         n, _, h, w = x.shape
+        link = ctx.link
+        if dy is None:
+            if link is None or link.operands is None:
+                return None, None, None, None
+            y1, gamma, beta, stats, dgamma, dbeta, dpool, codes = link.operands
+            link.operands = None
+
+            def launch_fused():
+                dw = torch.empty((64, 2, 7, 7), dtype=torch.float32, device=x.device)
+                work = _floats(lib.dmc_stem_wgrad_bnpool_workspace_bytes(n, h, w), x.device)
+                _lib.check(lib.dmc_stem_wgrad_bnpool(_lib.ptr(x), _lib.ptr(y1), _lib.ptr(gamma), _lib.ptr(beta), _lib.ptr(stats),
+                                                     _lib.ptr(dgamma), _lib.ptr(dbeta), _lib.ptr(dpool), _lib.ptr(codes), _lib.ptr(dw),
+                                                     _lib.ptr(work), n, h, w, _stream()), "dmc_stem_wgrad_bnpool")
+                if weight.is_contiguous(memory_format=torch.channels_last) and not weight.is_contiguous():
+                    dw = dw.contiguous(memory_format=torch.channels_last)
+                return dw
+            with _span("stem_wgrad"):
+                dw = _on_wgrad_stream(weight, (x, y1, stats, dgamma, dbeta, dpool, codes), launch_fused)
+            return None, dw, None, None
         dy = dy.contiguous(memory_format=torch.channels_last)
         dw = dx = None
         if ctx.needs_input_grad[1]:
@@ -575,7 +621,7 @@
                 g = dy.permute(0, 2, 3, 1).reshape(n, oh * ow, 64)
                 cols = torch.matmul(weight.reshape(64, 98).t(), g.transpose(1, 2))
                 dx = torch.nn.functional.fold(cols, (h, w), kernel_size=7, padding=3, stride=2)
-        return dx, dw, None
+        return dx, dw, None, None
 
 
 def stem_conv_supported(x, weight):
@@ -588,9 +634,16 @@
 STEM_STATS = __import__("os").environ.get("DMC_STEM_STATS", "1") != "0"
 
 
-def stem_conv(x, weight, want_stats=False):
+def stem_conv(x, weight, want_stats=False, tail_follows=False):
     _need_cuda(x, weight)
-    y, stat = _StemConv.apply(x, weight, bool(want_stats) and STEM_STATS)
+    link = None
+    if (tail_follows and STEM_WGRAD_FUSED and STEM_FWD_HIP and torch.is_grad_enabled() and weight.requires_grad
+            and not x.requires_grad
+            and _lib.load().dmc_stem_wgrad_bnpool_supported(int(x.shape[2]), int(x.shape[3]))):
+        link = StemTailLink()
+    y, stat = _StemConv.apply(x, weight, bool(want_stats) and STEM_STATS, link)
+    if link is not None:
+        y._dmc_stem_link = link
     if stat.numel():
         lib = _lib.load()
         y._dmc_stat_partials = (stat, lib.dmc_stem_fwd_x3_stat_blocks(int(x.shape[0]), int(x.shape[2]), int(x.shape[3])))
diff --git a/dmc-net_amd/resnet.py b/dmc-net_amd/resnet.py
--- a/dmc-net_amd/resnet.py
+++ b/dmc-net_amd/resnet.py
@@ -141,7 +141,7 @@
                 and c.dilation == (1, 1) and c.groups == 1
                 and (not torch.is_grad_enabled() or c.weight.requires_grad or x.requires_grad)
                 and ops.stem_conv_supported(x, c.weight)):
-            return ops.stem_conv(x, c.weight, want_stats=self.bn1.training and self.bn1.track_running_stats)
+            return ops.stem_conv(x, c.weight, want_stats=self.bn1.training and self.bn1.track_running_stats, tail_follows=True)
         return c(x)
 
     def _stem_tail(self, x):
diff --git a/include/dmcnet_hip.h b/include/dmcnet_hip.h
--- a/include/dmcnet_hip.h
+++ b/include/dmcnet_hip.h
@@ -168,6 +168,8 @@
 int dmc_bn_relu_pool_bwd_arg(const float* x, const float* gamma, const float* beta, const float* stats, void* scratch,
                              const float* d_pool, const void* codes, const float* xmax, float* dx, float* dgamma, float* dbeta,
                              int N, int H, int W, int C, dmc_stream_t stream);
+int dmc_bn_relu_pool_bwd_sums(const float* gamma, const float* beta, const float* stats, void* scratch, const float* d_pool,
+                              const float* xmax, float* dgamma, float* dbeta, int N, int H, int W, int C, dmc_stream_t stream);
 size_t dmc_x3q_wpack_bytes(int Cin, int Cout);
 int dmc_x3q_supported(int N, int OH, int OW, int Cin, int Cout);
 int dmc_x3q_stat_blocks(int N, int OH, int OW, int Cout);
@@ -209,6 +211,11 @@
 size_t dmc_stem_wgrad_partials_bytes(int N, int H, int W);
 int dmc_stem_wgrad(const float* x, const float* dy, float* dw, float* partials, int N, int H, int W,
                    dmc_stream_t stream);
+int dmc_stem_wgrad_bnpool_supported(int H, int W);
+size_t dmc_stem_wgrad_bnpool_workspace_bytes(int N, int H, int W);
+int dmc_stem_wgrad_bnpool(const float* x, const float* y1, const float* gamma, const float* beta, const float* stats,
+                          const float* dgamma, const float* dbeta, const float* dpool, const void* codes, float* dw,
+                          void* workspace, int N, int H, int W, dmc_stream_t stream);
 int dmc_stem_fwd(const float* x, const float* w, long ws_co, long ws_ci, long ws_ky, long ws_kx, float* y, int N, int H, int W,
                  dmc_stream_t stream);
 size_t dmc_stem_fwd_x3_workspace_bytes(int N, int H, int W);
```

After: 3630, median of 6. About the same (+0.5%).
